# andi611/ZeroSpeech-TTS-without-T

Measured on AMD Instinct MI355X. Metric: mel-frames/sec (train_ae, seg_len=128, enc_size=1024), higher is better.
Workload: dtype bf16; 1 GPU; train_ae english hps seg_len=128 enc_size=1024 emb_size=1024 n_speakers=102 F=513, batch=256/GPU, dropout+Gumbel on, fwd+bwd+clip+Adam; global_batch=256, parallelism=dp1

## Files before the change

include/zs_amd.h:

```cpp
#ifndef ZS_AMD_H
#define ZS_AMD_H
#include <stddef.h>
#include <stdint.h>

#ifdef __cplusplus
extern "C" {
#endif

#define ZS_ABI_VERSION 1

enum { ZS_F32 = 0, ZS_BF16 = 1 };
enum { ZS_OK = 0, ZS_EINVAL = -1, ZS_ELAUNCH = -2, ZS_EWORKSPACE = -3 };
enum { ZS_PAD_ZERO = 0, ZS_PAD_REFLECT = 1 };
enum { ZS_ACT_NONE = 0, ZS_ACT_LRELU = 1, ZS_ACT_SIGMOID = 2, ZS_ACT_TANH = 3 };
enum { ZS_STORE_ROWS = 0, ZS_STORE_SPLIT2 = 1 };
enum { ZS_RES_NONE = 0, ZS_RES_IDENTITY = 1, ZS_RES_AVGPOOL2 = 2, ZS_RES_UPSAMPLE2 = 3 };

int zs_abi_version(void);
const char* zs_last_error(void);
int zs_set_option(const char* key, int value);

typedef struct {
  int32_t dtype;
  const void* A; int64_t lda; int64_t a_batch_stride;
  int32_t B, T_in, T_out;
  int32_t taps, stride, pad_left, pad_mode, gather;
  int32_t cin_pad;
  const void* W; int64_t ldw;
  int32_t N, n_pad;
  const float* bias;
  const float* pre_vec; int64_t pre_vec_ld; const int64_t* vec_idx;
  int32_t act; float slope;
  const void* dact_src; int64_t dact_ld;
  const void* add_src; int64_t add_ld; int32_t add_f32;
  void* out; int64_t ldc; int32_t out_f32; int32_t out_cols; int32_t store_mode;
  void* out2; int64_t ldc2; int32_t out2_cols; int32_t store_mode2;
  const float* vec2; int64_t vec2_ld;
  int32_t groups; int64_t a_gstride, w_gstride, out_gstride, bias_gstride;
  float* colsum; int64_t colsum_ld; int32_t colsum_col0;
  int32_t colsum_post;
  const int32_t* lengths; int32_t pad_right;
  int32_t w_in, w_out, taps_h;
} ZsGemmConv;
int zs_gemm_conv(const ZsGemmConv* p, void* stream);
enum { ZS_GEMM_PATH_P8 = 0, ZS_GEMM_PATH_RING_PP = 1, ZS_GEMM_PATH_RING = 2, ZS_GEMM_PATH_DMA64 = 3, ZS_GEMM_PATH_DMA128 = 4,
       ZS_GEMM_PATH_REG = 5 };
int zs_gemm_conv_path(const ZsGemmConv* p);

typedef struct {
  int32_t dtype;
  const void* dY; int64_t ldy; int32_t y_cols;
  const void* X; int64_t ldx; int64_t x_batch_stride; int32_t x_cols;
  int32_t B, T_in, T_out;
  int32_t taps, stride, pad_left, pad_mode;
  int32_t Cout, Cin;
  float* dW; int64_t so, si, sj;
  float* db;
  int32_t co_split2; int32_t accumulate;
  int32_t splits;
  void* workspace; size_t workspace_bytes;
  int32_t w_in, w_out, taps_h;
} ZsGemmWgrad;
size_t zs_gemm_wgrad_workspace_bytes(const ZsGemmWgrad* p);
int zs_gemm_wgrad(const ZsGemmWgrad* p, void* stream);

typedef struct {
  int32_t dtype;
  const float* W; int64_t so, si, sj;
  int32_t Cout, Cin, taps;
  int32_t transpose, co_split2;
  int32_t inner_pad;
  void* dst; int64_t ldw;
  int32_t n_rows, n_cols, row_offset, col_offset;
  const int32_t* row_perm;
} ZsPackWeight;
int zs_pack_weight(const ZsPackWeight* p, void* stream);
int zs_pack_weight_batch(const ZsPackWeight* jobs, int32_t n, int32_t max_blocks, void* stream);

typedef struct {
  const float* src; float* dst;
  int32_t len, src_stride, dst_stride;
} ZsVecCopy;
int zs_copy_vec_batch(const ZsVecCopy* jobs, int32_t n, void* stream);

typedef struct {
  int32_t dtype;
  const void* src; int64_t ld_src; int32_t src_f32;
  void* dst; int64_t ld_dst; int32_t dst_f32; int32_t col_off;
  int64_t rows; int32_t cols, fill_cols;
  int32_t act; float slope;
  void* dst2; int64_t ld_dst2; int32_t col_off2, fill_cols2; int32_t act2; float slope2;
} ZsCastRows;
int zs_cast_rows(const ZsCastRows* p, void* stream);

typedef struct {
  int32_t dtype;
  const void* x; int64_t ldx;
  const float* vec; int64_t vec_ld; const int64_t* idx;
  void* out; int64_t ldo; int32_t B, T, C, fill_cols;
} ZsAddRowvec;
int zs_add_rowvec(const ZsAddRowvec* p, void* stream);

typedef struct {
  int32_t dtype;
  const void* x; int64_t ldx;
  void* out; int64_t ldo;
  void* out2; int64_t ldo2; const float* vec2; int64_t vec2_ld; int32_t vec2_cols; const int64_t* idx;
  float* mean; float* rstd;
  int32_t B, T, C; float eps;
  float drop_p; uint64_t seed; uint32_t stream_id; const uint8_t* mask; int64_t mask_ld;
  int32_t res_mode; const void* res; int64_t ldres; int32_t T_res; int32_t res_pad_mode;
  const uint64_t* seed_ptr;
  const int32_t* lengths; const int32_t* res_lengths;
  int32_t stats_given;
} ZsInstNormFwd;
int zs_instnorm_fwd(const ZsInstNormFwd* p, void* stream);

typedef struct {
  int32_t dtype;
  const void* dout; int64_t ldd;
  const void* x; int64_t ldx;
  const float* mean; const float* rstd;
  void* dz; int64_t ldz;
  int32_t B, T, C;
  float drop_p; uint64_t seed; uint32_t stream_id; const uint8_t* mask; int64_t mask_ld;
  float slope;
  const uint64_t* seed_ptr;
} ZsInstNormBwd;
int zs_instnorm_bwd(const ZsInstNormBwd* p, void* stream);

typedef struct {
  int32_t dtype;
  const void* gp; int64_t ldg; int32_t pad_left, pad_right, pad_mode;
  int32_t B, T, C;
  float* emb_sum; int64_t emb_ld; int32_t emb_cols;
  int32_t res_mode; const void* res; int64_t ldres;
  const void* dact_src; int64_t dact_ld; float slope;
  void* out; int64_t ldo; int32_t unshuffle;
} ZsGradCombine;
int zs_grad_combine(const ZsGradCombine* p, void* stream);
int zs_norm_decomposition(int32_t kernel, int32_t dtype, int32_t T, int32_t C);

typedef struct {
  const float* emb_sum; int64_t emb_ld; const int64_t* idx; int32_t B;
  float* demb; int64_t demb_ld; int32_t n_rows, C; int32_t accumulate;
} ZsEmbScatter;
int zs_emb_scatter(const ZsEmbScatter* p, void* stream);

typedef struct {
  int32_t dtype;
  const void* logits; int64_t ld; int32_t logits_f32;
  const float* noise; int32_t noise_kind; uint64_t seed;
  int64_t rows; int32_t E; float tau;
  void* bits; int64_t ld_bits; int32_t bits_fill_cols;
  float* bits_f32;
  float* y0;
  const uint64_t* seed_ptr;
} ZsMbvFwd;
int zs_mbv_fwd(const ZsMbvFwd* p, void* stream);
typedef struct {
  int32_t dtype;
  const void* dbits; int64_t ld_dbits;
  const float* y0; int64_t rows; int32_t E; float tau;
  void* dlogits; int64_t ld; int32_t fill_cols;
} ZsMbvBwd;
int zs_mbv_bwd(const ZsMbvBwd* p, void* stream);

enum { ZS_ENC_ONE_HOT = 0, ZS_ENC_BINARY = 1, ZS_ENC_CONTINUES = 2 };
typedef struct {
  int32_t dtype; int32_t mode;
  const void* logits; int64_t ld; int32_t logits_f32;
  const float* noise; int32_t noise_kind; uint64_t seed;
  int64_t rows; int32_t E; float tau; float slope;
  void* bits; int64_t ld_bits; int32_t bits_fill_cols;
  float* bits_f32;
  float* y;
  float* s;
  const uint64_t* seed_ptr;
} ZsGumbelStFwd;
int zs_gumbel_st_fwd(const ZsGumbelStFwd* p, void* stream);
typedef struct {
  int32_t dtype; int32_t mode;
  const void* dbits; int64_t ld_dbits;
  const float* y; int64_t ld_y;
  const float* s;
  int64_t rows; int32_t E; float tau; float slope;
  void* dlogits; int64_t ld; int32_t fill_cols;
} ZsGumbelStBwd;
int zs_gumbel_st_bwd(const ZsGumbelStBwd* p, void* stream);

typedef struct {
  int32_t dtype;
  int32_t B, T, H;
  const void* gi; int64_t ldgi;
  const void* whh; int64_t ldw; int32_t n_pad; int64_t w_gstride;
  const float* bhh; int64_t bhh_gstride;
  void* out; int64_t ldo; int32_t out_col;
  void* gates;
  float* work; size_t work_bytes;
  int32_t whh_interleaved;
  uint32_t* status;
  const float* bcast_vec; int64_t bcast_ld; const int64_t* bcast_idx; int32_t bcast_col;
  int32_t dir1_forward;
} ZsGruFwd;
size_t zs_gru_work_bytes(int32_t B, int32_t H);
int zs_gru_fwd(const ZsGruFwd* p, void* stream);
int zs_gru_check(const float* work, int32_t B, int32_t H, void* stream);

typedef struct {
  int32_t dtype;
  void* x; int64_t ld; int32_t col0, cols;
  int32_t B, T; const int32_t* lengths;
} ZsRowsReverse;
int zs_rows_reverse(const ZsRowsReverse* p, void* stream);
typedef struct {
  int32_t dtype;
  int32_t B, T, H;
  const void* dout; int64_t ldd; int32_t dout_col;
  const void* out; int64_t ldo; int32_t out_col;
  const void* gates;
  const void* whh_t; int64_t ldw; int32_t n_pad; int64_t w_gstride;
  void* dgi; int64_t ldgi;
  void* dgh; int64_t ldgh;
  float* work; size_t work_bytes;
  uint32_t* status;
} ZsGruBwd;
int zs_gru_bwd(const ZsGruBwd* p, void* stream);
enum { ZS_GRU_PATH_WIDE = 0, ZS_GRU_PATH_PERSIST = 1, ZS_GRU_PATH_STEP_FUSED = 2, ZS_GRU_PATH_STEP_GEMM = 3 };
int zs_gru_path(int32_t pass, int32_t dtype, int32_t B, int32_t T, int32_t H, int32_t whh_interleaved, int32_t wide_aligned);

typedef struct {
  int32_t dtype;
  const float* x_dec; int64_t ld_dec;
  const float* x; int64_t ldx;
  int64_t rows; int32_t F;
  void* dlogits; int64_t ldg; int32_t fill_cols;
  float* partial; float* loss_out; float grad_scale;
} ZsL1Loss;
int zs_l1_loss(const ZsL1Loss* p, void* stream);

int zs_sqnorm(const float* g, int64_t n, double* partial, float* out_sq, void* stream);

typedef struct {
  float* p; float* g; float* m; float* v; int64_t n;
  float lr, beta1, beta2, eps, bc1, bc2;
  const float* sumsq; float max_norm; int32_t write_clipped_grad;
  const int32_t* step_ptr;
  float grad_scale;
  int32_t max_blocks;
} ZsAdam;
int zs_adam_clip(const ZsAdam* p, void* stream);

int zs_host_fetch(const void* src, void* dst, size_t bytes, int32_t workgroups, void* stream);

typedef struct {
  const float* pool; const int32_t* speaker; const int64_t* first;
  int64_t* cursor;
  int64_t n; int32_t B, seg_len, F, rank, world;
  float* x; int64_t* c;
  int32_t advance;
} ZsPoolGather;
int zs_pool_gather(const ZsPoolGather* p, void* stream);

int zs_step_counters(uint64_t* seed, int32_t* step, void* stream);

typedef struct {
  const float* logits; int64_t ld; const int64_t* target; int32_t B, n_class;
  float* loss_out; float* dlogits; int64_t ldg; float grad_scale; int32_t* correct_out;
} ZsSoftmaxCE;
int zs_softmax_ce(const ZsSoftmaxCE* p, void* stream);

typedef struct {
  const float* spec; const float* mag; const int32_t* lengths; int32_t n_utt, T_max;
  float* wav; int64_t wav_ld; float* frames_ws;
} ZsGlIstft;
int zs_gl_istft(const ZsGlIstft* p, void* stream);
typedef struct {
  const float* wav; int64_t wav_ld; const float* mag; const int32_t* lengths; int32_t n_utt, T_max;
  float* spec;
} ZsGlStft;
int zs_gl_stft_project(const ZsGlStft* p, void* stream);
typedef struct {
  const float* spec_in; float* spec_out;
  const float* mag; const int32_t* lengths; int32_t n_utt, T_max;
  float* wav; int64_t wav_ld;
  int32_t tile_frames;
  const int32_t* host_lengths;
  float momentum;
  float* spec_prev;
} ZsGlIter;
int zs_gl_iter(const ZsGlIter* p, void* stream);
int zs_griffin_lim(const ZsGlIter* p, float* spec_a, float* spec_b, int32_t n_iter, void* stream);
int zs_gl_chains_used(void);
typedef struct {
  const float* wav; int64_t wav_ld; const int32_t* n_samples; int32_t n_utt, T_max;
  float preemph, ref_db, max_db;
  float* mag; int64_t mag_ld;
  float* amp;
  const int32_t* start;
} ZsPreSpec;
int zs_pre_spectrogram(const ZsPreSpec* p, void* stream);
typedef struct {
  const float* wav; int64_t wav_ld;
  const int32_t* n_samples;
  int32_t n_utt, frame_length, hop;
  float top_db;
  int32_t* bounds;
  double* work; size_t work_bytes;
} ZsTrim;
size_t zs_trim_workspace_bytes(int32_t n_utt, int64_t wav_ld, int32_t frame_length, int32_t hop);
int zs_trim(const ZsTrim* p, void* stream);
int zs_pre_mel(const float* amp, const float* basis, float* mel, int64_t rows, int32_t n_mels, float ref_db, float max_db, void* stream);
int zs_gl_denormalize(const float* mag_norm, float* mag_amp, int64_t n, void* stream);
typedef struct {
  const float* xd; int64_t ld_xd;
  const float* m; int64_t ld_m;
  const int32_t* dst; int64_t rows;
  float* amp; int64_t amp_ld, amp_rows;
  int32_t mode, denorm;
} ZsGenScatter;
int zs_gen_scatter(const ZsGenScatter* p, void* stream);
typedef struct {
  const float* src; int64_t utt_stride; int32_t n_utt, T_max;
  const int32_t* table; int32_t n_frag, seg_len;
  float* dst;
} ZsFragGather;
int zs_frag_gather(const ZsFragGather* p, void* stream);
typedef struct {
  const float* logits; int64_t ld;
  const int32_t* target; int32_t n_frag;
  int32_t* pred; int32_t* correct; int32_t* count;
} ZsTclfScore;
int zs_tclf_score(const ZsTclfScore* p, void* stream);
int zs_gl_deemphasis(float* wav, int64_t wav_ld, const int32_t* lengths, int32_t n_utt, float coef, void* stream);
int zs_gl_frame_mse(const float* wav, int64_t wav_ld, const int32_t* lengths, int32_t n_utt, int32_t frame_length, int32_t hop,
                    double* mse, int64_t mse_ld, void* stream);
typedef struct {
  const float* src; int64_t src_ld;
  const int32_t* n_in;
  int32_t n_utt, sr_in, sr_out;
  const float* bank; int32_t n_phase, n_tap;
  float* dst; int64_t dst_ld;
  int32_t n_in_max;
} ZsResample;
int zs_resample(const ZsResample* p, void* stream);


typedef struct {
  int32_t dtype;
  const void* x; int64_t ldx; int32_t x_f32;
  void* out; int64_t ldo;
  int32_t B, H_in, H_out, Wd, C;
  int32_t k, stride, pad, pad_mode;
  int32_t full;
} ZsConv2dGather;
int zs_conv2d_gather(const ZsConv2dGather* p, void* stream);
typedef struct {
  int32_t dtype;
  const void* gp; int64_t ldg;
  void* out; int64_t ldo; int32_t out_f32;
  int32_t fill_cols;
  const void* add; int64_t ldadd;
  int32_t B, H_in, H_out, Wd, C;
  int32_t k, stride, pad, pad_mode;
  int32_t gp_rows;
  int32_t full;
} ZsConv2dFold;
int zs_conv2d_fold(const ZsConv2dFold* p, void* stream);
typedef struct {
  const float* x;
  const void* W; int64_t ldw;
  const float* bias; int32_t act; float slope;
  void* out; int64_t ldo;
  int32_t B, H, Wd, Cout, k, pad_mode;
} ZsConv1Fwd;
int zs_conv1_fwd(const ZsConv1Fwd* p, void* stream);
typedef struct {
  const float* x;
  const void* gz; int64_t ldg;
  float* dW; int64_t lddw;
  float* db;
  int32_t accumulate;
  int32_t B, H, Wd, Cout, k, pad_mode;
  float* workspace; size_t workspace_bytes;
} ZsConv1Wgrad;
size_t zs_conv1_wgrad_workspace(void);
int zs_conv1_wgrad(const ZsConv1Wgrad* p, void* stream);
typedef struct {
  int32_t dtype;
  const void* g00; const void* g01; const void* g10; const void* g11; int64_t ldg;
  int32_t B, H, W, C, Hp, Wp, pad, pad_mode;
  const void* add; int64_t ldadd;
  void* out; int64_t ldo; int32_t fill_cols;
} ZsConv2dUnpad;
int zs_conv2d_unpad(const ZsConv2dUnpad* p, void* stream);

typedef struct {
  int32_t dtype;
  const void* u; int64_t ldu;
  const void* v; int64_t ldv;
  const void* y; int64_t ldy; float slope;
  const void* w; int64_t ldw;
  const float* center_sum; float center_scale;
  int32_t B, T, C;
  float* s1; float* s2; float* s3;
  float* partial; size_t partial_bytes;
} ZsRowMoments;
size_t zs_row_moments_workspace(int32_t B, int32_t T, int32_t C);
int zs_row_moments(const ZsRowMoments* p, void* stream);

int zs_in2d_finalize(const float* s1, const float* q, float* mean, float* rstd, int64_t n_bc, int32_t T, float eps, void* stream);
int zs_in2d_stats(int32_t dtype, const void* y, int64_t ldy, int32_t B, int32_t T, int32_t C, float eps, float* mean, float* rstd,
                  float* partial, size_t partial_bytes, void* stream);
typedef struct {
  int32_t dtype;
  const void* y; int64_t ldy; void* a; int64_t lda;
  const float* mean; const float* rstd; const float* dm;
  int32_t B, T, C;
} ZsIn2dFwd;
int zs_in2d_fwd(const ZsIn2dFwd* p, void* stream);
typedef struct {
  int32_t dtype;
  const void* ga; int64_t ldga; const void* ga2; int64_t ldga2;
  const void* a; int64_t lda; const void* y; int64_t ldy;
  const float* S1; const float* S2; const float* S2x; const float* rstd; const float* dm;
  float slope;
  void* gz; int64_t ldgz;
  int32_t B, T, C;
} ZsIn2dBwd;
int zs_in2d_bwd(const ZsIn2dBwd* p, void* stream);
typedef struct {
  int32_t dtype;
  const void* gbz; int64_t ldgbz; const void* y; int64_t ldy; const void* a; int64_t lda; const void* ga; int64_t ldga;
  const float* A1; const float* A2; const float* S2; const float* rstd; const float* dm;
  float slope;
  void* gba; int64_t ldgba; void* xba; int64_t ldxba;
  int32_t B, T, C;
} ZsIn2dAdj;
int zs_in2d_adj(const ZsIn2dAdj* p, void* stream);

int zs_lerp_rows(const float* x, const float* y, const float* alpha, float* out, int32_t B, int64_t n, void* stream);
int zs_gp_penalty(const float* g, int32_t B, int64_t n, float scale, float* s_out, float* gp_out, float* gbar, void* stream);

int zs_gen_combine_fwd(const float* xd, const float* m, int64_t ld_in, float* x_gen, int64_t rows, int32_t F, int32_t mode, void* stream);
typedef struct {
  int32_t dtype;
  const float* dx_gen; int64_t ld_dx; const float* xd; const float* m; int64_t ld_in;
  void* dpre; int64_t ldo; int32_t fill_cols;
  int64_t rows; int32_t F; int32_t mode, tanh_out;
} ZsGenCombineBwd;
int zs_gen_combine_bwd(const ZsGenCombineBwd* p, void* stream);
int zs_l1_plain(const float* a, const float* b, int64_t n, float scale, float* partial, float* loss_out, float* d, void* stream);

typedef struct {
  int32_t dtype;
  const float* bits; const float* y0; const float* target;
  int64_t rows; int32_t E; float tau; float grad_scale;
  void* dlogits; int64_t ld; int32_t fill_cols;
  double* partial; float* loss_out;
} ZsBceMbvBwd;
int zs_bce_mbv_bwd(const ZsBceMbvBwd* p, void* stream);

typedef struct {
  int32_t dtype;
  const float* g; int64_t ldg;
  const void* pass_through; int64_t ld_pass;
  int32_t B, T, C, pad, pad_mode;
  float* dx; int64_t ldx;
} ZsEncDxFold;
int zs_enc_dx_fold(const ZsEncDxFold* p, void* stream);

#ifdef __cplusplus
}
#endif
#endif
```

zerospeech-tts-without-t_amd/_lib.py:

```python
import ctypes
import os
import re

_PKG = os.path.dirname(os.path.abspath(__file__))
_ROOT = os.path.dirname(_PKG)
HEADER = os.path.join(_ROOT, 'include', 'zs_amd.h')
_SAN = os.environ.get('ZS_SANITIZE', '').strip()
LIB_PATH = os.environ.get('ZS_LIB_PATH') or os.path.join(_PKG, 'libzs_amd.%s.so' % _SAN if _SAN else 'libzs_amd.so')

_CTYPES = {
    'int32_t': ctypes.c_int32, 'int64_t': ctypes.c_int64, 'uint32_t': ctypes.c_uint32, 'uint64_t': ctypes.c_uint64,
    'float': ctypes.c_float, 'double': ctypes.c_double, 'size_t': ctypes.c_size_t, 'int': ctypes.c_int,
}


def _strip_comments(text):
    return re.sub(r'/\*.*?\*/', ' ', text, flags=re.S)


def parse_header(path=HEADER):
    text = _strip_comments(open(path).read())
    structs = {}
    for body, name in re.findall(r'typedef\s+struct\s*\{(.*?)\}\s*(\w+)\s*;', text, flags=re.S):
        fields = []
        for decl in body.split(';'):
            decl = decl.strip()
            if not decl:
                continue
            decl = re.sub(r'\bconst\b', ' ', decl).strip()
            m = re.match(r'(\w+)\s*(.*)', decl, flags=re.S)
            base, rest = m.group(1), m.group(2)
            for item in rest.split(','):
                item = item.strip()
                ptr = item.startswith('*')
                fname = item.lstrip('* ').strip()
                fields.append((fname, ctypes.c_void_p if ptr else _CTYPES[base]))
        structs[name] = fields
    funcs = re.findall(r'^\s*(?:const\s+)?(?:int|size_t|char\s*\*|const char\s*\*)\s*\*?\s*(zs_\w+)\s*\(', text, flags=re.M)
    enums = {k: int(v) for k, v in re.findall(r'#define\s+(ZS_\w+)\s+(\d+)', text)}
    for body in re.findall(r'enum\s*\{(.*?)\}', text, flags=re.S):
        val = -1
        for item in body.split(','):
            item = item.strip()
            if not item:
                continue
            if '=' in item:
                k, v = item.split('=')
                val = int(v.strip(), 0)
                enums[k.strip()] = val
            else:
                val += 1
                enums[item] = val
    return structs, funcs, enums


_STRUCT_FIELDS, FUNCTIONS, ENUMS = parse_header()
globals().update(ENUMS)


def _make_struct(name, fields):
    return type(name, (ctypes.Structure,), {'_fields_': fields})


STRUCTS = {name: _make_struct(name, fields) for name, fields in _STRUCT_FIELDS.items()}

_lib = None


class ZsError(RuntimeError):
    pass


def lib():
    global _lib
    if _lib is None:
        if not os.path.exists(LIB_PATH):
            raise ZsError('libzs_amd.so is missing at %s: run `python -c "import __graft_entry__ as g; g.build()"` '
                          '(the HIP extension is mandatory; there is no fallback path)' % LIB_PATH)
        L = ctypes.CDLL(LIB_PATH)
        L.zs_last_error.restype = ctypes.c_char_p
        L.zs_abi_version.restype = ctypes.c_int
        L.zs_gemm_wgrad_workspace_bytes.restype = ctypes.c_size_t
        L.zs_gru_work_bytes.restype = ctypes.c_size_t
        L.zs_gru_work_bytes.argtypes = [ctypes.c_int32, ctypes.c_int32]
        L.zs_gru_check.argtypes = [ctypes.c_void_p, ctypes.c_int32, ctypes.c_int32, ctypes.c_void_p]
        L.zs_sqnorm.argtypes = [ctypes.c_void_p, ctypes.c_int64, ctypes.c_void_p, ctypes.c_void_p, ctypes.c_void_p]
        L.zs_step_counters.argtypes = [ctypes.c_void_p, ctypes.c_void_p, ctypes.c_void_p]
        L.zs_set_option.argtypes = [ctypes.c_char_p, ctypes.c_int]
        L.zs_pre_mel.argtypes = [ctypes.c_void_p, ctypes.c_void_p, ctypes.c_void_p, ctypes.c_int64, ctypes.c_int32, ctypes.c_float,
                                 ctypes.c_float, ctypes.c_void_p]
        V, I32, I64, F32 = ctypes.c_void_p, ctypes.c_int32, ctypes.c_int64, ctypes.c_float
        L.zs_row_moments_workspace.restype = ctypes.c_size_t
        L.zs_row_moments_workspace.argtypes = [I32, I32, I32]
        L.zs_in2d_finalize.argtypes = [V, V, V, V, I64, I32, F32, V]
        L.zs_in2d_stats.argtypes = [I32, V, I64, I32, I32, I32, F32, V, V, V, ctypes.c_size_t, V]
        L.zs_lerp_rows.argtypes = [V, V, V, V, I32, I64, V]
        L.zs_gp_penalty.argtypes = [V, I32, I64, F32, V, V, V, V]
        L.zs_gen_combine_fwd.argtypes = [V, V, I64, V, I64, I32, I32, V]
        L.zs_l1_plain.argtypes = [V, V, I64, F32, V, V, V, V]
        L.zs_host_fetch.argtypes = [V, V, ctypes.c_size_t, I32, V]
        L.zs_griffin_lim.argtypes = [ctypes.c_void_p, ctypes.c_void_p, ctypes.c_void_p, ctypes.c_int32, ctypes.c_void_p]
        L.zs_conv1_wgrad_workspace.restype = ctypes.c_size_t
        L.zs_conv1_wgrad_workspace.argtypes = []
        L.zs_gl_chains_used.argtypes = []
        L.zs_gl_chains_used.restype = ctypes.c_int
        if hasattr(L, 'zs_gl_denormalize'):
            L.zs_gl_denormalize.argtypes = [ctypes.c_void_p, ctypes.c_void_p, ctypes.c_int64, ctypes.c_void_p]
        if hasattr(L, 'zs_gl_deemphasis'):
            L.zs_gl_deemphasis.argtypes = [ctypes.c_void_p, ctypes.c_int64, ctypes.c_void_p, ctypes.c_int32, ctypes.c_float,
                                           ctypes.c_void_p]
        L.zs_gl_frame_mse.argtypes = [ctypes.c_void_p, ctypes.c_int64, ctypes.c_void_p, ctypes.c_int32, ctypes.c_int32, ctypes.c_int32,
                                      ctypes.c_void_p, ctypes.c_int64, ctypes.c_void_p]
        L.zs_trim_workspace_bytes.restype = ctypes.c_size_t
        L.zs_trim_workspace_bytes.argtypes = [I32, I64, I32, I32]
        if L.zs_abi_version() != ENUMS.get('ZS_ABI_VERSION', 1) and 'ZS_ABI_VERSION' in ENUMS:
            raise ZsError('libzs_amd.so ABI version mismatch')
        _lib = L
        for kv in filter(None, os.environ.get('ZS_OPTIONS', '').split(',')):
            k, _, v = kv.partition('=')
            set_option(k.strip(), int(v))
    return _lib


def set_option(key, value):
    rc = lib().zs_set_option(key.encode(), int(value))
    if rc < 0:
        check(rc, 'zs_set_option')
    return rc


def last_error():
    return lib().zs_last_error().decode('utf-8', 'replace')


def check(rc, what):
    if rc != 0:
        raise ZsError('%s failed (%d): %s' % (what, rc, last_error()))


def ptr(t, offset_elems=0):
    if t is None:
        return None
    return t.data_ptr() + offset_elems * t.element_size()


_FN = {}
_PACK = None
_VEC = None


def vec_copy(dst, src, stream, src_stride=1, dst_stride=1, n=None):
    n = n if n is not None else (dst.numel() + dst_stride - 1) // dst_stride
    job = STRUCTS['ZsVecCopy'](src=ptr(src), dst=ptr(dst), len=n, src_stride=src_stride, dst_stride=dst_stride)
    if _VEC is not None:
        _VEC.append(job)
        return
    fn = lib().zs_copy_vec_batch
    fn.argtypes = [ctypes.c_void_p, ctypes.c_int32, ctypes.c_void_p]
    check(fn(ctypes.addressof(job), 1, stream), 'zs_copy_vec_batch')


class pack_batch(object):

    def __init__(self, stream):
        self.stream = stream

    def __enter__(self):
        global _PACK, _VEC
        self._outer = (_PACK, _VEC)
        _PACK, _VEC = [], []
        return self

    def __exit__(self, et, ev, tb):
        global _PACK, _VEC
        jobs, vjobs = _PACK, _VEC
        _PACK, _VEC = self._outer
        if et is None and jobs:
            S = STRUCTS['ZsPackWeight']
            arr = (S * len(jobs))(*jobs)
            fn = lib().zs_pack_weight_batch
            fn.argtypes = [ctypes.c_void_p, ctypes.c_int32, ctypes.c_int32, ctypes.c_void_p]
            check(fn(ctypes.addressof(arr), len(jobs), 0, self.stream), 'zs_pack_weight_batch')
        if et is None and vjobs:
            S = STRUCTS['ZsVecCopy']
            arr = (S * len(vjobs))(*vjobs)
            fn = lib().zs_copy_vec_batch
            fn.argtypes = [ctypes.c_void_p, ctypes.c_int32, ctypes.c_void_p]
            check(fn(ctypes.addressof(arr), len(vjobs), self.stream), 'zs_copy_vec_batch')
        return False


def call(fname, sname, stream, **kw):
    try:
        s = STRUCTS[sname](**{k: v for k, v in kw.items() if v is not None})
    except TypeError as e:
        raise KeyError('%s: %s' % (sname, e))
    if _PACK is not None and fname == 'zs_pack_weight':
        _PACK.append(s)
        return s
    fn = _FN.get(fname)
    if fn is None:
        fn = getattr(lib(), fname)
        fn.argtypes = [ctypes.c_void_p, ctypes.c_void_p]
        _FN[fname] = fn
    rc = fn(ctypes.addressof(s), stream)
    if rc != 0:
        check(rc, fname)
    return s
```

zerospeech-tts-without-t_amd/csrc/zs_api.hip:

```cpp
#include <stdarg.h>

#include "zs_common.h"

static thread_local char g_err[512] = "";

void zs_set_error(const char* fmt, ...) {
  va_list ap;
  va_start(ap, fmt);
  vsnprintf(g_err, sizeof(g_err), fmt, ap);
  va_end(ap);
}

Knob* g_knobs = nullptr;

extern "C" int zs_set_option(const char* key, int value) {
  for (Knob* k = g_knobs; key && k; k = k->next)
    if (!strcmp(k->key, key)) return k->set(value);
  zs_set_error("zs_set_option: unknown key %s", key ? key : "(null)");
  return ZS_EINVAL;
}

int zs_check_launch(const char* what) {
  hipError_t e = hipGetLastError();
  if (e != hipSuccess) {
    zs_set_error("%s: launch failed: %s", what, hipGetErrorString(e));
    return ZS_ELAUNCH;
  }
  return ZS_OK;
}

extern "C" int zs_abi_version(void) { return ZS_ABI_VERSION; }
extern "C" const char* zs_last_error(void) { return g_err; }
```

zerospeech-tts-without-t_amd/csrc/zs_elem.hip:

```cpp
#include <string.h>

#include "zs_common.h"

namespace {

constexpr int NTE = 256;

template <typename T> __device__ __forceinline__ float ldT(const void* p, int64_t i) { return Elem<T>::ld((const T*)p + i); }
template <typename T> __device__ __forceinline__ void stT(void* p, int64_t i, float v) { Elem<T>::st((T*)p + i, v); }

template <typename T>
__device__ __forceinline__ void pack_weight_body(const ZsPackWeight& p, int64_t first, int64_t step) {
  const int64_t total = (int64_t)p.n_rows * p.n_cols;
  for (int64_t i = first; i < total; i += step) {
    const int row = (int)(i / p.n_cols);
    const int k = (int)(i - (int64_t)row * p.n_cols);
    const int tap = k / p.inner_pad, inner = k - tap * p.inner_pad;
    int n, ci;
    if (p.transpose == 0) { n = row; ci = inner; } else { n = inner; ci = row; }
    float v = 0.f;
    if (n < p.Cout && ci < p.Cin && tap < p.taps) {
      const int half = p.Cout >> 1;
      const int co = p.row_perm ? p.row_perm[n] : (p.co_split2 ? (n < half ? 2 * n : 2 * (n - half) + 1) : n);
      v = p.W[(int64_t)co * p.so + (int64_t)ci * p.si + (int64_t)tap * p.sj];
    }
    stT<T>(p.dst, (int64_t)(row + p.row_offset) * p.ldw + p.col_offset + k, v);
  }
}

template <typename T>
__global__ void pack_weight_kernel(const ZsPackWeight p) {
  pack_weight_body<T>(p, (int64_t)blockIdx.x * blockDim.x + threadIdx.x, (int64_t)gridDim.x * blockDim.x);
}

constexpr int PK_THREADS = 256, PK_MAX_TAPS = 7;
__host__ __device__ constexpr int pk_pow2_le(int x) { return x >= 64 ? 64 : x >= 32 ? 32 : x >= 16 ? 16 : x >= 8 ? 8 : x >= 4 ? 4 : x >= 2 ? 2 : 1; }
__host__ __device__ constexpr int pk_inner(int transpose) { return transpose ? 64 : 128; }
__host__ __device__ constexpr int pk_rows(int transpose, int taps) { return pk_pow2_le((transpose ? 64 : 32) / taps); }
inline int pk_tiles(const ZsPackWeight& p) {
  const int R = pk_rows(p.transpose, p.taps), I = pk_inner(p.transpose);
  return ((p.n_rows + R - 1) / R) * ((p.inner_pad + I - 1) / I);
}
constexpr size_t PK_LDS_BYTES = (4096 + 128) * sizeof(float);

template <typename T, int TAPS, int TR>
__device__ __forceinline__ void pack_tile(const ZsPackWeight& p, int tile, float* lds) {
  constexpr int R = pk_rows(TR, TAPS), I = pk_inner(TR);
  const int tid = threadIdx.x;
  const int tiles_i = (p.inner_pad + I - 1) / I;
  const int tr = tile / tiles_i, ti = tile - tr * tiles_i;
  const int r0 = tr * R, i0 = ti * I;
  if (r0 >= p.n_rows) return;
  const int half = p.Cout >> 1;
  auto co_of = [&](int n) { return p.row_perm ? p.row_perm[n] : (p.co_split2 ? (n < half ? 2 * n : 2 * (n - half) + 1) : n); };
  if (TR == 0) {
    constexpr int RUN = I * TAPS, PITCH = RUN + 1;
#pragma unroll 4
    for (int e = tid; e < R * RUN; e += PK_THREADS) {
      const int rl = e / RUN, x = e - rl * RUN;
      const int il = x / TAPS, tap = x - il * TAPS;
      const int n = r0 + rl, ci = i0 + il;
      float v = 0.f;
      if (n < p.Cout && ci < p.Cin) v = p.W[(int64_t)co_of(n) * p.so + (int64_t)ci * p.si + (int64_t)tap * p.sj];
      lds[rl * PITCH + x] = v;
    }
  } else {
    constexpr int RUN = R * TAPS, PITCH = RUN + 1;
#pragma unroll 4
    for (int e = tid; e < I * RUN; e += PK_THREADS) {
      const int il = e / RUN, x = e - il * RUN;
      const int rl = x / TAPS, tap = x - rl * TAPS;
      const int n = i0 + il, ci = r0 + rl;
      float v = 0.f;
      if (n < p.Cout && ci < p.Cin) v = p.W[(int64_t)co_of(n) * p.so + (int64_t)ci * p.si + (int64_t)tap * p.sj];
      lds[il * PITCH + x] = v;
    }
  }
  __syncthreads();
#pragma unroll 4
  for (int e = tid; e < R * TAPS * I; e += PK_THREADS) {
    const int il = e % I, t2 = e / I;
    const int tap = t2 % TAPS, rl = t2 / TAPS;
    const int row = r0 + rl, inner = i0 + il;
    if (row < p.n_rows && inner < p.inner_pad) {
      const float v = TR ? lds[il * (R * TAPS + 1) + rl * TAPS + tap] : lds[rl * (I * TAPS + 1) + il * TAPS + tap];
      stT<T>(p.dst, (int64_t)(row + p.row_offset) * p.ldw + p.col_offset + tap * p.inner_pad + inner, v);
    }
  }
  const int tail0 = TAPS * p.inner_pad, tw = p.n_cols - tail0;
  if (ti == 0 && tw > 0) {
    for (int e = tid; e < R * tw; e += PK_THREADS) {
      const int rl = e / tw, k = e - rl * tw;
      if (r0 + rl < p.n_rows) stT<T>(p.dst, (int64_t)(r0 + rl + p.row_offset) * p.ldw + p.col_offset + tail0 + k, 0.f);
    }
  }
}

template <typename T>
__device__ __forceinline__ void pack_tile_any(const ZsPackWeight& p, int tile, float* lds) {
#define ZS_PK_CASE(K) case K: if (p.transpose) pack_tile<T, K, 1>(p, tile, lds); else pack_tile<T, K, 0>(p, tile, lds); break;
  switch (p.taps) { ZS_PK_CASE(1) ZS_PK_CASE(2) ZS_PK_CASE(3) ZS_PK_CASE(4) ZS_PK_CASE(5) ZS_PK_CASE(6) ZS_PK_CASE(7) default: break; }
#undef ZS_PK_CASE
}

template <typename T>
__global__ __launch_bounds__(PK_THREADS) void pack_weight_tiled_kernel(const ZsPackWeight p) {
  extern __shared__ float pk_lds[];
  pack_tile_any<T>(p, blockIdx.x, pk_lds);
}

constexpr int PACK_BATCH = 32;
struct PackBatch { ZsPackWeight job[PACK_BATCH]; int32_t tile_start[PACK_BATCH + 1]; int32_t n; };

template <typename T>
__global__ __launch_bounds__(PK_THREADS) void pack_weight_batch_kernel(const PackBatch b) {
  extern __shared__ float pk_lds[];
  const int total = b.tile_start[b.n];
  for (int g = blockIdx.x; g < total; g += gridDim.x) {
    int j = 0;
    while (g >= b.tile_start[j + 1]) ++j;
    const ZsPackWeight& p = b.job[j];
    const int tile = g - b.tile_start[j], ntile = b.tile_start[j + 1] - b.tile_start[j];
    if (p.taps <= PK_MAX_TAPS) pack_tile_any<T>(p, tile, pk_lds);
    else pack_weight_body<T>(p, (int64_t)tile * blockDim.x + threadIdx.x, (int64_t)ntile * blockDim.x);
    __syncthreads();
  }
}

constexpr int VEC_BATCH = 32;
struct VecBatch { ZsVecCopy job[VEC_BATCH]; };
__global__ void copy_vec_batch_kernel(const VecBatch b) {
  const ZsVecCopy& j = b.job[blockIdx.y];
  for (int i = blockIdx.x * blockDim.x + threadIdx.x; i < j.len; i += gridDim.x * blockDim.x)
    j.dst[(int64_t)i * j.dst_stride] = j.src[(int64_t)i * j.src_stride];
}

template <typename T>
__global__ void cast_rows_kernel(const ZsCastRows p) {
  const int fc = (p.dst2 && p.fill_cols2 > p.fill_cols) ? p.fill_cols2 : p.fill_cols;
  const int lane = threadIdx.x & 63, wpb = blockDim.x >> 6;
  const int64_t nw = (int64_t)gridDim.x * wpb;
  const bool pair1 = !p.dst_f32 && sizeof(T) == 2 && ((p.col_off | (int)(p.ld_dst & 1)) & 1) == 0 && (((uintptr_t)p.dst) & 3) == 0;
  const bool pair2 = p.dst2 && sizeof(T) == 2 && ((p.col_off2 | (int)(p.ld_dst2 & 1)) & 1) == 0 && (((uintptr_t)p.dst2) & 3) == 0;
  for (int64_t r = (int64_t)blockIdx.x * wpb + (threadIdx.x >> 6); r < p.rows; r += nw) {
    for (int c = 2 * lane; c < fc; c += 128) {
      float x[2];
#pragma unroll
      for (int e = 0; e < 2; ++e)
        x[e] = (c + e < p.cols) ? (p.src_f32 ? ((const float*)p.src)[r * p.ld_src + c + e] : ldT<T>(p.src, r * p.ld_src + c + e)) : 0.f;
      {
        const float v0 = (p.act == ZS_ACT_LRELU) ? lrelu_f(x[0], p.slope) : x[0], v1 = (p.act == ZS_ACT_LRELU) ? lrelu_f(x[1], p.slope) : x[1];
        if (pair1 && c + 1 < p.fill_cols) {
          *reinterpret_cast<uint32_t*>((bf16_t*)p.dst + r * p.ld_dst + p.col_off + c) = (uint32_t)f2bf(v0) | ((uint32_t)f2bf(v1) << 16);
        } else {
          if (c < p.fill_cols) { if (p.dst_f32) ((float*)p.dst)[r * p.ld_dst + p.col_off + c] = v0; else stT<T>(p.dst, r * p.ld_dst + p.col_off + c, v0); }
          if (c + 1 < p.fill_cols) { if (p.dst_f32) ((float*)p.dst)[r * p.ld_dst + p.col_off + c + 1] = v1; else stT<T>(p.dst, r * p.ld_dst + p.col_off + c + 1, v1); }
        }
      }
      if (p.dst2) {
        const float v0 = (p.act2 == ZS_ACT_LRELU) ? lrelu_f(x[0], p.slope2) : x[0], v1 = (p.act2 == ZS_ACT_LRELU) ? lrelu_f(x[1], p.slope2) : x[1];
        if (pair2 && c + 1 < p.fill_cols2) {
          *reinterpret_cast<uint32_t*>((bf16_t*)p.dst2 + r * p.ld_dst2 + p.col_off2 + c) = (uint32_t)f2bf(v0) | ((uint32_t)f2bf(v1) << 16);
        } else {
          if (c < p.fill_cols2) stT<T>(p.dst2, r * p.ld_dst2 + p.col_off2 + c, v0);
          if (c + 1 < p.fill_cols2) stT<T>(p.dst2, r * p.ld_dst2 + p.col_off2 + c + 1, v1);
        }
      }
    }
  }
}

template <typename T>
__global__ void add_rowvec_kernel(const ZsAddRowvec p) {
  const int64_t rows = (int64_t)p.B * p.T;
  const int64_t total = rows * p.fill_cols;
  for (int64_t i = (int64_t)blockIdx.x * blockDim.x + threadIdx.x; i < total; i += (int64_t)gridDim.x * blockDim.x) {
    const int64_t r = i / p.fill_cols;
    const int c = (int)(i - r * p.fill_cols);
    const int b = (int)(r / p.T);
    float v = p.x ? ldT<T>(p.x, r * p.ldx + c) : 0.f;
    if (c < p.C) v += p.vec[p.idx[b] * p.vec_ld + c];
    stT<T>(p.out, r * p.ldo + c, v);
  }
}

template <typename T>
__global__ void add_rowvec_bcast8_kernel(const ZsAddRowvec p) {
  const int groups = p.fill_cols / 8;
  const int64_t total = (int64_t)p.B * p.T * groups;
  for (int64_t i = (int64_t)blockIdx.x * blockDim.x + threadIdx.x; i < total; i += (int64_t)gridDim.x * blockDim.x) {
    const int64_t r = i / groups;
    const int c0 = (int)(i - r * groups) * 8;
    const int b = (int)(r / p.T);
    const float* v = p.vec + p.idx[b] * p.vec_ld + c0;
    float o[8];
#pragma unroll
    for (int e = 0; e < 8; ++e) o[e] = (c0 + e < p.C) ? v[e] : 0.f;
    store8<T>((T*)p.out + r * p.ldo + c0, o);
  }
}

__global__ __launch_bounds__(128) void emb_scatter_kernel(const ZsEmbScatter p) {
  __shared__ int list[128];
  __shared__ int wcount[2];
  const int tid = threadIdx.x, lane = tid & 63, wave = tid >> 6;
  const int c = blockIdx.x * 128 + tid;
  const int r = blockIdx.y;
  float s = 0.f;
  for (int b0 = 0; b0 < p.B; b0 += 128) {
    const int b = b0 + tid;
    const bool hit = b < p.B && p.idx[b] == (int64_t)r;
    const unsigned long long m = __ballot(hit);
    if (lane == 0) wcount[wave] = __popcll(m);
    __syncthreads();
    const int n0 = wcount[0], n = n0 + wcount[1];
    if (hit) list[(wave ? n0 : 0) + __popcll(m & ((1ull << lane) - 1ull))] = b;
    __syncthreads();
    if (c < p.C)
      for (int i = 0; i < n; ++i) s += p.emb_sum[(int64_t)list[i] * p.emb_ld + c];
    __syncthreads();
  }
  if (c >= p.C) return;
  float* d = p.demb + (int64_t)r * p.demb_ld + c;
  *d = p.accumulate ? (*d + s) : s;
}

template <typename T>
__global__ void mbv_fwd_kernel(const ZsMbvFwd p) {
  const int64_t total = p.rows * p.bits_fill_cols;
  const uint64_t seed = p.seed + (p.seed_ptr ? *p.seed_ptr : 0ull);
  for (int64_t i = (int64_t)blockIdx.x * blockDim.x + threadIdx.x; i < total; i += (int64_t)gridDim.x * blockDim.x) {
    const int64_t r = i / p.bits_fill_cols;
    const int e = (int)(i - r * p.bits_fill_cols);
    float bit = 0.f;
    if (e < p.E) {
      float l0, l1;
      if (p.logits_f32) { l0 = ((const float*)p.logits)[r * p.ld + 2 * e]; l1 = ((const float*)p.logits)[r * p.ld + 2 * e + 1]; }
      else { l0 = ldT<T>(p.logits, r * p.ld + 2 * e); l1 = ldT<T>(p.logits, r * p.ld + 2 * e + 1); }
      const int64_t ni = (r * p.E + e) * 2;
      float g0, g1;
      if (p.noise_kind == 0) { g0 = p.noise[ni]; g1 = p.noise[ni + 1]; }
      else {
        float u0, u1;
        if (p.noise_kind == 1) { u0 = p.noise[ni]; u1 = p.noise[ni + 1]; }
        else { u0 = zs_uniform(seed, 0x6d627600u, (uint64_t)ni); u1 = zs_uniform(seed, 0x6d627600u, (uint64_t)ni + 1); }
        g0 = -logf(-logf(u0 + 1e-20f) + 1e-20f);
        g1 = -logf(-logf(u1 + 1e-20f) + 1e-20f);
      }
      const float a0 = __fdiv_rn(__fadd_rn(l0, g0), p.tau);
      const float a1 = __fdiv_rn(__fadd_rn(l1, g1), p.tau);
      const float mx = fmaxf(a0, a1);
      const float e0 = expf(a0 - mx), e1 = expf(a1 - mx);
      const float sum = __fadd_rn(e0, e1);
      const float y0 = __fdiv_rn(e0, sum), y1 = __fdiv_rn(e1, sum);
      const float hard = (y0 >= y1) ? 1.f : 0.f;
      bit = __fadd_rn(__fsub_rn(hard, y0), y0);
      if (p.bits_f32) p.bits_f32[r * p.E + e] = bit;
      if (p.y0) p.y0[r * p.E + e] = y0;
    }
    if (p.bits) stT<T>(p.bits, r * p.ld_bits + e, bit);
  }
}

template <typename T>
__global__ void mbv_bwd_kernel(const ZsMbvBwd p) {
  const int64_t total = p.rows * (p.fill_cols / 2);
  for (int64_t i = (int64_t)blockIdx.x * blockDim.x + threadIdx.x; i < total; i += (int64_t)gridDim.x * blockDim.x) {
    const int64_t r = i / (p.fill_cols / 2);
    const int e = (int)(i - r * (p.fill_cols / 2));
    float d0 = 0.f;
    if (e < p.E) {
      const float y0 = p.y0[r * p.E + e];
      d0 = ldT<T>(p.dbits, r * p.ld_dbits + e) * y0 * (1.f - y0) / p.tau;
    }
    stT<T>(p.dlogits, r * p.ld + 2 * e, d0);
    stT<T>(p.dlogits, r * p.ld + 2 * e + 1, -d0);
  }
}

template <typename T>
__global__ void l1_stage1_kernel(const ZsL1Loss p) {
  __shared__ float red[NTE / 64];
  const float gs = p.grad_scale / ((float)p.rows * (float)p.F);
  const int lane = threadIdx.x & 63, wpb = blockDim.x >> 6;
  const int64_t nw = (int64_t)gridDim.x * wpb;
  float s = 0.f;
  const bool pair = p.dlogits && sizeof(T) == 2 && (p.ldg & 1) == 0 && (((uintptr_t)p.dlogits) & 3) == 0;
  for (int64_t r = (int64_t)blockIdx.x * wpb + (threadIdx.x >> 6); r < p.rows; r += nw) {
    for (int c = 2 * lane; c < p.fill_cols; c += 128) {
      float g[2] = {0.f, 0.f};
#pragma unroll
      for (int e = 0; e < 2; ++e)
        if (c + e < p.F) {
          const float xd = p.x_dec[r * p.ld_dec + c + e];
          const float d = xd - p.x[r * p.ldx + c + e];
          s += fabsf(d);
          g[e] = (d > 0.f ? gs : (d < 0.f ? -gs : 0.f)) * xd * (1.f - xd);
        }
      if (pair && c + 1 < p.fill_cols) {
        *reinterpret_cast<uint32_t*>((bf16_t*)p.dlogits + r * p.ldg + c) = (uint32_t)f2bf(g[0]) | ((uint32_t)f2bf(g[1]) << 16);
      } else if (p.dlogits) {
        stT<T>(p.dlogits, r * p.ldg + c, g[0]);
        if (c + 1 < p.fill_cols) stT<T>(p.dlogits, r * p.ldg + c + 1, g[1]);
      }
    }
  }
  s = wave_sum(s);
  if (lane == 0) red[threadIdx.x >> 6] = s;
  __syncthreads();
  if (threadIdx.x == 0) { float t = 0.f; for (int w = 0; w < NTE / 64; ++w) t += red[w]; p.partial[blockIdx.x] = t; }
}
__global__ void l1_stage2_kernel(const float* partial, int n, float* out, double denom) {
  __shared__ double red[4];
  double s = 0.0;
  for (int i = threadIdx.x; i < n; i += blockDim.x) s += (double)partial[i];
  s = wave_sum_d(s);
  if ((threadIdx.x & 63) == 0) red[threadIdx.x >> 6] = s;
  __syncthreads();
  if (threadIdx.x == 0) *out = (float)((red[0] + red[1] + red[2] + red[3]) / denom);
}

__global__ void sqnorm_stage1_kernel(const float* g, int64_t n, double* partial) {
  __shared__ double red[NTE / 64];
  double s = 0.0;
  const int64_t n4 = ((((uintptr_t)g) & 15) == 0) ? (n >> 2) : 0;
  const float4* g4 = reinterpret_cast<const float4*>(g);
  const int64_t stride = (int64_t)gridDim.x * blockDim.x;
  int64_t i = (int64_t)blockIdx.x * blockDim.x + threadIdx.x;
  for (; i + stride < n4; i += 2 * stride) {
    const float4 a = g4[i], b = g4[i + stride];
    s += (double)a.x * a.x + (double)a.y * a.y + (double)a.z * a.z + (double)a.w * a.w;
    s += (double)b.x * b.x + (double)b.y * b.y + (double)b.z * b.z + (double)b.w * b.w;
  }
  for (; i < n4; i += stride) {
    const float4 a = g4[i];
    s += (double)a.x * a.x + (double)a.y * a.y + (double)a.z * a.z + (double)a.w * a.w;
  }
  for (int64_t k = 4 * n4 + (int64_t)blockIdx.x * blockDim.x + threadIdx.x; k < n; k += stride) {
    const float v = g[k]; s += (double)v * (double)v;
  }
  s = wave_sum_d(s);
  if ((threadIdx.x & 63) == 0) red[threadIdx.x >> 6] = s;
  __syncthreads();
  if (threadIdx.x == 0) { double t = 0.0; for (int w = 0; w < NTE / 64; ++w) t += red[w]; partial[blockIdx.x] = t; }
}
__global__ void sqnorm_stage2_kernel(const double* partial, int n, float* out) {
  __shared__ double red[4];
  double s = 0.0;
  for (int i = threadIdx.x; i < n; i += blockDim.x) s += partial[i];
  s = wave_sum_d(s);
  if ((threadIdx.x & 63) == 0) red[threadIdx.x >> 6] = s;
  __syncthreads();
  if (threadIdx.x == 0) *out = (float)(red[0] + red[1] + red[2] + red[3]);
}

__global__ void adam_kernel(const ZsAdam p) {
  const float gs = p.grad_scale != 0.f ? p.grad_scale : 1.f;
  float coef = gs;
  if (p.max_norm > 0.f && p.sumsq) {
    const float norm = sqrtf(*p.sumsq) * gs;
    coef = gs * fminf(p.max_norm / (norm + 1e-6f), 1.f);
  }
  float bc1 = p.bc1, bc2 = p.bc2;
  if (p.step_ptr) {
    const float t = (float)(*p.step_ptr);
    bc1 = 1.f - powf(p.beta1, t);
    bc2 = 1.f - powf(p.beta2, t);
  }
  const float step_size = p.lr / bc1;
  const float bc2_sqrt = sqrtf(bc2);
  auto upd = [&](float& w, float& g, float& m, float& v) {
    g *= coef;
    m = m + (g - m) * (1.f - p.beta1);
    v = v * p.beta2 + g * g * (1.f - p.beta2);
    const float denom = sqrtf(v) / bc2_sqrt + p.eps;
    w = w - step_size * (m / denom);
  };
  const int64_t tid = (int64_t)blockIdx.x * blockDim.x + threadIdx.x, nthr = (int64_t)gridDim.x * blockDim.x;
  const bool vec = ((((uintptr_t)p.p) | ((uintptr_t)p.g) | ((uintptr_t)p.m) | ((uintptr_t)p.v)) & 15) == 0;
  const int64_t n4 = vec ? p.n / 4 : 0;
  for (int64_t i = tid; i < n4; i += nthr) {
    float4 w = reinterpret_cast<float4*>(p.p)[i], g = reinterpret_cast<float4*>(p.g)[i];
    float4 m = reinterpret_cast<float4*>(p.m)[i], v = reinterpret_cast<float4*>(p.v)[i];
    upd(w.x, g.x, m.x, v.x); upd(w.y, g.y, m.y, v.y); upd(w.z, g.z, m.z, v.z); upd(w.w, g.w, m.w, v.w);
    reinterpret_cast<float4*>(p.p)[i] = w; reinterpret_cast<float4*>(p.m)[i] = m; reinterpret_cast<float4*>(p.v)[i] = v;
    if (p.write_clipped_grad) reinterpret_cast<float4*>(p.g)[i] = g;
  }
  for (int64_t i = 4 * n4 + tid; i < p.n; i += nthr) {
    float w = p.p[i], g = p.g[i], m = p.m[i], v = p.v[i];
    upd(w, g, m, v);
    p.p[i] = w; p.m[i] = m; p.v[i] = v;
    if (p.write_clipped_grad) p.g[i] = g;
  }
}

typedef __attribute__((ext_vector_type(4))) unsigned fetch_u32x4;
__global__ __launch_bounds__(256) void host_fetch_kernel(const fetch_u32x4* __restrict__ src, fetch_u32x4* __restrict__ dst, int64_t n16) {
  const int64_t stride = (int64_t)gridDim.x * blockDim.x;
  int64_t i = (int64_t)blockIdx.x * blockDim.x + threadIdx.x;
  for (; i + 7 * stride < n16; i += 8 * stride) {
    fetch_u32x4 v[8];
#pragma unroll
    for (int u = 0; u < 8; ++u) v[u] = __builtin_nontemporal_load(src + i + u * stride);
#pragma unroll
    for (int u = 0; u < 8; ++u) dst[i + u * stride] = v[u];
  }
  for (; i < n16; i += stride) dst[i] = __builtin_nontemporal_load(src + i);
}

__global__ void step_counters_kernel(uint64_t* seed, int32_t* step) {
  if (threadIdx.x == 0 && blockIdx.x == 0) {
    if (seed) *seed += 0x9E3779B97F4A7C15ull;
    if (step) *step += 1;
  }
}

__global__ void softmax_ce_kernel(const ZsSoftmaxCE p) {
  __shared__ float red[4];
  __shared__ int redc[4];
  float ls = 0.f; int corr = 0;
  for (int b = threadIdx.x; b < p.B; b += blockDim.x) {
    const float* l = p.logits + (int64_t)b * p.ld;
    float mx = l[0]; int am = 0;
    for (int j = 1; j < p.n_class; ++j) if (l[j] > mx) { mx = l[j]; am = j; }
    float se = 0.f;
    for (int j = 0; j < p.n_class; ++j) se += expf(l[j] - mx);
    const int t = (int)p.target[b];
    ls += (logf(se) + mx) - l[t];
    corr += (am == t);
    if (p.dlogits) {
      const float gs = p.grad_scale / (float)p.B;
      for (int j = 0; j < p.n_class; ++j)
        p.dlogits[(int64_t)b * p.ldg + j] = (expf(l[j] - mx) / se - (j == t ? 1.f : 0.f)) * gs;
    }
  }
  ls = wave_sum(ls);
  corr = (int)wave_sum((float)corr);
  if ((threadIdx.x & 63) == 0) { red[threadIdx.x >> 6] = ls; redc[threadIdx.x >> 6] = corr; }
  __syncthreads();
  if (threadIdx.x == 0) {
    *p.loss_out = (red[0] + red[1] + red[2] + red[3]) / (float)p.B;
    if (p.correct_out) *p.correct_out = redc[0] + redc[1] + redc[2] + redc[3];
  }
}

inline unsigned nblocks(int64_t total, int cap = 2048) {
  int64_t b = (total + NTE - 1) / NTE;
  if (b > cap) b = cap;
  if (b < 1) b = 1;
  return (unsigned)b;
}

}

#define ZS_DISPATCH(dtype, KERNEL, grid, block, stream, ...)                                            \
  do {                                                                                                  \
    if ((dtype) == ZS_F32) hipLaunchKernelGGL(KERNEL<float>, grid, block, 0, (hipStream_t)(stream), __VA_ARGS__); \
    else hipLaunchKernelGGL(KERNEL<bf16_t>, grid, block, 0, (hipStream_t)(stream), __VA_ARGS__);          \
  } while (0)

__global__ __launch_bounds__(NTE) void rows_reverse_kernel(const ZsRowsReverse p, int words, int64_t ld_bytes, int64_t col_bytes) {
  const int half = p.T >> 1;
  const int64_t total = (int64_t)p.B * half * words;
  for (int64_t i = (int64_t)blockIdx.x * blockDim.x + threadIdx.x; i < total; i += (int64_t)gridDim.x * blockDim.x) {
    const int w = (int)(i % words);
    const int64_t r = i / words;
    const int t = (int)(r % half), b = (int)(r / half);
    const int len = p.lengths ? p.lengths[b] : p.T;
    if (t >= (len >> 1)) continue;
    unsigned char* base = (unsigned char*)p.x + col_bytes + (int64_t)w * 4;
    uint32_t* lo = reinterpret_cast<uint32_t*>(base + ((int64_t)b * p.T + t) * ld_bytes);
    uint32_t* hi = reinterpret_cast<uint32_t*>(base + ((int64_t)b * p.T + (len - 1 - t)) * ld_bytes);
    const uint32_t a = *lo, c = *hi;
    *lo = c; *hi = a;
  }
}

static int pack_check(const ZsPackWeight* p) {
  ZS_REQUIRE(p && p->W && p->dst, "zs_pack_weight: null operand");
  ZS_REQUIRE(p->dtype == ZS_F32 || p->dtype == ZS_BF16, "zs_pack_weight: bad dtype");
  ZS_REQUIRE(p->Cout > 0 && p->Cin > 0 && p->taps > 0 && p->inner_pad > 0 && p->n_rows > 0 && p->n_cols > 0 &&
                 p->ldw >= (int64_t)p->col_offset + p->n_cols && p->n_cols >= p->taps * p->inner_pad,
             "zs_pack_weight: sizes (ldw %lld n_cols %d taps %d inner_pad %d)", (long long)p->ldw, p->n_cols, p->taps, p->inner_pad);
  ZS_REQUIRE((p->transpose ? p->Cout : p->Cin) <= p->inner_pad, "zs_pack_weight: inner_pad too small");
  ZS_REQUIRE(!p->co_split2 || p->Cout % 2 == 0, "zs_pack_weight: SPLIT2 needs even Cout");
  return ZS_OK;
}

extern "C" int zs_pack_weight(const ZsPackWeight* p, void* stream) {
  int rc = pack_check(p);
  if (rc) return rc;
  if (p->taps <= PK_MAX_TAPS) {
    const size_t lds = PK_LDS_BYTES;
    if (p->dtype == ZS_F32) hipLaunchKernelGGL(pack_weight_tiled_kernel<float>, dim3(pk_tiles(*p)), dim3(PK_THREADS), lds, (hipStream_t)stream, *p);
    else hipLaunchKernelGGL(pack_weight_tiled_kernel<bf16_t>, dim3(pk_tiles(*p)), dim3(PK_THREADS), lds, (hipStream_t)stream, *p);
  } else {
    ZS_DISPATCH(p->dtype, pack_weight_kernel, dim3(nblocks((int64_t)p->n_rows * p->n_cols, 4096)), dim3(NTE), stream, *p);
  }
  return zs_check_launch("zs_pack_weight");
}

extern "C" int zs_pack_weight_batch(const ZsPackWeight* jobs, int32_t n, int32_t max_blocks, void* stream) {
  ZS_REQUIRE(jobs && n > 0, "zs_pack_weight_batch: no jobs");
  for (int i = 0; i < n; ++i) {
    int rc = pack_check(jobs + i);
    if (rc) return rc;
    ZS_REQUIRE(jobs[i].dtype == jobs[0].dtype, "zs_pack_weight_batch: mixed dtypes");
  }
  for (int i0 = 0; i0 < n; i0 += PACK_BATCH) {
    const int m = n - i0 < PACK_BATCH ? n - i0 : PACK_BATCH;
    PackBatch b;
    memset(&b, 0, sizeof(b));
    int64_t total = 0;
    for (int i = 0; i < m; ++i) {
      b.job[i] = jobs[i0 + i];
      const ZsPackWeight& j = jobs[i0 + i];
      b.tile_start[i] = (int32_t)total;
      total += j.taps <= PK_MAX_TAPS ? (int64_t)pk_tiles(j) : (int64_t)nblocks((int64_t)j.n_rows * j.n_cols, 4096);
      ZS_REQUIRE(total < (1ll << 30), "zs_pack_weight_batch: too many tiles");
    }
    for (int i = m; i <= PACK_BATCH; ++i) b.tile_start[i] = (int32_t)total;
    b.n = m;
    const unsigned gx = (unsigned)((max_blocks > 0 && total > max_blocks) ? max_blocks : total);
    const size_t lds = PK_LDS_BYTES;
    if (jobs[0].dtype == ZS_F32) hipLaunchKernelGGL(pack_weight_batch_kernel<float>, dim3(gx), dim3(PK_THREADS), lds, (hipStream_t)stream, b);
    else hipLaunchKernelGGL(pack_weight_batch_kernel<bf16_t>, dim3(gx), dim3(PK_THREADS), lds, (hipStream_t)stream, b);
    int rc = zs_check_launch("zs_pack_weight_batch");
    if (rc) return rc;
  }
  return ZS_OK;
}

extern "C" int zs_copy_vec_batch(const ZsVecCopy* jobs, int32_t n, void* stream) {
  ZS_REQUIRE(jobs && n > 0, "zs_copy_vec_batch: no jobs");
  for (int i = 0; i < n; ++i)
    ZS_REQUIRE(jobs[i].src && jobs[i].dst && jobs[i].len > 0, "zs_copy_vec_batch: bad job %d", i);
  for (int i0 = 0; i0 < n; i0 += VEC_BATCH) {
    const int m = n - i0 < VEC_BATCH ? n - i0 : VEC_BATCH;
    VecBatch b;
    memset(&b, 0, sizeof(b));
    int mx = 1;
    for (int i = 0; i < m; ++i) { b.job[i] = jobs[i0 + i]; if (jobs[i0 + i].len > mx) mx = jobs[i0 + i].len; }
    unsigned gx = (unsigned)((mx + 255) / 256);
    if (gx > 64) gx = 64;
    hipLaunchKernelGGL(copy_vec_batch_kernel, dim3(gx, (unsigned)m), dim3(256), 0, (hipStream_t)stream, b);
    int rc = zs_check_launch("zs_copy_vec_batch");
    if (rc) return rc;
  }
  return ZS_OK;
}

extern "C" int zs_cast_rows(const ZsCastRows* p, void* stream) {
  ZS_REQUIRE(p && p->src && p->dst && p->rows > 0 && p->cols > 0 && p->fill_cols >= p->cols, "zs_cast_rows: bad args");
  ZS_REQUIRE(p->dtype == ZS_F32 || p->dtype == ZS_BF16, "zs_cast_rows: bad dtype");
  ZS_REQUIRE(!p->dst2 || p->fill_cols2 >= p->cols, "zs_cast_rows: fill_cols2 < cols");
  ZS_DISPATCH(p->dtype, cast_rows_kernel, dim3(nblocks(p->rows * 64, 2048)), dim3(NTE), stream, *p);
  return zs_check_launch("zs_cast_rows");
}

extern "C" int zs_add_rowvec(const ZsAddRowvec* p, void* stream) {
  ZS_REQUIRE(p && p->vec && p->idx && p->out && p->B > 0 && p->T > 0 && p->C > 0 && p->fill_cols >= p->C, "zs_add_rowvec: bad args");
  ZS_REQUIRE(p->dtype == ZS_F32 || p->dtype == ZS_BF16, "zs_add_rowvec: bad dtype");
  if (!p->x && p->fill_cols % 8 == 0 && p->ldo % 8 == 0 && (((uintptr_t)p->out) & 15) == 0) {
    ZS_DISPATCH(p->dtype, add_rowvec_bcast8_kernel, dim3(nblocks((int64_t)p->B * p->T * (p->fill_cols / 8), 4096)), dim3(NTE), stream, *p);
    return zs_check_launch("zs_add_rowvec");
  }
  ZS_DISPATCH(p->dtype, add_rowvec_kernel, dim3(nblocks((int64_t)p->B * p->T * p->fill_cols, 4096)), dim3(NTE), stream, *p);
  return zs_check_launch("zs_add_rowvec");
}

extern "C" int zs_rows_reverse(const ZsRowsReverse* p, void* stream) {
  ZS_REQUIRE(p && p->x && p->B > 0 && p->T > 0 && p->cols > 0 && p->col0 >= 0 && p->ld >= (int64_t)p->col0 + p->cols, "zs_rows_reverse: bad args");
  ZS_REQUIRE(p->dtype == ZS_F32 || p->dtype == ZS_BF16, "zs_rows_reverse: bad dtype");
  const int es = p->dtype == ZS_F32 ? 4 : 2;
  ZS_REQUIRE((p->cols * es) % 4 == 0 && (p->col0 * es) % 4 == 0 && (p->ld * es) % 4 == 0 && (((uintptr_t)p->x) & 3) == 0,
             "zs_rows_reverse: the column block must be made of whole 4-byte words");
  if (p->T < 2) return ZS_OK;
  const int words = p->cols * es / 4;
  hipLaunchKernelGGL(rows_reverse_kernel, dim3(nblocks((int64_t)p->B * (p->T >> 1) * words, 4096)), dim3(NTE), 0, (hipStream_t)stream, *p, words,
                     (int64_t)p->ld * es, (int64_t)p->col0 * es);
  return zs_check_launch("zs_rows_reverse");
}

extern "C" int zs_emb_scatter(const ZsEmbScatter* p, void* stream) {
  ZS_REQUIRE(p && p->emb_sum && p->idx && p->demb && p->B > 0 && p->n_rows > 0 && p->C > 0, "zs_emb_scatter: bad args");
  hipLaunchKernelGGL(emb_scatter_kernel, dim3((p->C + 127) / 128, p->n_rows), dim3(128), 0, (hipStream_t)stream, *p);
  return zs_check_launch("zs_emb_scatter");
}

extern "C" int zs_mbv_fwd(const ZsMbvFwd* p, void* stream) {
  ZS_REQUIRE(p && p->logits && p->rows > 0 && p->E > 0 && p->tau > 0.f, "zs_mbv_fwd: bad args");
  ZS_REQUIRE(p->dtype == ZS_F32 || p->dtype == ZS_BF16, "zs_mbv_fwd: bad dtype");
  ZS_REQUIRE(p->noise_kind == 2 || p->noise, "zs_mbv_fwd: noise missing");
  ZS_REQUIRE(p->bits || p->bits_f32, "zs_mbv_fwd: no output");
  ZsMbvFwd q = *p;
  if (!q.bits || q.bits_fill_cols < q.E) q.bits_fill_cols = q.E;
  ZS_DISPATCH(p->dtype, mbv_fwd_kernel, dim3(nblocks(q.rows * q.bits_fill_cols)), dim3(NTE), stream, q);
  return zs_check_launch("zs_mbv_fwd");
}

extern "C" int zs_mbv_bwd(const ZsMbvBwd* p, void* stream) {
  ZS_REQUIRE(p && p->dbits && p->y0 && p->dlogits && p->rows > 0 && p->E > 0 && p->fill_cols >= 2 * p->E && p->fill_cols % 2 == 0,
             "zs_mbv_bwd: bad args");
  ZS_REQUIRE(p->dtype == ZS_F32 || p->dtype == ZS_BF16, "zs_mbv_bwd: bad dtype");
  ZS_DISPATCH(p->dtype, mbv_bwd_kernel, dim3(nblocks(p->rows * (p->fill_cols / 2))), dim3(NTE), stream, *p);
  return zs_check_launch("zs_mbv_bwd");
}

extern "C" int zs_l1_loss(const ZsL1Loss* p, void* stream) {
  ZS_REQUIRE(p && p->x_dec && p->x && p->partial && p->loss_out && p->rows > 0 && p->F > 0, "zs_l1_loss: bad args");
  ZS_REQUIRE(p->dtype == ZS_F32 || p->dtype == ZS_BF16, "zs_l1_loss: bad dtype");
  ZsL1Loss q = *p;
  if (!q.dlogits || q.fill_cols < q.F) q.fill_cols = q.F;
  const unsigned nb = nblocks(q.rows * 64, 1024);
  ZS_DISPATCH(p->dtype, l1_stage1_kernel, dim3(nb), dim3(NTE), stream, q);
  int rc = zs_check_launch("zs_l1_loss.stage1");
  if (rc) return rc;
  hipLaunchKernelGGL(l1_stage2_kernel, dim3(1), dim3(256), 0, (hipStream_t)stream, (const float*)p->partial, (int)nb, p->loss_out,
                     (double)p->rows * (double)p->F);
  return zs_check_launch("zs_l1_loss.stage2");
}

extern "C" int zs_sqnorm(const float* g, int64_t n, double* partial, float* out_sq, void* stream) {
  ZS_REQUIRE(g && partial && out_sq && n > 0, "zs_sqnorm: bad args");
  const unsigned nb = nblocks(n, 1024);
  hipLaunchKernelGGL(sqnorm_stage1_kernel, dim3(nb), dim3(NTE), 0, (hipStream_t)stream, g, n, partial);
  int rc = zs_check_launch("zs_sqnorm.stage1");
  if (rc) return rc;
  hipLaunchKernelGGL(sqnorm_stage2_kernel, dim3(1), dim3(256), 0, (hipStream_t)stream, (const double*)partial, (int)nb, out_sq);
  return zs_check_launch("zs_sqnorm.stage2");
}

extern "C" int zs_adam_clip(const ZsAdam* p, void* stream) {
  ZS_REQUIRE(p && p->p && p->g && p->m && p->v && p->n > 0, "zs_adam_clip: bad args");
  ZS_REQUIRE(p->step_ptr || (p->bc1 > 0.f && p->bc2 > 0.f), "zs_adam_clip: bias corrections");
  unsigned nb = nblocks((p->n + 3) / 4, 4096);
  if (p->max_blocks > 0 && nb > (unsigned)p->max_blocks) nb = (unsigned)p->max_blocks;
  hipLaunchKernelGGL(adam_kernel, dim3(nb), dim3(NTE), 0, (hipStream_t)stream, *p);
  return zs_check_launch("zs_adam_clip");
}

extern "C" int zs_host_fetch(const void* src, void* dst, size_t bytes, int32_t workgroups, void* stream) {
  ZS_REQUIRE(src && dst && bytes > 0 && bytes % 16 == 0 && (((uintptr_t)src) & 15) == 0 && (((uintptr_t)dst) & 15) == 0, "zs_host_fetch: bad args (16-byte granularity)");
  const int wg = workgroups > 0 ? workgroups : 32;
  hipLaunchKernelGGL(host_fetch_kernel, dim3((unsigned)wg), dim3(256), 0, (hipStream_t)stream, (const fetch_u32x4*)src, (fetch_u32x4*)dst, (int64_t)(bytes / 16));
  return zs_check_launch("zs_host_fetch");
}

extern "C" int zs_step_counters(uint64_t* seed, int32_t* step, void* stream) {
  ZS_REQUIRE(seed || step, "zs_step_counters: bad args");
  hipLaunchKernelGGL(step_counters_kernel, dim3(1), dim3(64), 0, (hipStream_t)stream, seed, step);
  return zs_check_launch("zs_step_counters");
}

extern "C" int zs_softmax_ce(const ZsSoftmaxCE* p, void* stream) {
  ZS_REQUIRE(p && p->logits && p->target && p->loss_out && p->B > 0 && p->n_class > 0, "zs_softmax_ce: bad args");
  hipLaunchKernelGGL(softmax_ce_kernel, dim3(1), dim3(256), 0, (hipStream_t)stream, *p);
  return zs_check_launch("zs_softmax_ce");
}
```

zerospeech-tts-without-t_amd/engine.py:

```python
import functools
import os
import torch

from . import _lib as L
from .layers import (Act, ConvLayer, GruLayer, cast_rows, colsum_ok, fork_side, grad_combine, instnorm_bwd, instnorm_fwd, join_side,
                     next_uid, rup)

LRELU = L.ZS_ACT_LRELU


def _half_up(t):
    return (t + 1) // 2


def _norm_stats(ctx, training, prefix, key, n):
    if not training:
        return None, None
    return ctx.f32(prefix + 'mean' + key, n), ctx.f32(prefix + 'rstd' + key, n)


def ragged_lengths(who, lengths, training, B, T, lo):
    if training:
        raise L.ZsError('%s: ragged batches are an inference feature' % who)
    l0 = torch.as_tensor(lengths, dtype=torch.int32).reshape(-1)
    if l0.numel() != B or int(l0.max()) > T or int(l0.min()) < lo:
        raise L.ZsError('%s: lengths must be %d values in [%d, %d]' % (who, B, lo, T))
    return l0


GUMBEL_MODES = {'one_hot': L.ZS_ENC_ONE_HOT, 'binary': L.ZS_ENC_BINARY, 'continues': L.ZS_ENC_CONTINUES}


def linear_width(enc_mode, E):
    return {'multilabel_binary': 2 * E, 'binary': E * E}.get(enc_mode, E)


class EncoderEngine(object):
    def __init__(self, ctx, P, G, c_in, c_h1, c_h2, c_h3, enc_size, ns, dp, seg_len, enc_mode='multilabel_binary'):
        self.ctx = ctx
        self.uid = next_uid()
        self.c_in, self.c1, self.c2, self.H, self.E = c_in, c_h1, c_h2, c_h3, enc_size
        self.mode = enc_mode
        self.n_lin = linear_width(enc_mode, enc_size)
        self.ns, self.dp = float(ns), float(dp)
        self.pad_mode = L.ZS_PAD_REFLECT if seg_len >= 64 else L.ZS_PAD_ZERO
        if c_h1 % 8 or c_h2 % 8:
            raise ValueError('c_h1 and c_h2 must be multiples of 8 (16-byte rows)')
        mk = functools.partial(ConvLayer.from_params, ctx, P, G, pad_mode=self.pad_mode)
        self.conv1s = [mk('conv1s.%d' % i) for i in range(7)]
        self.conv2 = mk('conv2')
        self.convs = [(mk('conv%d' % a), mk('conv%d' % b, stride=2)) for a, b in ((3, 4), (5, 6), (7, 8))]
        self.dense = [(mk('dense%d' % a), mk('dense%d' % b)) for a, b in ((1, 2), (3, 4))]
        self.gru = GruLayer(ctx, P, G, 'RNN.', name='enc%d' % self.uid)
        self.linear = mk('linear')
        self.layers = self.conv1s + [self.conv2] + [l for p in self.convs for l in p] + [l for p in self.dense for l in p] + \
            [self.linear]
        self.ncat = 7 * c_h1 + c_in
        self.tape = None
        self.tapes = {}
        self.bank_d = None

    def pack(self):
        with L.pack_batch(self.ctx.stream):
            for l in self.layers:
                l.pack()
            self.gru.pack()
            if self.bank_d is not None:
                self._pack_bank_d()

    def forward(self, x, training, noise=None, noise_kind=2, seed=0, drop_masks=None, seed_ptr=None, lengths=None, tape=None):
        c, ns = self.ctx, self.ns
        B, T, F = x.shape
        Ls = [None] * 4
        if lengths is not None:
            l0 = ragged_lengths('EncoderEngine', lengths, training, B, T, 9)
            l1 = (l0 + 1) // 2; l2 = (l1 + 1) // 2; l3 = (l2 + 1) // 2
            self.last_lengths = l3
            ld = torch.stack([l0, l1, l2, l3]).to(c.device, non_blocking=True)
            Ls = [ld[i] for i in range(4)]
        assert F == self.c_in and x.dtype == torch.float32 and x.is_contiguous()
        st = c.stream
        c1, c2, H, E = self.c1, self.c2, self.H, self.E
        dp = self.dp if training else 0.0
        masks = drop_masks if drop_masks is not None else [None] * 6
        Ts = [T, _half_up(T), _half_up(_half_up(T)), _half_up(_half_up(_half_up(T)))]
        T4 = Ts[3]
        ksfx = '' if tape is None else '_' + str(tape)
        tag = '_%d_%d_%d' % (self.uid, B, T) + ksfx
        tp = {'B': B, 'T': T, 'Ts': Ts, 'training': training, 'seed': seed, 'masks': masks, 'dp': dp, 'seed_ptr': seed_ptr,
              'tag': tag, 'ksfx': ksfx}
        drop = dict(p=dp, seed=seed, seed_ptr=seed_ptr)
        skey = lambda k, Tk: '%d_%d_%d_%d' % (self.uid, k, B, Tk) + ksfx

        xin = c.act('e_xin' + tag, B, T, F)
        cat = c.act('e_cat' + tag, B, T, self.ncat)
        cast_rows(c, L.ptr(x), F, xin, dst2=cat, col_off2=7 * c1, act2=LRELU, slope2=ns)
        if c.overlap_wgrad and B * T >= 4096:
            sts = fork_side(c.device)
            for i, l in enumerate(self.conv1s):
                with torch.cuda.stream(sts[i % len(sts)]):
                    l.fwd(xin, out=cat.sub(i * c1, c1), act=LRELU, slope=ns, lengths=Ls[0])
            join_side(c.device)
        else:
            for i, l in enumerate(self.conv1s):
                l.fwd(xin, out=cat.sub(i * c1, c1), act=LRELU, slope=ns, lengths=Ls[0])
        y2 = c.act('e_y2' + tag, B, T, c2)
        self.conv2.fwd(cat, out=y2, act=LRELU, slope=ns)
        a = c.act('e_a0' + tag, B, T, c2)
        mean, rstd = _norm_stats(c, training, 'e_', skey(0, T), B * y2.ld)
        instnorm_fwd(c, y2, a, mean, rstd, self.pad_mode, lengths=Ls[0], stream_id=1, mask=masks[0], **drop)
        tp.update(xin=xin, cat=cat, y2=y2, a0=a, st0=(mean, rstd, 0), blocks=[], dense=[])
        for i, (la, lb) in enumerate(self.convs):
            ya = c.act('e_ya%d' % i + tag, B, Ts[i], c2)
            la.fwd(a, out=ya, act=LRELU, slope=ns, lengths=Ls[i])
            yb = c.act('e_yb%d' % i + tag, B, Ts[i + 1], c2)
            lb.fwd(ya, out=yb, act=LRELU, slope=ns, lengths=Ls[i])
            an = c.act('e_a%d' % (i + 1) + tag, B, Ts[i + 1], c2)
            k = 1 + i
            mean, rstd = _norm_stats(c, training, 'e_', skey(k, Ts[i + 1]), B * yb.ld)
            instnorm_fwd(c, yb, an, mean, rstd, self.pad_mode, res_mode=L.ZS_RES_AVGPOOL2, res=a, lengths=Ls[i + 1],
                         res_lengths=Ls[i], stream_id=k + 1, mask=masks[k], **drop)
            tp['blocks'].append((a, ya, yb, (mean, rstd, k)))
            a = an
        cat2 = c.act('e_cat2' + tag, B, T4, c2 + 2 * H)
        for j, (la, lb) in enumerate(self.dense):
            d1 = c.act('e_d1%d' % j + tag, B, T4, c2)
            la.fwd(a, out=d1, act=LRELU, slope=ns)
            d2 = c.act('e_d2%d' % j + tag, B, T4, c2)
            lb.fwd(d1, out=d2, act=LRELU, slope=ns)
            out = c.act('e_do%d' % j + tag, B, T4, c2) if j == 0 else Act(cat2.t, B, T4, c2, cat2.ld, 0, rup(c2, 32))
            k = 4 + j
            mean, rstd = _norm_stats(c, training, 'e_', skey(k, T4), B * d2.ld)
            instnorm_fwd(c, d2, out, mean, rstd, self.pad_mode, res_mode=L.ZS_RES_IDENTITY, res=a, lengths=Ls[3], stream_id=k + 1,
                         mask=masks[k], **drop)
            tp['dense'].append((a, d1, d2, (mean, rstd, k)))
            a = out
        gi = c.act('e_gi' + tag, B, T4, 6 * H)
        gates = c.raw('e_gates' + tag, B * T4 * 8 * H, c.tdt) if training else None
        self.gru.fwd(a, cat2, c2, gi, gates, lengths=Ls[3])
        logits = c.act('e_logits' + tag, B, T4, self.n_lin, dtype=torch.float32)
        self.linear.fwd(cat2, out=logits, out_f32=True)
        bits = c.act('e_bits' + tag, B, T4, E)
        bits_f32 = c.f32('e_bitsf' + tag, B * T4 * E)
        s = None
        if self.mode == 'multilabel_binary':
            y0 = c.f32('e_y0' + tag, B * T4 * E)
            L.call('zs_mbv_fwd', 'ZsMbvFwd', st, dtype=c.dt, logits=logits.ptr(), ld=logits.ld, logits_f32=1,
                   noise=L.ptr(noise), noise_kind=noise_kind, seed=seed, seed_ptr=seed_ptr, rows=B * T4, E=E, tau=0.1, bits=bits.ptr(),
                   ld_bits=bits.ld, bits_fill_cols=bits.ld, bits_f32=L.ptr(bits_f32), y0=L.ptr(y0))
        else:
            soft = self.mode != 'continues'
            y0 = c.f32('e_y0' + tag, B * T4 * self.n_lin) if (training and soft) else None
            s = c.f32('e_s' + tag, B * T4 * E) if (training and self.mode == 'binary') else None
            L.call('zs_gumbel_st_fwd', 'ZsGumbelStFwd', st, dtype=c.dt, mode=GUMBEL_MODES[self.mode], logits=logits.ptr(),
                   ld=logits.ld, logits_f32=1, noise=(L.ptr(noise) if soft else None), noise_kind=noise_kind, seed=seed,
                   seed_ptr=seed_ptr, rows=B * T4, E=E, tau=0.1, slope=self.ns, bits=bits.ptr(), ld_bits=bits.ld,
                   bits_fill_cols=bits.ld, bits_f32=L.ptr(bits_f32), y=L.ptr(y0), s=L.ptr(s))
        tp.update(cat2=cat2, gates=gates, y0=y0, s=s, T4=T4, gru_in=a, logits=logits, bits_f32=bits_f32)
        self.tape = tp
        self.tapes[tape] = tp
        return bits, bits_f32[:B * T4 * E].view(B, T4, E), logits

    def backward(self, dbits, dlogits_extra=None):
        self.backward_main(dbits, dlogits_extra)
        self.backward_bank()

    def backward_main(self, dbits, dlogits_extra=None, param_grads=True, tape=None):
        c, ns = self.ctx, self.ns
        tp = self.tape if tape is None else self.tapes[tape]
        assert tp is not None and tp['training']
        pg = param_grads
        B, T, Ts, T4 = tp['B'], tp['T'], tp['Ts'], tp['T4']
        c1, c2, H, E = self.c1, self.c2, self.H, self.E
        st = c.stream
        tag = tp['tag']
        cat2 = tp['cat2']
        drop, masks = dict(p=tp['dp'], seed=tp['seed'], seed_ptr=tp['seed_ptr']), tp['masks']
        dlog = c.act('e_dlog' + tag, B, T4, self.n_lin)
        if dbits is not None:
            if self.mode == 'multilabel_binary':
                L.call('zs_mbv_bwd', 'ZsMbvBwd', st, dtype=c.dt, dbits=dbits.ptr(), ld_dbits=dbits.ld, y0=L.ptr(tp['y0']),
                       rows=B * T4, E=E, tau=0.1, dlogits=dlog.ptr(), ld=dlog.ld, fill_cols=dlog.ld)
            else:
                cont = self.mode == 'continues'
                y, ld_y = (tp['logits'].ptr(), tp['logits'].ld) if cont else (L.ptr(tp['y0']), self.n_lin)
                L.call('zs_gumbel_st_bwd', 'ZsGumbelStBwd', st, dtype=c.dt, mode=GUMBEL_MODES[self.mode], dbits=dbits.ptr(),
                       ld_dbits=dbits.ld, y=y, ld_y=ld_y, s=L.ptr(tp['s']), rows=B * T4, E=E, tau=0.1, slope=ns,
                       dlogits=dlog.ptr(), ld=dlog.ld, fill_cols=dlog.ld)
            if dlogits_extra is not None:
                dlog.t[:B * T4 * dlog.ld].add_(dlogits_extra.t[:B * T4 * dlogits_extra.ld])
        else:
            dlog = dlogits_extra
        if pg:
            self.linear.wgrad(dlog, cat2)
        dcat2 = c.act('e_dcat2' + tag, B, T4, cat2.C)
        self.linear.dgrad(dlog, T4, dcat2)
        dgi = c.act('e_dgi' + tag, B, T4, 6 * H)
        dgh = c.act('e_dgh' + tag, B, T4, 6 * H)
        gin = tp['gru_in']
        da = c.act('e_da_d' + tag, B, T4, c2)
        self.gru.bwd(dcat2, c2, cat2, c2, tp['gates'], gin, dgi, dgh, da, add_src=dcat2, param_grads=pg)
        for j in (1, 0):
            la, lb = self.dense[j]
            xin, d1, d2, (mean, rstd, k) = tp['dense'][j]
            dz2 = c.act('e_dz2%d' % j + tag, B, T4, c2)
            instnorm_bwd(c, da, d2, mean, rstd, dz2, ns, stream_id=k + 1, mask=masks[k], **drop)
            if pg:
                lb.wgrad(dz2, d1)
            dz1 = c.act('e_dz1%d' % j + tag, B, T4, c2)
            lb.dgrad(dz2, T4, dz1, dact_src=d1, slope=ns)
            if pg:
                la.wgrad(dz1, xin)
            dn = c.act('e_da_d%d' % j + tag, B, T4, c2)
            la.dgrad(dz1, T4, dn, add_src=da)
            da = dn
        for i in (2, 1, 0):
            la, lb = self.convs[i]
            a, ya, yb, (mean, rstd, k) = tp['blocks'][i]
            dzb = c.act('e_dzb%d' % i + tag, B, Ts[i + 1], c2)
            instnorm_bwd(c, da, yb, mean, rstd, dzb, ns, stream_id=k + 1, mask=masks[k], **drop)
            if pg:
                lb.wgrad(dzb, ya)
            gp = c.act('e_gp%d' % i + tag, B, Ts[i] + 4, c2)
            lb.dgrad(dzb, Ts[i], gp)
            dza = c.act('e_dza%d' % i + tag, B, Ts[i], c2)
            grad_combine(c, gp, Ts[i], 2, 2, self.pad_mode, gp.ld, dza, ns, dact=ya)
            if pg:
                la.wgrad(dza, a)
            la.dgrad(dza, Ts[i], gp)
            dn = c.act('e_da%d' % i + tag, B, Ts[i], c2)
            grad_combine(c, gp, Ts[i], 2, 2, self.pad_mode, gp.ld, dn, ns, res_mode=L.ZS_RES_AVGPOOL2, res=da)
            da = dn
        y2, cat, xin = tp['y2'], tp['cat'], tp['xin']
        dz = c.act('e_dzy2' + tag, B, T, c2)
        mean, rstd, k = tp['st0']
        instnorm_bwd(c, da, y2, mean, rstd, dz, ns, stream_id=k + 1, mask=masks[k], **drop)
        dcat = c.act('e_dcat' + tag, B, T, self.ncat)
        if not pg:
            self.conv2.dgrad(dz, T, dcat, dact_src=cat, slope=ns)
            return dcat
        self.conv2.wgrad(dz, cat)
        self.conv2.dgrad(dz, T, dcat, dact_src=cat, slope=ns, n_cols=7 * c1)
        self._bank = (dcat, xin)

    BANK_PAD = 3

    def _pack_bank_d(self):
        c, c1 = self.ctx, self.c1
        ld, cp = self.bank_d_ld, self.bank_d_cp
        for i, l in enumerate(self.conv1s):
            k = l.k
            for j in range(k):
                s = j + self.BANK_PAD - k // 2
                L.call('zs_pack_weight', 'ZsPackWeight', c.stream, dtype=c.dt, W=L.ptr(l.w, j), so=self.c_in * k, si=k, sj=1,
                       Cout=c1, Cin=self.c_in, taps=1, transpose=1, co_split2=0, inner_pad=c1, dst=L.ptr(self.bank_d), ldw=ld,
                       n_rows=self.bank_d_rows, n_cols=c1, row_offset=0, col_offset=s * cp + i * c1)

    def _bank_operand(self):
        if self.bank_d is None:
            c = self.ctx
            self.bank_d_cp = rup(7 * self.c1, c.kc)
            self.bank_d_ld = 7 * self.bank_d_cp
            self.bank_d_rows = rup(self.c_in, 128)
            self.bank_d = torch.zeros(self.bank_d_rows * self.bank_d_ld + 512, dtype=c.tdt, device=c.device)
            with L.pack_batch(c.stream):
                self._pack_bank_d()
        return self.bank_d

    def backward_input(self, dbits=None, dlogits=None, tape=None):
        if dbits is None and dlogits is None:
            raise ValueError('backward_input: dbits or dlogits')
        tp = self.tape if tape is None else self.tapes[tape]
        dcat = self.backward_main(dbits, dlogits, param_grads=False, tape=tape)
        c = self.ctx
        B, T, P = tp['B'], tp['T'], self.BANK_PAD
        W = self._bank_operand()
        if dcat.ld < self.bank_d_cp:
            raise L.ZsError('backward_input: concatenation rows of %d columns < K chunk %d' % (dcat.ld, self.bank_d_cp))
        g = c.act('e_gbank' + tp['tag'], B, T + 2 * P, self.c_in, dtype=torch.float32)
        L.call('zs_gemm_conv', 'ZsGemmConv', c.stream, dtype=c.dt, A=dcat.ptr(), lda=dcat.ld, a_batch_stride=T * dcat.ld, B=B, T_in=T,
               T_out=T + 2 * P, taps=7, stride=1, pad_left=0, pad_mode=L.ZS_PAD_ZERO, gather=1, cin_pad=self.bank_d_cp, W=L.ptr(W),
               ldw=self.bank_d_ld, N=self.c_in, n_pad=self.bank_d_rows, act=L.ZS_ACT_NONE, out=g.ptr(), ldc=g.ld,
               out_cols=g.ld, store_mode=L.ZS_STORE_ROWS, groups=1, out_f32=1)
        n = B * T * self.c_in
        dx = c.f32('e_dx' + tp['tag'], n)[:n].view(B, T, self.c_in)
        L.call('zs_enc_dx_fold', 'ZsEncDxFold', c.stream, dtype=c.dt, g=g.ptr(), ldg=g.ld, pass_through=dcat.ptr(7 * self.c1), ld_pass=dcat.ld, B=B, T=T, C=self.c_in, pad=P,
               pad_mode=self.pad_mode, dx=L.ptr(dx), ldx=self.c_in)
        return dx

    def backward_bank(self):
        dcat, xin = self._bank
        for i, l in enumerate(self.conv1s):
            l.wgrad(dcat.sub(i * self.c1, self.c1), xin)


class DecoderEngine(object):
    def __init__(self, ctx, P, G, c_in, c_out, c_h, c_a, ns, seg_len, output_mask=False):
        self.ctx = ctx
        self.uid = next_uid()
        self.E, self.F, self.ch, self.n_spk = c_in, c_out, c_h, c_a
        self.ns = float(ns)
        self.pad_mode = L.ZS_PAD_REFLECT if seg_len >= 64 else L.ZS_PAD_ZERO
        self.out_act = L.ZS_ACT_TANH if output_mask else L.ZS_ACT_SIGMOID
        if c_h % 32:
            raise ValueError('Decoder c_h must be a multiple of 32 (got %d)' % c_h)
        mk = functools.partial(ConvLayer.from_params, ctx, P, G, pad_mode=self.pad_mode)
        self.input_emb = mk('input_emb')
        self.convs = [(mk('conv%d' % a, split2=True), mk('conv%d' % b)) for a, b in ((1, 2), (3, 4), (5, 6))]
        self.dense = [(mk('dense%d' % a), mk('dense%d' % b)) for a, b in ((1, 2), (3, 4))]
        self.gru = GruLayer(ctx, P, G, 'RNN.', name='dec%d' % self.uid)
        self.dense5 = mk('dense5')
        self.linear = mk('linear')
        self.emb = [P['emb%d.weight' % i] for i in range(1, 6)]
        self.gemb = [G['emb%d.weight' % i] for i in range(1, 6)]
        self.e_dense, self.e_rnn = 3, 4
        self.layers = [self.input_emb] + [l for p in self.convs for l in p] + [l for p in self.dense for l in p] + \
            [self.dense5, self.linear]
        self.tape = None

    def pack(self):
        with L.pack_batch(self.ctx.stream):
            for l in self.layers:
                l.pack()
            self.gru.pack()

    def forward(self, bits, cidx, training, lengths=None):
        c, ns, ch = self.ctx, self.ns, self.ch
        B, T0 = bits.B, bits.T
        Ls = [None] * 4
        if lengths is not None:
            l0 = ragged_lengths('DecoderEngine', lengths, training, B, T0, 2)
            ld = torch.stack([l0, 2 * l0, 4 * l0, 8 * l0]).to(c.device, non_blocking=True)
            Ls = [ld[i] for i in range(4)]
        tag = '_%d_%d_%d' % (self.uid, B, T0)
        st = c.stream
        emb = self.emb
        tp = {'B': B, 'T0': T0, 'training': training, 'cidx': cidx, 'bits': bits, 'blocks': [], 'dense': []}
        x = c.act('d_x0' + tag, B, T0, ch)
        xe = c.act('d_xe0' + tag, B, T0, ch)
        self.input_emb.fwd(bits, out=x, out2=xe, vec2=emb[0], idx=cidx)
        T = T0
        for i, (la, lb) in enumerate(self.convs):
            ya = c.act('d_ya%d' % i + tag, B, T, 2 * ch) if training else None
            s = c.act('d_s%d' % i + tag, B, 2 * T, ch)
            la.fwd(xe, out=ya, act=LRELU, slope=ns, out2=s, vec2=emb[i], idx=cidx, store_mode2=L.ZS_STORE_SPLIT2, lengths=Ls[i])
            yb = c.act('d_yb%d' % i + tag, B, 2 * T, ch)
            lb.fwd(s, out=yb, act=LRELU, slope=ns, lengths=Ls[i + 1])
            xn = c.act('d_x%d' % (i + 1) + tag, B, 2 * T, ch)
            xen = c.act('d_xe%d' % (i + 1) + tag, B, 2 * T, ch)
            nxt = emb[i + 1] if i < 2 else emb[3]
            stt = _norm_stats(c, training, 'd_', '%d_c%d_%d_%d' % (self.uid, i, B, 2 * T), B * yb.ld)
            instnorm_fwd(c, yb, xn, *stt, self.pad_mode, res_mode=L.ZS_RES_UPSAMPLE2, res=x, lengths=Ls[i + 1], out2=xen, vec2=nxt,
                         idx=cidx)
            tp['blocks'].append((x, xe, ya, s, yb, stt, T))
            x, xe, T = xn, xen, 2 * T
        return self._fwd_dense(tp, x, xe, cidx, T, tag, B, training, Ls[3])

    def _fwd_dense(self, tp, x, xe, cidx, T, tag, B, training, lengths):
        c, ns, ch, emb = self.ctx, self.ns, self.ch, self.emb
        ed, er = self.e_dense, self.e_rnn
        cat3 = c.act('d_cat3' + tag, B, T, 3 * ch)
        for j, (la, lb) in enumerate(self.dense):
            y1 = c.act('d_y1%d' % j + tag, B, T, ch)
            y1e = c.act('d_y1e%d' % j + tag, B, T, ch)
            la.fwd(xe, out=y1, act=LRELU, slope=ns, out2=y1e, vec2=emb[ed], idx=cidx)
            y2 = c.act('d_y2%d' % j + tag, B, T, ch)
            lb.fwd(y1e, out=y2, act=LRELU, slope=ns)
            xn = c.act('d_dx%d' % j + tag, B, T, ch) if j == 0 else Act(cat3.t, B, T, ch, cat3.ld, 0, ch)
            xen = c.act('d_dxe%d' % j + tag, B, T, ch)
            stt = _norm_stats(c, training, 'd_', '%d_d%d_%d_%d' % (self.uid, j, B, T), B * y2.ld)
            instnorm_fwd(c, y2, xn, *stt, self.pad_mode, res_mode=L.ZS_RES_IDENTITY, res=x, lengths=lengths, out2=xen,
                         vec2=(emb[ed] if j == 0 else emb[er]), idx=cidx)
            tp['dense'].append((x, xe, y1, y1e, y2, stt))
            x, xe = xn, xen
        H = ch // 2
        gi = c.act('d_gi' + tag, B, T, 6 * H)
        gates = c.raw('d_gates' + tag, B * T * 8 * H, c.tdt) if training else None
        self.gru.fwd(xe, cat3, ch, gi, gates, bcast=(emb[er], cidx, 2 * ch), lengths=lengths)
        h5 = c.act('d_h5' + tag, B, T, ch)
        self.dense5.fwd(cat3, out=h5, act=LRELU, slope=ns)
        return self._fwd_tail(c, tp, h5, cat3, gates, xe, T, tag, B)

    def _fwd_tail(self, c, tp, h5, cat3, gates, xe, T, tag, B):
        xdec = c.act('d_xdec' + tag, B, T, self.F, dtype=torch.float32)
        self.linear.fwd(h5, out=xdec, act=self.out_act, out_f32=True)
        tp.update(cat3=cat3, gates=gates, gru_in=xe, h5=h5, T=T)
        self.tape = tp
        return xdec

    def backward(self, dlogit, need_dbits=True):
        self.backward_head(dlogit)
        return self.backward_convs(need_dbits)

    def backward_head(self, dlogit):
        c, ns, ch, tp = self.ctx, self.ns, self.ch, self.tape
        assert tp is not None and tp['training']
        B, T0, T = tp['B'], tp['T0'], tp['T']
        tag = '_%d_%d_%d' % (self.uid, B, T0)
        cat3, h5 = tp['cat3'], tp['h5']
        H = ch // 2
        ed, er = self.e_dense, self.e_rnn
        self._embsum = c.f32('d_embsum' + tag, 6 * B * ch)
        self._embsum.zero_()
        self.linear.wgrad(dlogit, h5)
        dz5 = c.act('d_dz5' + tag, B, T, ch)
        fuse = colsum_ok(T) and os.environ.get('ZS_FUSE_COLSUM', '1') == '1'
        esum = lambda k: L.ptr(self._embsum, k * B * ch)
        slot = lambda k, col0=0: (esum(k), ch, col0)
        thin5 = fuse and ch % 128 == 0 and os.environ.get('ZS_THIN_EMB5', '1') == '1'
        self.linear.dgrad(dlogit, T, dz5, dact_src=h5, slope=ns, colsum=(slot(5) if thin5 else None), colsum_post=True)
        self.dense5.wgrad(dz5, cat3)
        dcat3 = c.act('d_dcat3' + tag, B, T, 3 * ch)
        if thin5:
            self.dense5.dgrad(dz5, T, dcat3, n_cols=2 * ch)
            s32 = Act(self._embsum, B, 1, ch, ch, 5 * B * ch)
            sT = c.act('d_s5' + tag, B, 1, ch)
            cast_rows(c, s32.ptr(), ch, sT)
            slot4 = Act(self._embsum, B, 1, ch, ch, er * B * ch)
            self.dense5.dgrad(sT, 1, slot4, add_src=slot4, out_f32=True, add_f32=True, n_cols=ch, n_off=2 * ch)
        elif fuse:
            self.dense5.dgrad(dz5, T, dcat3, colsum=slot(er, 2 * ch), out_cols=2 * ch)
        else:
            self.dense5.dgrad(dz5, T, dcat3)
            grad_combine(c, dcat3.sub(2 * ch, ch), T, 0, 0, self.pad_mode, ch, None, ns, emb_sum=esum(er))
        dgi = c.act('d_dgi' + tag, B, T, 6 * H)
        dgh = c.act('d_dgh' + tag, B, T, 6 * H)
        gp = c.act('d_gpA' + tag, B, T + 2, ch)
        gpv = Act(gp.t, B, T, ch, gp.ld)
        dx = c.act('d_dxA' + tag, B, T, ch)
        if fuse:
            self.gru.bwd(dcat3, ch, cat3, ch, tp['gates'], tp['gru_in'], dgi, dgh, dx, add_src=dcat3.sub(0, ch), colsum=slot(er))
        else:
            self.gru.bwd(dcat3, ch, cat3, ch, tp['gates'], tp['gru_in'], dgi, dgh, gpv)
            grad_combine(c, gpv, T, 0, 0, self.pad_mode, ch, dx, ns, emb_sum=esum(er), res_mode=L.ZS_RES_IDENTITY, res=dcat3.sub(0, ch))
        for j in (1, 0):
            la, lb = self.dense[j]
            xin, xe, y1, y1e, y2, stt = tp['dense'][j]
            dz2 = c.act('d_dz2%d' % j + tag, B, T, ch)
            instnorm_bwd(c, dx, y2, *stt, dz2, ns)
            lb.wgrad(dz2, y1e)
            dz1 = c.act('d_dz1%d' % j + tag, B, T, ch)
            if fuse:
                lb.dgrad(dz2, T, dz1, dact_src=y1, slope=ns, colsum=slot(ed))
            else:
                lb.dgrad(dz2, T, gpv)
                grad_combine(c, gpv, T, 0, 0, self.pad_mode, ch, dz1, ns, emb_sum=esum(ed), dact=y1)
            la.wgrad(dz1, xe)
            dn = c.act('d_dxD%d' % j + tag, B, T, ch)
            if fuse:
                la.dgrad(dz1, T, dn, add_src=dx, colsum=slot(ed))
            else:
                la.dgrad(dz1, T, gpv)
                grad_combine(c, gpv, T, 0, 0, self.pad_mode, ch, dn, ns, emb_sum=esum(ed), res_mode=L.ZS_RES_IDENTITY, res=dx)
            dx = dn
        self._bw = (dx, gp, tag)

    def backward_convs(self, need_dbits=True):
        c, ns, ch, tp = self.ctx, self.ns, self.ch, self.tape
        dx, gp, tag = self._bw
        B, T0 = tp['B'], tp['T0']
        for i in (2, 1, 0):
            la, lb = self.convs[i]
            xin, xe, ya, s, yb, stt, Ti = tp['blocks'][i]
            esum = L.ptr(self._embsum, i * B * ch)
            T2 = 2 * Ti
            dzb = c.act('d_dzb%d' % i + tag, B, T2, ch)
            instnorm_bwd(c, dx, yb, *stt, dzb, ns)
            lb.wgrad(dzb, s)
            gp2 = Act(gp.t, B, T2 + 2, ch, gp.ld)
            lb.dgrad(dzb, T2, gp2)
            dza = c.act('d_dza%d' % i + tag, B, Ti, 2 * ch)
            grad_combine(c, gp2, T2, 1, 1, self.pad_mode, ch, dza, ns, emb_sum=esum, dact=ya, unshuffle=1)
            la.wgrad(dza, xe)
            gp1 = Act(gp.t, B, Ti + 2, ch, gp.ld)
            la.dgrad(dza, Ti, gp1)
            dn = c.act('d_dxC%d' % i + tag, B, Ti, ch)
            grad_combine(c, gp1, Ti, 1, 1, self.pad_mode, ch, dn, ns, emb_sum=esum, res_mode=L.ZS_RES_UPSAMPLE2,
                         res=dx)
            dx = dn
        sts = fork_side(c.device) if c.overlap_wgrad else None
        for k in range(5):
            st_k = sts[k % len(sts)].cuda_stream if sts is not None else c.stream
            L.call('zs_emb_scatter', 'ZsEmbScatter', st_k, emb_sum=L.ptr(self._embsum, k * B * ch), emb_ld=ch,
                   idx=L.ptr(tp['cidx']), B=B, demb=L.ptr(self.gemb[k]), demb_ld=ch, n_rows=self.n_spk, C=ch, accumulate=0)
        bits = tp['bits']
        self.input_emb.wgrad(dx, bits)
        dbits = None
        if need_dbits:
            dbits = c.act('d_dbits' + tag, B, T0, self.E)
            self.input_emb.dgrad(dx, T0, dbits)
        return dbits


class PatcherEngine(DecoderEngine):

    def __init__(self, ctx, P, G, c_in, c_out, c_h, c_a, ns):
        self.ctx = ctx
        self.uid = next_uid()
        self.E, self.F, self.ch, self.n_spk = c_in, c_out, c_h, c_a
        self.ns = float(ns)
        self.pad_mode = L.ZS_PAD_ZERO
        self.out_act = L.ZS_ACT_SIGMOID
        if c_h % 32:
            raise ValueError('Spectrogram_Patcher c_h must be a multiple of 32 (got %d)' % c_h)
        mk = functools.partial(ConvLayer.from_params, ctx, P, G, pad_mode=self.pad_mode)
        self.input_layer = mk('input_layer')
        self.dense = [(mk('dense%d' % a), mk('dense%d' % b)) for a, b in ((1, 2), (3, 4))]
        self.gru = GruLayer(ctx, P, G, 'RNN.', name='sp%d' % self.uid)
        self.dense5 = mk('dense5')
        self.linear = mk('linear')
        self.emb = [P['emb1.weight'], P['emb2.weight']]
        self.gemb = [G['emb1.weight'], G['emb2.weight']]
        self.e_dense, self.e_rnn = 0, 1
        self.layers = [self.input_layer] + [l for p in self.dense for l in p] + [self.dense5, self.linear]
        self.tape = None

    def forward(self, xd, cidx, training, lengths=None):
        c, ch = self.ctx, self.ch
        B, T = xd.B, xd.T
        ln = None
        if lengths is not None:
            ln = ragged_lengths('PatcherEngine', lengths, training, B, T, 1).to(c.device, non_blocking=True)
        tag = '_%d_%d_%d' % (self.uid, B, T)
        xin = c.act('p_xin' + tag, B, T, self.E)
        cast_rows(c, xd.ptr(), xd.ld, xin)
        tp = {'B': B, 'T0': T, 'training': training, 'cidx': cidx, 'xin': xin, 'dense': []}
        x = c.act('d_x0' + tag, B, T, ch)
        xe = c.act('d_xe0' + tag, B, T, ch)
        self.input_layer.fwd(xin, out=x, out2=xe, vec2=self.emb[0], idx=cidx)
        return self._fwd_dense(tp, x, xe, cidx, T, tag, B, training, ln)

    def backward(self, dlogit, need_dbits=False):
        if need_dbits:
            raise L.ZsError('PatcherEngine: the gradient w.r.t. the input spectrogram is not computed')
        self.backward_head(dlogit)
        dx, _, _ = self._bw
        c, tp, B, ch = self.ctx, self.tape, self.tape['B'], self.ch
        for k in range(2):
            L.call('zs_emb_scatter', 'ZsEmbScatter', c.stream, emb_sum=L.ptr(self._embsum, k * B * ch), emb_ld=ch, idx=L.ptr(tp['cidx']),
                   B=B, demb=L.ptr(self.gemb[k]), demb_ld=ch, n_rows=self.n_spk, C=ch, accumulate=0)
        self.input_layer.wgrad(dx, tp['xin'])
        return None


class ClassifierEngine(object):

    def __init__(self, ctx, P, G, c_in, c_h, n_class, dp, ns, seg_len):
        self.ctx, self.uid = ctx, next_uid()
        self.c_in, self.c_h, self.n_class = c_in, c_h, n_class
        self.ns, self.dp = float(ns), float(dp)
        self.pad_mode = L.ZS_PAD_REFLECT if seg_len >= 64 else L.ZS_PAD_ZERO
        mk = functools.partial(ConvLayer.from_params, ctx, P, G, pad_mode=self.pad_mode)
        self.blocks = [(mk('conv1'), mk('conv2'), False), (mk('conv3'), mk('conv4'), True), (mk('conv5'), mk('conv6'), True),
                       (mk('conv7'), mk('conv8'), False)]
        self.conv9 = mk('conv9', padded=False)
        self.layers = [l for b in self.blocks for l in b[:2]] + [self.conv9]
        self.tape = None

    def pack(self):
        with L.pack_batch(self.ctx.stream):
            for l in self.layers:
                l.pack()

    def forward(self, x, training, seed=0, drop_masks=None):
        c, ns = self.ctx, self.ns
        B, T = x.B, x.T
        if T != self.conv9.k:
            raise L.ZsError('SpeakerClassifier expects %d encoded frames (got %d)' % (self.conv9.k, T))
        tag = '_%d_%d_%d' % (self.uid, B, T)
        dp = self.dp if training else 0.0
        masks = drop_masks if drop_masks is not None else [None] * 4
        tp = {'B': B, 'T': T, 'training': training, 'seed': seed, 'masks': masks, 'dp': dp, 'x': x, 'blocks': []}
        a = x
        for i, (la, lb, res) in enumerate(self.blocks):
            ya = c.act('c_ya%d' % i + tag, B, T, la.Cout)
            la.fwd(a, out=ya, act=LRELU, slope=ns)
            yb = c.act('c_yb%d' % i + tag, B, T, lb.Cout)
            lb.fwd(ya, out=yb, act=LRELU, slope=ns)
            out = c.act('c_o%d' % i + tag, B, T, lb.Cout)
            mean, rstd = _norm_stats(c, training, 'c_', '%d' % i + tag, B * yb.ld)
            instnorm_fwd(c, yb, out, mean, rstd, self.pad_mode, res_mode=(L.ZS_RES_IDENTITY if res else L.ZS_RES_NONE),
                         res=(a if res else None), p=dp, seed=seed, stream_id=20 + i, mask=masks[i])
            tp['blocks'].append((a, ya, yb, (mean, rstd, i), res))
            a = out
        logits = c.act('c_logits' + tag, B, 1, self.n_class, dtype=torch.float32)
        self.conv9.fwd(a, out=logits, out_f32=True)
        tp['last'] = a
        self.tape = tp
        return logits

    def backward(self, dlogits_f32, ld, need_dx=True, param_grads=True):
        c, ns, tp = self.ctx, self.ns, self.tape
        B, T = tp['B'], tp['T']
        tag = '_%d_%d_%d' % (self.uid, B, T)
        dl = c.act('c_dl' + tag, B, 1, self.n_class)
        cast_rows(c, L.ptr(dlogits_f32), ld, dl)
        if param_grads:
            self.conv9.wgrad(dl, tp['last'])
        da = c.act('c_da_last' + tag, B, T, self.conv9.Cin)
        self.conv9.dgrad(dl, T, da)
        for i in (3, 2, 1, 0):
            la, lb, _ = self.blocks[i]
            a, ya, yb, stt, res = tp['blocks'][i]
            mean, rstd, k = stt
            dzb = c.act('c_dzb%d' % i + tag, B, T, lb.Cout)
            instnorm_bwd(c, da, yb, mean, rstd, dzb, ns, p=tp['dp'], seed=tp['seed'], stream_id=20 + k, mask=tp['masks'][k])
            if param_grads:
                lb.wgrad(dzb, ya)
            gp = c.act('c_gp%d' % i + tag, B, T + lb.pad_l + lb.pad_r, lb.Cin)
            lb.dgrad(dzb, T, gp)
            dza = c.act('c_dza%d' % i + tag, B, T, la.Cout)
            grad_combine(c, gp, T, lb.pad_l, lb.pad_r, self.pad_mode, gp.ld, dza, ns, dact=ya)
            if param_grads:
                la.wgrad(dza, a)
            if i == 0 and not need_dx:
                return None
            gp2 = c.act('c_gq%d' % i + tag, B, T + la.pad_l + la.pad_r, la.Cin)
            la.dgrad(dza, T, gp2)
            dn = c.act('c_da%d' % i + tag, B, T, la.Cin)
            grad_combine(c, gp2, T, la.pad_l, la.pad_r, self.pad_mode, gp2.ld, dn, ns, res_mode=(L.ZS_RES_IDENTITY if res else L.ZS_RES_NONE),
                         res=(da if res else None))
            da = dn
        return da
```

zerospeech-tts-without-t_amd/layers.py:

```python
import ctypes
import os

import torch

from . import _lib as L


def colsum_ok(T):
    return T > 0 and 128 % T == 0


def rup(x, m):
    return (x + m - 1) // m * m


DTYPES = {'fp32': (L.ZS_F32, torch.float32), 'bf16': (L.ZS_BF16, torch.bfloat16)}
SLACK = 512
EPS_IN = 1e-5


class Act(object):
    __slots__ = ('t', 'B', 'T', 'C', 'ld', 'off', 'cols')

    def __init__(self, t, B, T, C, ld, off=0, cols=None):
        self.t, self.B, self.T, self.C, self.ld, self.off = t, B, T, C, ld, off
        self.cols = cols if cols is not None else ld

    @property
    def rows(self):
        return self.B * self.T

    def ptr(self, col=0):
        return self.t.data_ptr() + (self.off + col) * self.t.element_size()

    def sub(self, col, C, cols=None):
        return Act(self.t, self.B, self.T, C, self.ld, self.off + col, cols if cols is not None else C)

    def view2d(self):
        return self.t[self.off:self.off + self.rows * self.ld].view(self.rows, self.ld) if self.off == 0 else \
            self.t[self.off - (self.off % self.ld):][:self.rows * self.ld].view(self.rows, self.ld)

    def valid(self):
        base = self.t[self.off:self.off + (self.rows - 1) * self.ld + self.C]
        return torch.as_strided(base, (self.B, self.T, self.C), (self.T * self.ld, self.ld, 1))


_SIDE = {}
N_SIDE = max(1, int(os.environ.get('ZS_SIDE_STREAMS', '4')))
HW_QUEUES = int(os.environ.get('GPU_MAX_HW_QUEUES') or 4)
MULTI_STREAM = HW_QUEUES >= 4


def side_stream(device):
    key = (device.type, device.index)
    if key not in _SIDE:
        _SIDE[key] = {'streams': [torch.cuda.Stream(device) for _ in range(N_SIDE)], 'used': False, 'next': 0, 'ws': [None] * N_SIDE}
    return _SIDE[key]


def side_events(device):
    sd = side_stream(device)
    evs = []
    for st in sd['streams']:
        ev = torch.cuda.Event()
        ev.record(st)
        evs.append(ev)
    return evs


def fork_side(device):
    sd = side_stream(device)
    ev = torch.cuda.Event()
    ev.record(torch.cuda.current_stream(device))
    for st in sd['streams']:
        st.wait_event(ev)
    sd['used'] = True
    return sd['streams']


def join_side(device):
    sd = side_stream(device)
    if sd['used']:
        cur = torch.cuda.current_stream(device)
        for ev in side_events(device):
            cur.wait_event(ev)
        sd['used'] = False
    sd['next'] = 0


_OPT = {}


def opt_stream(device):
    key = (device.type, device.index)
    if key not in _OPT:
        _OPT[key] = torch.cuda.Stream(device)
    return _OPT[key]


_STATUS = {}


def device_status(device):
    device = torch.device(device)
    key = (device.type, device.index if device.index is not None else torch.cuda.current_device())
    if key not in _STATUS:
        _STATUS[key] = torch.zeros(4, dtype=torch.int32, device=device)
    return _STATUS[key]


def check_status(device):
    st = device_status(device)
    v = int(st[0].item())
    if v:
        st.zero_()
        raise L.ZsError('persistent GRU %s timed out waiting for its workgroup group: the results since the last check are '
                        'invalid (status 0x%x; is another process holding CUs of this GPU?)' %
                        (' and '.join(n for b, n in ((1, 'forward'), (2, 'BPTT')) if v & b), v))


_COPY = {}


def copy_stream(device):
    key = (device.type, device.index)
    if key not in _COPY:
        _COPY[key] = torch.cuda.Stream(device)
    return _COPY[key]


class Ctx(object):

    def __init__(self, device, dtype='fp32'):
        if dtype not in DTYPES:
            raise ValueError('dtype must be fp32 or bf16')
        self.device = torch.device(device)
        if self.device.type != 'cuda':
            raise L.ZsError('zs_amd runs on an MI355X only (device %s requested); there is no CPU path' % device)
        L.lib()
        self.dtype_name = dtype
        self.dt, self.tdt = DTYPES[dtype]
        self.es = 4 if dtype == 'fp32' else 2
        self.kc = 128 // self.es
        self._bufs = {}
        self._ws = None
        self.pin_wgrad_streams = False
        self.status = device_status(self.device)
        self.overlap_wgrad = os.environ.get('ZS_OVERLAP_WGRAD', '1' if MULTI_STREAM else '0') == '1'
        L.set_option('wgrad_alone', 0 if self.overlap_wgrad else 1)

    @property
    def stream(self):
        return torch.cuda.current_stream(self.device).cuda_stream

    def raw(self, name, n, dtype, zero=True):
        key = (name, n, dtype)
        t = self._bufs.get(key)
        if t is None:
            t = torch.zeros(n + SLACK, dtype=dtype, device=self.device)
            self._bufs[key] = t
        return t

    def act(self, name, B, T, C, ld=None, dtype=None):
        ld = ld if ld is not None else rup(C, 32)
        dtype = dtype if dtype is not None else self.tdt
        return Act(self.raw(name, B * T * ld, dtype), B, T, C, ld)

    def f32(self, name, n):
        return self.raw(name, n, torch.float32)

    def workspace(self, nbytes):
        if self._ws is None or self._ws.numel() < nbytes:
            if self._ws is not None:
                torch.cuda.synchronize(self.device)
            self._ws = torch.empty(int(nbytes * 1.25) + 1024, dtype=torch.uint8, device=self.device)
        return self._ws

    def release(self):
        self._bufs.clear()
        self._ws = None

    def check_status(self):
        check_status(self.device)


class ConvLayer(object):

    def __init__(self, ctx, weight, bias, gweight, gbias, stride=1, split2=False, pad_mode=L.ZS_PAD_REFLECT, name='', padded=True,
                 strides=None):
        self.ctx, self.name = ctx, name
        self.w, self.b, self.gw, self.gb = weight, bias, gweight, gbias
        self.Cout, self.Cin = weight.shape[0], weight.shape[1]
        self.k = weight.shape[2] if weight.dim() == 3 else 1
        self.stride, self.split2, self.pad_mode = stride, split2, pad_mode
        self.pad_l = self.k // 2 if padded else 0
        self.pad_r = (self.k - 1 - self.k // 2) if padded else 0
        self.so, self.si, self.sj = (self.Cin * self.k, self.k, 1) if weight.dim() == 3 else (self.Cin, 1, 0)
        if strides is not None:
            self.so, self.si, self.sj = strides
        kc = ctx.kc
        self.cin_pad, self.cout_pad = rup(self.Cin, kc), rup(self.Cout, kc)
        self.ldw, self.n_pad = self.k * self.cin_pad, rup(self.Cout, 128)
        self.ldw_d, self.n_pad_d = self.k * self.cout_pad, rup(self.Cin, 128)
        dev, tdt = ctx.device, ctx.tdt
        self.wf = torch.zeros(self.n_pad * self.ldw + SLACK, dtype=tdt, device=dev)
        self.wd = torch.zeros(self.n_pad_d * self.ldw_d + SLACK, dtype=tdt, device=dev)
        self.bias_p = torch.zeros(self.Cout, dtype=torch.float32, device=dev) if (split2 and bias is not None) else None
        self.sid = next_sid()
        self.parity = (stride == 2 and self.k > 1)

    @classmethod
    def from_params(cls, ctx, P, G, name, pad_mode, **kw):
        return cls(ctx, P[name + '.weight'], P[name + '.bias'], G[name + '.weight'], G[name + '.bias'], pad_mode=pad_mode, name=name, **kw)

    def pack(self):
        c = self.ctx
        common = dict(dtype=c.dt, W=L.ptr(self.w), so=self.so, si=self.si, sj=self.sj, Cout=self.Cout, Cin=self.Cin,
                      taps=self.k, co_split2=int(self.split2))
        L.call('zs_pack_weight', 'ZsPackWeight', c.stream, transpose=0, inner_pad=self.cin_pad, dst=L.ptr(self.wf),
               ldw=self.ldw, n_rows=self.n_pad, n_cols=self.ldw, **common)
        if self.parity:
            ne, no = (self.k + 1) // 2, self.k // 2
            ev = dict(common, taps=ne, sj=2 * self.sj)
            od = dict(common, taps=no, sj=2 * self.sj, W=L.ptr(self.w, self.sj))
            L.call('zs_pack_weight', 'ZsPackWeight', c.stream, transpose=1, inner_pad=self.cout_pad, dst=L.ptr(self.wd),
                   ldw=self.ldw_d, n_rows=self.n_pad_d, n_cols=ne * self.cout_pad, **ev)
            L.call('zs_pack_weight', 'ZsPackWeight', c.stream, transpose=1, inner_pad=self.cout_pad, dst=L.ptr(self.wd),
                   ldw=self.ldw_d, n_rows=self.n_pad_d, n_cols=no * self.cout_pad, col_offset=ne * self.cout_pad, **od)
        else:
            L.call('zs_pack_weight', 'ZsPackWeight', c.stream, transpose=1, inner_pad=self.cout_pad, dst=L.ptr(self.wd),
                   ldw=self.ldw_d, n_rows=self.n_pad_d, n_cols=self.ldw_d, **common)
        if self.bias_p is not None:
            h = self.Cout // 2
            L.vec_copy(self.bias_p[:h], self.b, c.stream, src_stride=2)
            L.vec_copy(self.bias_p[h:], self.b[1:], c.stream, src_stride=2)

    def bias_ptr(self):
        if self.b is None:
            return None
        return L.ptr(self.bias_p if self.bias_p is not None else self.b)

    def t_out(self, T_in):
        return (T_in + self.pad_l + self.pad_r - self.k) // self.stride + 1

    def fwd(self, A, out=None, act=L.ZS_ACT_NONE, slope=0.0, out_f32=False, out_cols=None, store_mode=L.ZS_STORE_ROWS,
            out2=None, vec2=None, idx=None, store_mode2=L.ZS_STORE_ROWS, out2_cols=None, pre_vec=None, bias=True, lengths=None):
        c = self.ctx
        T_out = self.t_out(A.T)
        kw = dict(dtype=c.dt, A=A.ptr(), lda=A.ld, a_batch_stride=A.T * A.ld, B=A.B, T_in=A.T, T_out=T_out, taps=self.k,
                  stride=self.stride, pad_left=self.pad_l, pad_mode=self.pad_mode, gather=0, cin_pad=self.cin_pad,
                  W=L.ptr(self.wf), ldw=self.ldw, N=self.Cout, n_pad=self.n_pad, bias=(self.bias_ptr() if bias else None), act=act,
                  slope=slope, groups=1)
        if pre_vec is not None:
            kw.update(pre_vec=L.ptr(pre_vec), pre_vec_ld=pre_vec.shape[1], vec_idx=L.ptr(idx))
        if lengths is not None and self.k > 1:
            kw.update(lengths=L.ptr(lengths), pad_right=self.pad_r)
        if out is not None:
            kw.update(out=out.ptr(), ldc=out.ld, out_f32=int(out_f32), store_mode=store_mode,
                      out_cols=out_cols if out_cols is not None else (min(out.cols, rup(self.Cout, 32)) if store_mode == L.ZS_STORE_ROWS else self.Cout // 2))
        if out2 is not None:
            kw.update(out2=out2.ptr(), ldc2=out2.ld, store_mode2=store_mode2,
                      out2_cols=out2_cols if out2_cols is not None else (min(out2.cols, rup(self.Cout, 32)) if store_mode2 == L.ZS_STORE_ROWS else self.Cout // 2))
            if vec2 is not None:
                kw.update(vec2=L.ptr(vec2), vec2_ld=vec2.shape[1], vec_idx=L.ptr(idx))
        L.call('zs_gemm_conv', 'ZsGemmConv', c.stream, **kw)
        return T_out

    def dgrad(self, dY, T_x, out, dact_src=None, slope=0.0, add_src=None, out_f32=False, add_f32=False, colsum=None, out_cols=None,
              n_cols=None, n_off=0, colsum_post=False):
        c = self.ctx
        Tp = T_x + self.pad_l + self.pad_r
        if self.parity:
            if dact_src is not None or add_src is not None or colsum is not None or n_cols is not None or n_off:
                raise ValueError('stride-2 dgrad: dact_src, add_src, colsum, n_cols and n_off are not supported')
            return self._dgrad_parity(dY, Tp, out, out_f32, out_cols)
        N, n_pad = self.Cin, self.n_pad_d
        if n_cols is not None and (n_cols < self.Cin or n_off):
            N = n_cols
            n_pad = rup(n_cols, 256) if n_off + rup(n_cols, 256) <= self.n_pad_d else rup(n_cols, 128)
            if n_off + n_pad > self.n_pad_d:
                raise ValueError('dgrad: channel block [%d, %d) does not fit the packed weight (%d rows)' % (n_off, n_off + n_cols, self.n_pad_d))
        kw = dict(dtype=c.dt, A=dY.ptr(), lda=dY.ld, a_batch_stride=dY.T * dY.ld, B=dY.B, T_in=dY.T, T_out=Tp, taps=self.k,
                  stride=self.stride, pad_left=0, pad_mode=L.ZS_PAD_ZERO, gather=1, cin_pad=self.cout_pad,
                  W=L.ptr(self.wd, n_off * self.ldw_d), ldw=self.ldw_d, N=N, n_pad=n_pad, act=L.ZS_ACT_NONE, slope=slope,
                  out=out.ptr(), ldc=out.ld, out_cols=(out_cols if out_cols is not None else min(out.cols, rup(N, 32))),
                  store_mode=L.ZS_STORE_ROWS, groups=1, out_f32=int(out_f32))
        if dact_src is not None:
            kw.update(dact_src=dact_src.ptr(), dact_ld=dact_src.ld)
        if add_src is not None:
            kw.update(add_src=add_src.ptr(), add_ld=add_src.ld, add_f32=int(add_f32))
        if colsum is not None:
            kw.update(colsum=colsum[0], colsum_ld=colsum[1], colsum_col0=colsum[2], colsum_post=int(colsum_post))
        L.call('zs_gemm_conv', 'ZsGemmConv', c.stream, **kw)
        return Tp

    def _dgrad_parity(self, dY, Tp, out, out_f32, out_cols):
        c = self.ctx
        Te = Tp + (Tp & 1)
        if out.T != Te:
            raise ValueError('stride-2 dgrad: the output needs %d rows per sample (padded domain %d rounded up to even), got %d' % (Te, Tp, out.T))
        ne = (self.k + 1) // 2
        for par, taps in ((0, ne), (1, self.k // 2)):
            kw = dict(dtype=c.dt, A=dY.ptr(), lda=dY.ld, a_batch_stride=dY.T * dY.ld, B=dY.B, T_in=dY.T, T_out=Te // 2, taps=taps,
                      stride=1, pad_left=0, pad_mode=L.ZS_PAD_ZERO, gather=1, cin_pad=self.cout_pad,
                      W=L.ptr(self.wd, par * ne * self.cout_pad), ldw=self.ldw_d, N=self.Cin, n_pad=self.n_pad_d, act=L.ZS_ACT_NONE,
                      out=out.ptr(par * out.ld), ldc=2 * out.ld, out_cols=(out_cols if out_cols is not None else min(out.cols, rup(self.Cin, 32))),
                      store_mode=L.ZS_STORE_ROWS, groups=1, out_f32=int(out_f32))
            L.call('zs_gemm_conv', 'ZsGemmConv', c.stream, **kw)
        return Tp

    def wgrad(self, dY, X, accumulate=False, bias=True):
        c = self.ctx
        es = c.es
        y_cols = min(dY.cols, rup(self.Cout, 16 // es))
        x_cols = min(X.cols, rup(self.Cin, 16 // es))
        kw = dict(dtype=c.dt, dY=dY.ptr(), ldy=dY.ld, y_cols=y_cols, X=X.ptr(), ldx=X.ld, x_batch_stride=X.T * X.ld,
                  x_cols=x_cols, B=X.B, T_in=X.T, T_out=dY.T, taps=self.k, stride=self.stride, pad_left=self.pad_l,
                  pad_mode=self.pad_mode, Cout=self.Cout, Cin=self.Cin, dW=L.ptr(self.gw), so=self.so, si=self.si, sj=self.sj,
                  db=(L.ptr(self.gb) if bias else None), co_split2=int(self.split2), accumulate=int(accumulate), splits=0)
        wgrad_call(c, kw, self.sid)


class Conv2dLayer(object):

    def __init__(self, ctx, weight, bias, gweight, gbias, stride=2, pad_mode=L.ZS_PAD_REFLECT, name='', dgrad_only=False):
        self.ctx, self.name = ctx, name
        self.w, self.b, self.gw, self.gb = weight, bias, gweight, gbias
        self.Cout, self.Cin, self.k = weight.shape[0], weight.shape[1], weight.shape[2]
        if weight.dim() != 4 or weight.shape[3] != self.k or stride not in (1, 2):
            raise ValueError('Conv2dLayer: square kernels, stride 1 or 2')
        self.stride, self.pad_mode, self.pad = stride, pad_mode, self.k // 2
        self.taps = self.k * self.k
        kc = ctx.kc
        self.cin_pad, self.cout_pad = rup(self.Cin, kc), rup(self.Cout, kc)
        self.ldw, self.n_pad, self.n_pad_d = self.taps * self.cin_pad, rup(self.Cout, 128), rup(self.Cin, 128)
        dev, tdt = ctx.device, ctx.tdt
        self.wf = None if dgrad_only else torch.zeros(self.n_pad * self.ldw + SLACK, dtype=tdt, device=dev)
        self.nt = [(self.k + 1) // 2, self.k // 2] if stride == 2 else [self.k]
        self.wd = {}
        for ph in range(len(self.nt)):
            for pw in range(len(self.nt)):
                ld = self.nt[ph] * self.nt[pw] * self.cout_pad
                self.wd[(ph, pw)] = (torch.zeros(self.n_pad_d * ld + SLACK, dtype=tdt, device=dev), ld)
        self.sid = next_sid()

    def out_hw(self, H, W):
        return (H + 2 * self.pad - self.k) // self.stride + 1, (W + 2 * self.pad - self.k) // self.stride + 1

    def pack(self):
        c, k = self.ctx, self.k
        common = dict(dtype=c.dt, so=self.Cin * self.taps, si=self.taps, Cout=self.Cout, Cin=self.Cin, co_split2=0)
        if self.wf is not None:
            L.call('zs_pack_weight', 'ZsPackWeight', c.stream, transpose=0, inner_pad=self.cin_pad, dst=L.ptr(self.wf), ldw=self.ldw,
                   n_rows=self.n_pad, n_cols=self.ldw, W=L.ptr(self.w), sj=1, taps=self.taps, **common)
        step = self.stride
        for (ph, pw), (buf, ld) in self.wd.items():
            nh, nw = self.nt[ph], self.nt[pw]
            for kwp in range(nw):
                L.call('zs_pack_weight', 'ZsPackWeight', c.stream, transpose=1, inner_pad=self.cout_pad, dst=L.ptr(buf), ldw=ld,
                       n_rows=self.n_pad_d, n_cols=nh * self.cout_pad, col_offset=kwp * nh * self.cout_pad,
                       W=L.ptr(self.w, (pw + step * kwp) * k + ph), sj=step, taps=nh, **common)

    def fwd(self, X, H, W, out, act=L.ZS_ACT_NONE, slope=0.0, bias=True, out_f32=False):
        c = self.ctx
        Ho, Wo = self.out_hw(H, W)
        if self.wf is None:
            raise ValueError('Conv2dLayer.fwd: built with dgrad_only')
        if X.T != H * W or out.T != Ho * Wo or X.B != out.B:
            raise ValueError('Conv2dLayer.fwd: rows %d x %d for an image of %d x %d, output %d x %d' % (X.B, X.T, H, W, out.B, out.T))
        L.call('zs_gemm_conv', 'ZsGemmConv', c.stream, dtype=c.dt, A=X.ptr(), lda=X.ld, a_batch_stride=X.T * X.ld, B=X.B, T_in=H * W,
               T_out=Ho * Wo, taps=self.taps, stride=self.stride, pad_left=self.pad, pad_mode=self.pad_mode, gather=0, cin_pad=self.cin_pad,
               W=L.ptr(self.wf), ldw=self.ldw, N=self.Cout, n_pad=self.n_pad, bias=(L.ptr(self.b) if (bias and self.b is not None) else None),
               act=act, slope=slope, groups=1, out=out.ptr(), ldc=out.ld, out_f32=int(out_f32), store_mode=L.ZS_STORE_ROWS,
               out_cols=min(out.cols, rup(self.Cout, 32)), w_in=W, w_out=Wo, taps_h=self.k)
        return Ho, Wo

    def wgrad(self, dY, X, H, W, accumulate=False, bias=True):
        c, es = self.ctx, self.ctx.es
        Ho, Wo = self.out_hw(H, W)
        kw = dict(dtype=c.dt, dY=dY.ptr(), ldy=dY.ld, y_cols=min(dY.cols, rup(self.Cout, 16 // es)), X=X.ptr(), ldx=X.ld,
                  x_batch_stride=X.T * X.ld, x_cols=min(X.cols, rup(self.Cin, 16 // es)), B=X.B, T_in=H * W, T_out=Ho * Wo, taps=self.taps,
                  stride=self.stride, pad_left=self.pad, pad_mode=self.pad_mode, Cout=self.Cout, Cin=self.Cin, dW=L.ptr(self.gw),
                  so=self.Cin * self.taps, si=self.taps, sj=1, db=(L.ptr(self.gb) if bias else None), co_split2=0,
                  accumulate=int(accumulate), splits=0, w_in=W, w_out=Wo, taps_h=self.k)
        wgrad_call(c, kw, self.sid)

    def padded_hw(self, H, W):
        Ho, Wo = self.out_hw(H, W)
        return (Ho - 1) * self.stride + self.k, (Wo - 1) * self.stride + self.k

    def dgrad(self, dY, H, W, out, name, add=None, fill_cols=None):
        c = self.ctx
        if self.stride != 2:
            raise ValueError('Conv2dLayer.dgrad: stride 2 only')
        Ho, Wo = self.out_hw(H, W)
        Hp, Wp = self.padded_hw(H, W)
        g = {}
        for (ph, pw), (buf, ld) in self.wd.items():
            Hc, Wc = (Hp - ph + 1) // 2, (Wp - pw + 1) // 2
            gq = c.act('%s_q%d%d' % (name, ph, pw), dY.B, Hc * Wc, self.Cin)
            L.call('zs_gemm_conv', 'ZsGemmConv', c.stream, dtype=c.dt, A=dY.ptr(), lda=dY.ld, a_batch_stride=dY.T * dY.ld, B=dY.B,
                   T_in=Ho * Wo, T_out=Hc * Wc, taps=self.nt[ph] * self.nt[pw], stride=1, pad_left=0, pad_mode=L.ZS_PAD_ZERO, gather=1,
                   cin_pad=self.cout_pad, W=L.ptr(buf), ldw=ld, N=self.Cin, n_pad=self.n_pad_d, act=L.ZS_ACT_NONE, out=gq.ptr(), ldc=gq.ld,
                   out_cols=min(gq.cols, rup(self.Cin, 32)), store_mode=L.ZS_STORE_ROWS, groups=1, out_f32=0, w_in=Wo, w_out=Wc,
                   taps_h=self.nt[ph])
            g[(ph, pw)] = gq
        g00 = g[(0, 0)]
        L.call('zs_conv2d_unpad', 'ZsConv2dUnpad', c.stream, dtype=c.dt, g00=g00.ptr(), g01=g[(0, 1)].ptr(), g10=g[(1, 0)].ptr(),
               g11=g[(1, 1)].ptr(), ldg=g00.ld, B=dY.B, H=H, W=W, C=rup(self.Cin, 8), Hp=Hp, Wp=Wp, pad=self.pad, pad_mode=self.pad_mode,
               add=(add.ptr() if add is not None else None), ldadd=(add.ld if add is not None else 0), out=out.ptr(), ldo=out.ld,
               fill_cols=(fill_cols if fill_cols is not None else out.ld))


_SID = [0]
_UID = [0]


def next_sid():
    _SID[0] += 1
    return _SID[0]


def next_uid():
    _UID[0] += 1
    return _UID[0]


def side_launch(ctx, sid, need):
    if not ctx.overlap_wgrad:
        return ctx.stream, ctx.workspace(need)
    sd = side_stream(ctx.device)
    if sid is not None and ctx.pin_wgrad_streams:
        i = sid % len(sd['streams'])
    else:
        i = sd['next']
        sd['next'] = (i + 1) % len(sd['streams'])
    ws = sd['ws'][i]
    if ws is None or ws.numel() < need:
        if any(w is not None for w in sd['ws']):
            torch.cuda.synchronize(ctx.device)
        size = int(need * 1.25) + 1024
        sd['ws'] = [torch.empty(size, dtype=torch.uint8, device=ctx.device) for _ in sd['streams']]
        ws = sd['ws'][i]
    ev = torch.cuda.Event()
    ev.record(torch.cuda.current_stream(ctx.device))
    sd['streams'][i].wait_event(ev)
    sd['used'] = True
    return sd['streams'][i].cuda_stream, ws


def wgrad_call(ctx, kw, sid=None):
    S = L.STRUCTS['ZsGemmWgrad']
    s = S()
    for k, v in kw.items():
        if v is not None:
            setattr(s, k, v)
    need = L.lib().zs_gemm_wgrad_workspace_bytes(ctypes.byref(s))
    stream, ws = side_launch(ctx, sid, need)
    s.workspace = ws.data_ptr()
    s.workspace_bytes = ws.numel()
    L.check(L.lib().zs_gemm_wgrad(ctypes.byref(s), ctypes.c_void_p(stream)), 'zs_gemm_wgrad')


def instnorm_fwd(ctx, x, out, mean, rstd, pad_mode, res_mode=L.ZS_RES_NONE, res=None, lengths=None, res_lengths=None, p=0.0,
                 seed=0, stream_id=0, mask=None, seed_ptr=None, out2=None, vec2=None, idx=None):
    L.call('zs_instnorm_fwd', 'ZsInstNormFwd', ctx.stream, dtype=ctx.dt, x=x.ptr(), ldx=x.ld, out=out.ptr(), ldo=out.ld,
           out2=(out2.ptr() if out2 is not None else None), ldo2=(out2.ld if out2 is not None else 0), vec2=L.ptr(vec2),
           vec2_ld=(vec2.shape[1] if vec2 is not None else 0), vec2_cols=(vec2.shape[1] if vec2 is not None else 0), idx=L.ptr(idx),
           mean=L.ptr(mean), rstd=L.ptr(rstd), B=x.B, T=x.T, C=x.ld, eps=EPS_IN, drop_p=p, seed=seed, stream_id=stream_id,
           mask=L.ptr(mask), mask_ld=(mask.shape[-1] if mask is not None else 0), res_mode=res_mode,
           res=(res.ptr() if res is not None else None), ldres=(res.ld if res is not None else 0), T_res=(res.T if res is not None else 0),
           res_pad_mode=pad_mode, seed_ptr=seed_ptr, lengths=L.ptr(lengths), res_lengths=L.ptr(res_lengths))


def instnorm_bwd(ctx, dout, x, mean, rstd, dz, slope, p=0.0, seed=0, stream_id=0, mask=None, seed_ptr=None):
    L.call('zs_instnorm_bwd', 'ZsInstNormBwd', ctx.stream, dtype=ctx.dt, dout=dout.ptr(), ldd=dout.ld, x=x.ptr(), ldx=x.ld,
           mean=L.ptr(mean), rstd=L.ptr(rstd), dz=dz.ptr(), ldz=dz.ld, B=x.B, T=x.T, C=x.ld, drop_p=p, seed=seed, stream_id=stream_id,
           mask=L.ptr(mask), mask_ld=(mask.shape[-1] if mask is not None else 0), slope=slope, seed_ptr=seed_ptr)


def grad_combine(ctx, gp, T, pad_l, pad_r, pad_mode, C, out, slope, res_mode=L.ZS_RES_NONE, res=None, dact=None, emb_sum=None,
                 unshuffle=0):
    L.call('zs_grad_combine', 'ZsGradCombine', ctx.stream, dtype=ctx.dt, gp=gp.ptr(), ldg=gp.ld, pad_left=pad_l, pad_right=pad_r,
           pad_mode=pad_mode, B=gp.B, T=T, C=C, emb_sum=emb_sum, emb_ld=(C if emb_sum is not None else 0),
           emb_cols=(C if emb_sum is not None else 0), res_mode=res_mode, res=(res.ptr() if res is not None else None),
           ldres=(res.ld if res is not None else 0), dact_src=(dact.ptr() if dact is not None else None),
           dact_ld=(dact.ld if dact is not None else 0), slope=slope, out=(out.ptr() if out is not None else None),
           ldo=(out.ld if out is not None else 0), unshuffle=unshuffle)


def cast_rows(ctx, src, ld_src, dst, dst_f32=False, dst2=None, col_off2=0, act2=L.ZS_ACT_NONE, slope2=0.0):
    L.call('zs_cast_rows', 'ZsCastRows', ctx.stream, dtype=ctx.dt, src=src, ld_src=ld_src, src_f32=1, dst=dst.ptr(), ld_dst=dst.ld,
           dst_f32=int(dst_f32), col_off=0, rows=dst.rows, cols=dst.C, fill_cols=dst.ld, act=L.ZS_ACT_NONE,
           dst2=(dst2.ptr() if dst2 is not None else None), ld_dst2=(dst2.ld if dst2 is not None else 0), col_off2=col_off2,
           fill_cols2=(dst2.ld - col_off2 if dst2 is not None else 0), act2=act2, slope2=slope2)


class GruLayer(object):

    def __init__(self, ctx, P, G, prefix, name=''):
        self.ctx, self.name = ctx, name
        sfx = ['', '_reverse']
        self.w_ih = [P[prefix + 'weight_ih_l0' + s] for s in sfx]
        self.w_hh = [P[prefix + 'weight_hh_l0' + s] for s in sfx]
        self.b_ih = [P[prefix + 'bias_ih_l0' + s] for s in sfx]
        self.b_hh = [P[prefix + 'bias_hh_l0' + s] for s in sfx]
        self.gw_ih = [G[prefix + 'weight_ih_l0' + s] for s in sfx]
        self.gw_hh = [G[prefix + 'weight_hh_l0' + s] for s in sfx]
        self.gb_ih = [G[prefix + 'bias_ih_l0' + s] for s in sfx]
        self.gb_hh = [G[prefix + 'bias_hh_l0' + s] for s in sfx]
        self.H = self.w_hh[0].shape[1]
        self.Cin = self.w_ih[0].shape[1]
        self.sids = [next_sid() for _ in range(4)]
        H, Cin = self.H, self.Cin
        if H % 8:
            raise ValueError('GRU hidden size must be a multiple of 8 (got %d)' % H)
        dev, tdt = ctx.device, ctx.tdt
        self.G6 = 6 * H
        self.g6_pad = rup(6 * H, ctx.kc)
        kc = ctx.kc
        self.cin_pad = rup(Cin, kc)
        self.ih_ldw, self.ih_npad = self.cin_pad, rup(6 * H, 128)
        self.wih_f = torch.zeros(self.ih_npad * self.ih_ldw + SLACK, dtype=tdt, device=dev)
        self.ih_ldw_d, self.ih_npad_d = self.g6_pad, rup(Cin, 128)
        self.wih_d = torch.zeros(self.ih_npad_d * self.ih_ldw_d + SLACK, dtype=tdt, device=dev)
        self.bih = torch.zeros(6 * H, dtype=torch.float32, device=dev)
        self.hh_ldw, self.hh_npad = rup(H, kc), rup(3 * H, 128)
        self.whh_f = torch.zeros(2 * self.hh_npad * self.hh_ldw + SLACK, dtype=tdt, device=dev)
        self.hh_ldw_t, self.hh_npad_t = rup(3 * H, kc), rup(H, 128)
        self.whh_t = torch.zeros(2 * self.hh_npad_t * self.hh_ldw_t + SLACK, dtype=tdt, device=dev)
        self.bhh = torch.zeros(2 * 3 * H, dtype=torch.float32, device=dev)
        self.fast = (H % 32 == 0)
        self.perm = None
        if self.fast:
            n = torch.arange(3 * H)
            hc, rem = n // 96, n % 96
            self.perm = ((rem // 32) * H + hc * 32 + (rem % 32)).to(torch.int32).to(dev)

    def pack(self):
        c, H, Cin = self.ctx, self.H, self.Cin
        for d in range(2):
            com = dict(dtype=c.dt, so=Cin, si=1, sj=0, Cout=3 * H, Cin=Cin, taps=1, co_split2=0, W=L.ptr(self.w_ih[d]))
            L.call('zs_pack_weight', 'ZsPackWeight', c.stream, transpose=0, inner_pad=self.cin_pad, dst=L.ptr(self.wih_f),
                   ldw=self.ih_ldw, n_rows=3 * H, n_cols=self.ih_ldw, row_offset=3 * H * d, **com)
            L.call('zs_pack_weight', 'ZsPackWeight', c.stream, transpose=1, inner_pad=3 * H, dst=L.ptr(self.wih_d),
                   ldw=self.ih_ldw_d, n_rows=self.ih_npad_d, n_cols=3 * H, col_offset=3 * H * d, **com)
            com = dict(dtype=c.dt, so=H, si=1, sj=0, Cout=3 * H, Cin=H, taps=1, co_split2=0, W=L.ptr(self.w_hh[d]))
            L.call('zs_pack_weight', 'ZsPackWeight', c.stream, transpose=0, inner_pad=rup(H, c.kc),
                   dst=L.ptr(self.whh_f, d * self.hh_npad * self.hh_ldw), ldw=self.hh_ldw,
                   n_rows=(3 * H if self.fast else self.hh_npad), n_cols=self.hh_ldw, row_perm=L.ptr(self.perm), **com)
            L.call('zs_pack_weight', 'ZsPackWeight', c.stream, transpose=1, inner_pad=rup(3 * H, c.kc),
                   dst=L.ptr(self.whh_t, d * self.hh_npad_t * self.hh_ldw_t), ldw=self.hh_ldw_t, n_rows=self.hh_npad_t,
                   n_cols=self.hh_ldw_t, **com)
            L.vec_copy(self.bih[3 * H * d:3 * H * (d + 1)], self.b_ih[d], c.stream)
            L.vec_copy(self.bhh[3 * H * d:3 * H * (d + 1)], self.b_hh[d], c.stream)

    def _work(self, B):
        n = L.lib().zs_gru_work_bytes(B, self.H)
        return self.ctx.f32('gru_work_%s' % self.name, (n + 3) // 4)

    def fwd(self, X, out, out_col, gi, gates, bcast=None, lengths=None):
        c, H = self.ctx, self.H
        if lengths is not None and gates is not None:
            raise L.ZsError('GruLayer.fwd: ragged batches are an inference feature (no tape)')
        L.call('zs_gemm_conv', 'ZsGemmConv', c.stream, dtype=c.dt, A=X.ptr(), lda=X.ld, a_batch_stride=X.T * X.ld, B=X.B,
               T_in=X.T, T_out=X.T, taps=1, stride=1, pad_left=0, pad_mode=L.ZS_PAD_ZERO, gather=0, cin_pad=self.cin_pad,
               W=L.ptr(self.wih_f), ldw=self.ih_ldw, N=6 * H, n_pad=self.ih_npad, bias=L.ptr(self.bih), act=L.ZS_ACT_NONE,
               out=gi.ptr(), ldc=gi.ld, out_cols=min(gi.cols, rup(6 * H, 32)), groups=1)
        if lengths is not None:
            L.call('zs_rows_reverse', 'ZsRowsReverse', c.stream, dtype=c.dt, x=gi.ptr(), ld=gi.ld, col0=3 * H, cols=3 * H, B=X.B, T=X.T,
                   lengths=L.ptr(lengths))
        work = self._work(X.B)
        L.call('zs_gru_fwd', 'ZsGruFwd', c.stream, dtype=c.dt, B=X.B, T=X.T, H=H, gi=gi.ptr(), ldgi=gi.ld,
               whh=L.ptr(self.whh_f), ldw=self.hh_ldw, n_pad=self.hh_npad, w_gstride=self.hh_npad * self.hh_ldw,
               bhh=L.ptr(self.bhh), bhh_gstride=3 * H, out=out.ptr(), ldo=out.ld, out_col=out_col,
               gates=L.ptr(gates) if gates is not None else None, work=L.ptr(work), work_bytes=work.numel() * 4,
               whh_interleaved=int(self.fast), status=L.ptr(c.status),
               bcast_vec=(L.ptr(bcast[0]) if bcast else None), bcast_ld=(bcast[0].shape[1] if bcast else 0),
               bcast_idx=(L.ptr(bcast[1]) if bcast else None), bcast_col=(bcast[2] if bcast else 0),
               dir1_forward=int(lengths is not None))
        if lengths is not None:
            L.call('zs_rows_reverse', 'ZsRowsReverse', c.stream, dtype=c.dt, x=out.ptr(), ld=out.ld, col0=out_col + H, cols=H, B=X.B, T=X.T,
                   lengths=L.ptr(lengths))

    def check(self, B):
        L.check(L.lib().zs_gru_check(L.ptr(self._work(B)), B, self.H, self.ctx.stream), 'zs_gru_check')

    def bwd(self, dout, dout_col, out, out_col, gates, X, dgi, dgh, dX, add_src=None, colsum=None, param_grads=True):
        c, H = self.ctx, self.H
        B, T = X.B, X.T
        work = self._work(B)
        L.call('zs_gru_bwd', 'ZsGruBwd', c.stream, dtype=c.dt, B=B, T=T, H=H, dout=dout.ptr(), ldd=dout.ld, dout_col=dout_col,
               out=out.ptr(), ldo=out.ld, out_col=out_col, gates=L.ptr(gates), whh_t=L.ptr(self.whh_t), ldw=self.hh_ldw_t,
               n_pad=self.hh_npad_t, w_gstride=self.hh_npad_t * self.hh_ldw_t, dgi=dgi.ptr(), ldgi=dgi.ld, dgh=dgh.ptr(),
               ldgh=dgh.ld, work=L.ptr(work), work_bytes=work.numel() * 4, status=L.ptr(c.status))
        for d in (range(2) if param_grads else ()):
            wgrad_call(c, dict(dtype=c.dt, dY=dgh.ptr(3 * H * d), ldy=dgh.ld, y_cols=3 * H, X=out.ptr(out_col + d * H),
                               ldx=out.ld, x_batch_stride=T * out.ld, x_cols=H, B=B, T_in=T, T_out=T, taps=1, stride=1,
                               pad_left=(1 if d == 0 else -1), pad_mode=L.ZS_PAD_ZERO, Cout=3 * H, Cin=H,
                               dW=L.ptr(self.gw_hh[d]), so=H, si=1, sj=0, db=L.ptr(self.gb_hh[d]), co_split2=0,
                               accumulate=0, splits=0), self.sids[2 * d])
            wgrad_call(c, dict(dtype=c.dt, dY=dgi.ptr(3 * H * d), ldy=dgi.ld, y_cols=3 * H, X=X.ptr(), ldx=X.ld,
                               x_batch_stride=T * X.ld, x_cols=min(X.cols, rup(self.Cin, 16 // c.es)), B=B, T_in=T, T_out=T,
                               taps=1, stride=1, pad_left=0, pad_mode=L.ZS_PAD_ZERO, Cout=3 * H, Cin=self.Cin,
                               dW=L.ptr(self.gw_ih[d]), so=self.Cin, si=1, sj=0, db=L.ptr(self.gb_ih[d]), co_split2=0,
                               accumulate=0, splits=0), self.sids[2 * d + 1])
        kw = dict(dtype=c.dt, A=dgi.ptr(), lda=dgi.ld, a_batch_stride=T * dgi.ld, B=B, T_in=T, T_out=T, taps=1, stride=1,
                  pad_left=0, pad_mode=L.ZS_PAD_ZERO, gather=0, cin_pad=self.g6_pad, W=L.ptr(self.wih_d), ldw=self.ih_ldw_d,
                  N=self.Cin, n_pad=self.ih_npad_d, act=L.ZS_ACT_NONE, out=dX.ptr(), ldc=dX.ld,
                  out_cols=min(dX.cols, rup(self.Cin, 32)), groups=1)
        if add_src is not None:
            kw.update(add_src=add_src.ptr(), add_ld=add_src.ld, add_f32=0)
        if colsum is not None:
            kw.update(colsum=colsum[0], colsum_ld=colsum[1], colsum_col0=colsum[2])
        L.call('zs_gemm_conv', 'ZsGemmConv', c.stream, **kw)
```

zerospeech-tts-without-t_amd/model.py:

```python
import os

import torch
import torch.nn as nn

from . import _lib as L
from .engine import ClassifierEngine, DecoderEngine, EncoderEngine, PatcherEngine, linear_width
from .layers import Act, Ctx, cast_rows, rup


def default_dtype():
    return os.environ.get('ZS_DTYPE', 'fp32')


class ZsModule(nn.Module):

    def __init__(self, dtype=None):
        super(ZsModule, self).__init__()
        self._zs_dtype = dtype or default_dtype()
        self._zs = {'flat': None, 'gflat': None, 'engine': None, 'ctx': None, 'version': None, 'offsets': None}

    def _flatten(self):
        params = list(self.named_parameters())
        if not params:
            return
        dev = params[0][1].device
        offs, n = {}, 0
        for name, p in params:
            offs[name] = n
            n += rup(p.numel(), 4)
        flat = torch.zeros(n, dtype=torch.float32, device=dev)
        gflat = torch.zeros(n, dtype=torch.float32, device=dev)
        for name, p in params:
            o = offs[name]
            flat[o:o + p.numel()].copy_(p.data.reshape(-1).float())
            p.data = flat[o:o + p.numel()].view(p.shape)
            p.grad = gflat[o:o + p.numel()].view(p.shape)
        self._zs.update(flat=flat, gflat=gflat, offsets=offs, engine=None, ctx=None, version=None)

    def _apply(self, fn, *a, **kw):
        out = super(ZsModule, self)._apply(fn, *a, **kw)
        self._flatten()
        return out

    def flat_params(self):
        if self._zs['flat'] is None:
            self._flatten()
        return self._zs['flat'], self._zs['gflat']

    def grad_view(self, name):
        o = self._zs['offsets'][name]
        p = dict(self.named_parameters())[name]
        return self._zs['gflat'][o:o + p.numel()].view(p.shape)

    def flat_range(self, first, last):
        if self._zs['flat'] is None:
            self._flatten()
        offs = self._zs['offsets']
        p = dict(self.named_parameters())[last]
        lo, hi = offs[first], offs[last] + rup(p.numel(), 4)
        if lo >= hi:
            raise ValueError('flat_range: %s does not precede %s' % (first, last))
        return lo, hi

    def mark_dirty(self):
        self._zs['version'] = None

    def repack(self):
        z = self._zs
        if z['engine'] is None:
            self._engine()
        else:
            z['engine'].pack()
            z['version'] = sum(p._version for p in self.parameters())

    def set_compute_dtype(self, dtype):
        if dtype != self._zs_dtype:
            self._zs_dtype = dtype
            self._zs.update(engine=None, ctx=None, version=None)

    def _engine(self):
        z = self._zs
        if z['flat'] is None:
            self._flatten()
        if z['engine'] is None:
            dev = z['flat'].device
            if dev.type != 'cuda':
                raise L.ZsError('zs_amd modules compute on an MI355X only: move the module to a cuda device '
                                '(there is no CPU fallback path)')
            z['ctx'] = Ctx(dev, self._zs_dtype)
            P = {k: p.data for k, p in self.named_parameters()}
            G = {k: self.grad_view(k) for k, _ in self.named_parameters()}
            z['engine'] = self._make_engine(z['ctx'], P, G)
            z['version'] = None
        ver = sum(p._version for p in self.parameters())
        if z['version'] != ver:
            z['engine'].pack()
            z['version'] = ver
        return z['engine']

    def load_state_dict(self, *a, **kw):
        out = super(ZsModule, self).load_state_dict(*a, **kw)
        self.mark_dirty()
        return out


ENC_MODES = ('multilabel_binary', 'one_hot', 'binary', 'continues')


class Encoder(ZsModule):

    def __init__(self, c_in=513, c_h1=128, c_h2=512, c_h3=128, ns=0.2, dp=0.5, enc_size=512, seg_len=64,
                 enc_mode='continues', dtype=None):
        super(Encoder, self).__init__(dtype)
        self.ns, self.dp, self.enc_size, self.seg_len, self.enc_mode = ns, dp, enc_size, seg_len, enc_mode
        self.c_in, self.c_h1, self.c_h2, self.c_h3 = c_in, c_h1, c_h2, c_h3
        if enc_mode not in ENC_MODES:
            if enc_mode == 'gumbel_t':
                raise NotImplementedError("enc_mode 'gumbel_t' (softmax over time) is not built: use one of %s" % ', '.join(ENC_MODES))
            raise NotImplementedError('Invalid encoding mode!')
        if enc_mode in ('one_hot', 'continues'):
            assert enc_size % 2 == 0
        if enc_mode == 'binary' and enc_size > 64:
            raise ValueError("enc_mode 'binary' supports enc_size <= 64 (its linear layer has enc_size^2 = %d outputs)" % enc_size ** 2)
        if enc_mode == 'one_hot' and enc_size > 1024:
            raise ValueError("enc_mode 'one_hot' supports enc_size <= 1024 (got %d)" % enc_size)
        self.n_lin = linear_width(enc_mode, enc_size)
        self.conv1s = nn.ModuleList([nn.Conv1d(c_in, c_h1, kernel_size=k) for k in range(1, 8)])
        self.conv2 = nn.Conv1d(len(self.conv1s) * c_h1 + c_in, c_h2, kernel_size=1)
        self.conv3 = nn.Conv1d(c_h2, c_h2, kernel_size=5)
        self.conv4 = nn.Conv1d(c_h2, c_h2, kernel_size=5, stride=2)
        self.conv5 = nn.Conv1d(c_h2, c_h2, kernel_size=5)
        self.conv6 = nn.Conv1d(c_h2, c_h2, kernel_size=5, stride=2)
        self.conv7 = nn.Conv1d(c_h2, c_h2, kernel_size=5)
        self.conv8 = nn.Conv1d(c_h2, c_h2, kernel_size=5, stride=2)
        self.dense1 = nn.Linear(c_h2, c_h2)
        self.dense2 = nn.Linear(c_h2, c_h2)
        self.dense3 = nn.Linear(c_h2, c_h2)
        self.dense4 = nn.Linear(c_h2, c_h2)
        self.RNN = nn.GRU(input_size=c_h2, hidden_size=c_h3, num_layers=1, bidirectional=True)
        self.linear = nn.Linear(c_h2 + 2 * c_h3, self.n_lin)

    def _make_engine(self, ctx, P, G):
        return EncoderEngine(ctx, P, G, self.c_in, self.c_h1, self.c_h2, self.c_h3, self.enc_size, self.ns, self.dp, self.seg_len,
                             enc_mode=self.enc_mode)

    def noise_shape(self, B, T4):
        E = self.enc_size
        return {'multilabel_binary': (B, T4, E, 2), 'one_hot': (B, T4, E), 'binary': (B, T4, E, E)}.get(self.enc_mode)

    def check_noise(self, x, U=None, G=None):
        noise = G if G is not None else U
        if noise is None or self.enc_mode == 'multilabel_binary':
            return
        B, T = x.shape[0], x.shape[2]
        want = self.noise_shape(B, (((T + 1) // 2 + 1) // 2 + 1) // 2)
        if want is None:
            raise ValueError("enc_mode %r draws no noise: U / G must be None" % self.enc_mode)
        if tuple(noise.shape) != want:
            raise ValueError('enc_mode %r: %s must have shape %s, got %s' % (self.enc_mode, 'G' if G is not None else 'U', want,
                                                                             tuple(noise.shape)))

    def forward(self, x, U=None, G=None, drop_masks=None, seed=None, lengths=None):
        self.check_noise(x, U=U, G=G)
        eng = self._engine()
        xb = x.detach().permute(0, 2, 1).contiguous().float()
        noise, kind = None, 2
        if G is not None:
            noise, kind = G.to(xb.device, torch.float32).contiguous(), 0
        elif U is not None:
            noise, kind = U.to(xb.device, torch.float32).contiguous(), 1
        if seed is None:
            seed = int(torch.randint(0, 2 ** 62, (1,)).item())
        masks = None
        if drop_masks is not None:
            masks = [m.to(xb.device, torch.uint8).contiguous() if m is not None else None for m in drop_masks]
        bits, bits_f32, logits = eng.forward(xb, self.training, noise=noise, noise_kind=kind, seed=seed, drop_masks=masks, lengths=lengths)
        self._last_bits = bits
        enc_act = bits_f32.permute(0, 2, 1).clone()
        enc = logits.valid().permute(0, 2, 1).clone()
        return enc_act, enc


class Decoder(ZsModule):

    def __init__(self, c_in=512, c_out=513, c_h=512, c_a=8, ns=0.2, seg_len=64, output_mask=False, dtype=None):
        super(Decoder, self).__init__(dtype)
        self.output_mask, self.ns, self.seg_len = output_mask, ns, seg_len
        self.c_in, self.c_out, self.c_h, self.c_a = c_in, c_out, c_h, c_a
        self.conv1 = nn.Conv1d(c_h, 2 * c_h, kernel_size=3)
        self.conv2 = nn.Conv1d(c_h, c_h, kernel_size=3)
        self.conv3 = nn.Conv1d(c_h, 2 * c_h, kernel_size=3)
        self.conv4 = nn.Conv1d(c_h, c_h, kernel_size=3)
        self.conv5 = nn.Conv1d(c_h, 2 * c_h, kernel_size=3)
        self.conv6 = nn.Conv1d(c_h, c_h, kernel_size=3)
        self.dense1 = nn.Linear(c_h, c_h)
        self.dense2 = nn.Linear(c_h, c_h)
        self.dense3 = nn.Linear(c_h, c_h)
        self.dense4 = nn.Linear(c_h, c_h)
        self.RNN = nn.GRU(input_size=c_h, hidden_size=c_h // 2, num_layers=1, bidirectional=True)
        self.dense5 = nn.Linear(2 * c_h + c_h, c_h)
        self.linear = nn.Linear(c_h, c_out)
        self.input_emb = nn.Linear(c_in, c_h)
        self.emb1 = nn.Embedding(c_a, c_h)
        self.emb2 = nn.Embedding(c_a, c_h)
        self.emb3 = nn.Embedding(c_a, c_h)
        self.emb4 = nn.Embedding(c_a, c_h)
        self.emb5 = nn.Embedding(c_a, c_h)

    def _make_engine(self, ctx, P, G):
        return DecoderEngine(ctx, P, G, self.c_in, self.c_out, self.c_h, self.c_a, self.ns, self.seg_len, self.output_mask)

    def emb_grad_views(self):
        return [self.grad_view('emb%d.weight' % i) for i in range(1, 6)]

    def forward(self, x, c, lengths=None):
        _, xdec = self.forward_rows(x, c, lengths=lengths)
        return xdec.valid().permute(0, 2, 1).clone()

    def forward_rows(self, x, c, lengths=None):
        eng = self._engine()
        ctx = eng.ctx
        xb = x.detach().permute(0, 2, 1).contiguous().float()
        B, T0, E = xb.shape
        bits = ctx.act('d_in_%d_%d_%d' % (eng.uid, B, T0), B, T0, E)
        cast_rows(ctx, L.ptr(xb), E, bits)
        cidx = c.detach().to(xb.device, torch.int64).contiguous()
        return bits, eng.forward(bits, cidx, self.training, lengths=lengths)


class Spectrogram_Patcher(ZsModule):

    def __init__(self, c_in=512, c_out=513, c_h=512, c_a=8, ns=0.2, seg_len=64, dtype=None):
        super(Spectrogram_Patcher, self).__init__(dtype)
        self.ns, self.seg_len = ns, seg_len
        self.c_in, self.c_out, self.c_h, self.c_a = c_in, c_out, c_h, c_a
        self.input_layer = nn.Linear(c_in, c_h)
        self.dense1 = nn.Linear(c_h, c_h)
        self.dense2 = nn.Linear(c_h, c_h)
        self.dense3 = nn.Linear(c_h, c_h)
        self.dense4 = nn.Linear(c_h, c_h)
        self.RNN = nn.GRU(input_size=c_h, hidden_size=c_h // 2, num_layers=1, bidirectional=True)
        self.dense5 = nn.Linear(2 * c_h + c_h, c_h)
        self.linear = nn.Linear(c_h, c_out)
        self.emb1 = nn.Embedding(c_a, c_h)
        self.emb2 = nn.Embedding(c_a, c_h)

    def _make_engine(self, ctx, P, G):
        return PatcherEngine(ctx, P, G, self.c_in, self.c_out, self.c_h, self.c_a, self.ns)

    def forward(self, x, c, lengths=None):
        eng = self._engine()
        ctx = eng.ctx
        xb = x.detach().permute(0, 2, 1).contiguous().float()
        B, T, F = xb.shape
        if F != self.c_in:
            raise ValueError('Spectrogram_Patcher expects %d channels (got %d)' % (self.c_in, F))
        xa = Act(xb.reshape(-1), B, T, F, F)
        cidx = c.detach().to(xb.device, torch.int64).contiguous()
        out = eng.forward(xa, cidx, self.training, lengths=lengths)
        return out.valid().permute(0, 2, 1).clone()


class SpeakerClassifier(ZsModule):

    def __init__(self, c_in=512, c_h=512, n_class=8, dp=0.1, ns=0.01, seg_len=128, dtype=None):
        super(SpeakerClassifier, self).__init__(dtype)
        self.dp, self.ns, self.seg_len = dp, ns, seg_len
        self.c_in, self.c_h, self.n_class = c_in, c_h, n_class
        self.conv1 = nn.Conv1d(c_in, c_h, kernel_size=5)
        self.conv2 = nn.Conv1d(c_h, c_h, kernel_size=5)
        self.conv3 = nn.Conv1d(c_h, c_h, kernel_size=5)
        self.conv4 = nn.Conv1d(c_h, c_h, kernel_size=5)
        self.conv5 = nn.Conv1d(c_h, c_h, kernel_size=5)
        self.conv6 = nn.Conv1d(c_h, c_h, kernel_size=5)
        self.conv7 = nn.Conv1d(c_h, c_h // 2, kernel_size=3)
        self.conv8 = nn.Conv1d(c_h // 2, c_h // 4, kernel_size=3)
        if seg_len == 128:
            self.conv9 = nn.Conv1d(c_h // 4, n_class, kernel_size=16)
        elif seg_len == 64:
            self.conv9 = nn.Conv1d(c_h // 4, n_class, kernel_size=8)
        elif seg_len == 32:
            self.conv9 = nn.Conv1d(c_h // 4, n_class, kernel_size=4)
        else:
            raise NotImplementedError('Segement length {} is not supported!'.format(seg_len))

    def _make_engine(self, ctx, P, G):
        return ClassifierEngine(ctx, P, G, self.c_in, self.c_h, self.n_class, self.dp, self.ns, self.seg_len)

    def input_act(self, x_btc_f32):
        eng = self._engine()
        ctx = eng.ctx
        B, T, C = x_btc_f32.shape
        a = ctx.act('c_in_%d_%d_%d' % (eng.uid, B, T), B, T, C)
        cast_rows(ctx, L.ptr(x_btc_f32), x_btc_f32.stride(1), a)
        return a

    def forward(self, x, drop_masks=None, seed=None):
        eng = self._engine()
        xb = x.detach().permute(0, 2, 1).contiguous().float()
        if seed is None:
            seed = int(torch.randint(0, 2 ** 62, (1,)).item())
        masks = None
        if drop_masks is not None:
            masks = [m.to(xb.device, torch.uint8).contiguous() if m is not None else None for m in drop_masks]
        logits = eng.forward(self.input_act(xb), self.training, seed=seed, drop_masks=masks)
        return logits.valid()[:, 0, :].clone()
```

zerospeech-tts-without-t_amd/optim.py:

```python
import torch

from . import _lib as L
from . import parallel


class NetOpt(object):

    def __init__(self, net, lr, betas=(0.5, 0.9), max_norm=0.0, reduce=True):
        self.net, self.lr, self.betas, self.max_norm, self.t = net, float(lr), betas, max_norm, 0
        flat, _ = net.flat_params()
        self.m, self.v = torch.zeros_like(flat), torch.zeros_like(flat)
        self.sq = torch.zeros(1, dtype=torch.float32, device=flat.device)
        self.part = torch.zeros(1024, dtype=torch.float64, device=flat.device)
        self.reducer = parallel.GradReducer() if reduce else None

    def state_dict(self):
        return {'m': self.m, 'v': self.v, 't': int(self.t)}

    def load_state_dict(self, sd):
        for k in ('m', 'v'):
            if tuple(sd[k].shape) != tuple(self.m.shape):
                raise ValueError('optimizer state: %s has %d elements, the net has %d' % (k, sd[k].numel(), self.m.numel()))
        self.m.copy_(sd['m'])
        self.v.copy_(sd['v'])
        self.t = int(sd['t'])
        self.net.mark_dirty()

    def sqnorm(self):
        _, gflat = self.net.flat_params()
        st = torch.cuda.current_stream(gflat.device).cuda_stream
        L.check(L.lib().zs_sqnorm(L.ptr(gflat), gflat.numel(), L.ptr(self.part), L.ptr(self.sq), st), 'zs_sqnorm')
        return self.sq

    def _adam(self, bc1, bc2, max_norm, step_ptr=None):
        flat, gflat = self.net.flat_params()
        b1, b2 = self.betas
        L.call('zs_adam_clip', 'ZsAdam', torch.cuda.current_stream(flat.device).cuda_stream, p=L.ptr(flat), g=L.ptr(gflat),
               m=L.ptr(self.m), v=L.ptr(self.v), n=flat.numel(), lr=self.lr, beta1=b1, beta2=b2, eps=1e-8, bc1=bc1, bc2=bc2,
               sumsq=L.ptr(self.sq), max_norm=float(max_norm) if max_norm else 0.0, write_clipped_grad=0, step_ptr=step_ptr,
               grad_scale=1.0 / parallel.world_size())

    def adam(self, t, max_norm=None):
        b1, b2 = self.betas
        self._adam(1.0 - b1 ** t, 1.0 - b2 ** t, self.max_norm if max_norm is None else max_norm)
        self.net.mark_dirty()

    def step(self, max_norm=None):
        if self.reducer is not None and parallel.world_size() > 1:
            self.reducer.start(self.net.flat_params()[1])
            self.reducer.finish()
        self.sqnorm()
        self.t += 1
        self.adam(self.t, max_norm)

    def device_step(self, step_ptr):
        self.sqnorm()
        self._adam(1.0, 1.0, self.max_norm, step_ptr=step_ptr)
        self.net.repack()


def softmax_ce(ctx, logits, target, loss, correct, grad_scale=1.0):
    B, n = logits.shape
    dl = ctx.f32('ce_dlogits_%d_%d' % (B, n), B * n)[:B * n].view(B, n)
    L.call('zs_softmax_ce', 'ZsSoftmaxCE', ctx.stream, logits=L.ptr(logits), ld=logits.stride(0), target=L.ptr(target), B=B,
           n_class=n, loss_out=L.ptr(loss), dlogits=L.ptr(dl), ldg=n, grad_scale=float(grad_scale), correct_out=L.ptr(correct))
    return dl
```

Baseline: 3.111 million frames/s.

## Fuse Adam update with weight repacking and sqnorm finalize into one kernel

Adds an adam_pack kernel that applies the clipped Adam update tile by tile and writes the new weights straight into the packed GEMM operand layouts (with transpose, parity and row permutation) through LDS. It also folds the second sqnorm reduction stage into that kernel. This replaces the separate sqnorm stage-2, adam and repack launches, and saves a full re-read of the parameters for packing. In exchange it adds a host-built job plan, a binary search per tile, and a fallback repack for operands the plan cannot cover.

```diff
diff --git a/include/zs_amd.h b/include/zs_amd.h
--- a/include/zs_amd.h
+++ b/include/zs_amd.h
@@ -19,6 +19,7 @@
 int zs_abi_version(void);
 const char* zs_last_error(void);
 int zs_set_option(const char* key, int value);
+int zs_get_option(const char* key);
 
 typedef struct {
   int32_t dtype;
@@ -251,6 +252,26 @@
 } ZsAdam;
 int zs_adam_clip(const ZsAdam* p, void* stream);
 
+int zs_sqnorm_stage1(const float* g, int64_t n, double* partial, void* stream);
+
+enum { ZS_APJ_WEIGHT = 0, ZS_APJ_VECTOR = 1, ZS_APJ_RANGE = 2 };
+typedef struct {
+  void* dst; int64_t ldw; int64_t dst_elems;
+  int32_t transpose, inner_pad, row_offset, col_offset, parity;
+  int32_t vlen, src_offset, src_stride;
+  const int32_t* row_inv;
+} ZsAdamPackView;
+typedef struct {
+  int32_t kind, dtype;
+  int64_t off, len;
+  int32_t Cout, Cin, taps, co_split2;
+  int32_t n_views, tile_start;
+  ZsAdamPackView view[2];
+} ZsAdamPackJob;
+int zs_adam_pack_tiles(const ZsAdamPackJob* job);
+int zs_adam_pack(const ZsAdam* a, const ZsAdamPackJob* jobs, const ZsAdamPackJob* jobs_dev, int32_t n, const double* sq_partial,
+                 int32_t n_partial, void* stream);
+
 int zs_host_fetch(const void* src, void* dst, size_t bytes, int32_t workgroups, void* stream);
 
 typedef struct {
diff --git a/zerospeech-tts-without-t_amd/_lib.py b/zerospeech-tts-without-t_amd/_lib.py
--- a/zerospeech-tts-without-t_amd/_lib.py
+++ b/zerospeech-tts-without-t_amd/_lib.py
@@ -18,9 +18,13 @@
     return re.sub(r'/\*.*?\*/', ' ', text, flags=re.S)
 
 
+def _make_struct(name, fields):
+    return type(name, (ctypes.Structure,), {'_fields_': fields})
+
+
 def parse_header(path=HEADER):
     text = _strip_comments(open(path).read())
-    structs = {}
+    structs, classes = {}, {}
     for body, name in re.findall(r'typedef\s+struct\s*\{(.*?)\}\s*(\w+)\s*;', text, flags=re.S):
         fields = []
         for decl in body.split(';'):
@@ -34,8 +38,13 @@
                 item = item.strip()
                 ptr = item.startswith('*')
                 fname = item.lstrip('* ').strip()
-                fields.append((fname, ctypes.c_void_p if ptr else _CTYPES[base]))
+                ct = ctypes.c_void_p if ptr else (_CTYPES.get(base) or classes[base])
+                arr = re.match(r'(\w+)\s*\[(\d+)\]$', fname)
+                if arr:
+                    fname, ct = arr.group(1), ct * int(arr.group(2))
+                fields.append((fname, ct))
         structs[name] = fields
+        classes[name] = _make_struct(name, fields)
     funcs = re.findall(r'^\s*(?:const\s+)?(?:int|size_t|char\s*\*|const char\s*\*)\s*\*?\s*(zs_\w+)\s*\(', text, flags=re.M)
     enums = {k: int(v) for k, v in re.findall(r'#define\s+(ZS_\w+)\s+(\d+)', text)}
     for body in re.findall(r'enum\s*\{(.*?)\}', text, flags=re.S):
@@ -57,12 +66,12 @@
 _STRUCT_FIELDS, FUNCTIONS, ENUMS = parse_header()
 globals().update(ENUMS)
 
-
-def _make_struct(name, fields):
-    return type(name, (ctypes.Structure,), {'_fields_': fields})
-
-
 STRUCTS = {name: _make_struct(name, fields) for name, fields in _STRUCT_FIELDS.items()}
+for _fields in _STRUCT_FIELDS.values():
+    for _, _ct in _fields:
+        _el = getattr(_ct, '_type_', None)
+        if isinstance(_el, type) and issubclass(_el, ctypes.Structure):
+            STRUCTS[_el.__name__] = _el
 
 _lib = None
 
@@ -85,6 +94,11 @@
         L.zs_gru_work_bytes.argtypes = [ctypes.c_int32, ctypes.c_int32]
         L.zs_gru_check.argtypes = [ctypes.c_void_p, ctypes.c_int32, ctypes.c_int32, ctypes.c_void_p]
         L.zs_sqnorm.argtypes = [ctypes.c_void_p, ctypes.c_int64, ctypes.c_void_p, ctypes.c_void_p, ctypes.c_void_p]
+        L.zs_sqnorm_stage1.argtypes = [ctypes.c_void_p, ctypes.c_int64, ctypes.c_void_p, ctypes.c_void_p]
+        L.zs_adam_pack_tiles.argtypes = [ctypes.c_void_p]
+        L.zs_adam_pack.argtypes = [ctypes.c_void_p, ctypes.c_void_p, ctypes.c_void_p, ctypes.c_int32, ctypes.c_void_p, ctypes.c_int32,
+                                   ctypes.c_void_p]
+        L.zs_get_option.argtypes = [ctypes.c_char_p]
         L.zs_step_counters.argtypes = [ctypes.c_void_p, ctypes.c_void_p, ctypes.c_void_p]
         L.zs_set_option.argtypes = [ctypes.c_char_p, ctypes.c_int]
         L.zs_pre_mel.argtypes = [ctypes.c_void_p, ctypes.c_void_p, ctypes.c_void_p, ctypes.c_int64, ctypes.c_int32, ctypes.c_float,
@@ -129,6 +143,13 @@
     return rc
 
 
+def get_option(key):
+    rc = lib().zs_get_option(key.encode())
+    if rc < 0:
+        check(rc, 'zs_get_option')
+    return rc
+
+
 def last_error():
     return lib().zs_last_error().decode('utf-8', 'replace')
 
diff --git a/zerospeech-tts-without-t_amd/csrc/zs_api.hip b/zerospeech-tts-without-t_amd/csrc/zs_api.hip
--- a/zerospeech-tts-without-t_amd/csrc/zs_api.hip
+++ b/zerospeech-tts-without-t_amd/csrc/zs_api.hip
@@ -20,6 +20,13 @@
   return ZS_EINVAL;
 }
 
+extern "C" int zs_get_option(const char* key) {
+  for (Knob* k = g_knobs; key && k; k = k->next)
+    if (!strcmp(k->key, key)) return k->get();
+  zs_set_error("zs_get_option: unknown key %s", key ? key : "(null)");
+  return ZS_EINVAL;
+}
+
 int zs_check_launch(const char* what) {
   hipError_t e = hipGetLastError();
   if (e != hipSuccess) {
diff --git a/zerospeech-tts-without-t_amd/csrc/zs_elem.hip b/zerospeech-tts-without-t_amd/csrc/zs_elem.hip
--- a/zerospeech-tts-without-t_amd/csrc/zs_elem.hip
+++ b/zerospeech-tts-without-t_amd/csrc/zs_elem.hip
@@ -354,11 +354,12 @@
   if (threadIdx.x == 0) *out = (float)(red[0] + red[1] + red[2] + red[3]);
 }
 
-__global__ void adam_kernel(const ZsAdam p) {
+struct AdamCoef { float coef, step_size, bc2_sqrt, beta1, beta2, eps; };
+__device__ __forceinline__ AdamCoef adam_coef(const ZsAdam& p, const float* sumsq) {
   const float gs = p.grad_scale != 0.f ? p.grad_scale : 1.f;
   float coef = gs;
-  if (p.max_norm > 0.f && p.sumsq) {
-    const float norm = sqrtf(*p.sumsq) * gs;
+  if (p.max_norm > 0.f && sumsq) {
+    const float norm = sqrtf(*sumsq) * gs;
     coef = gs * fminf(p.max_norm / (norm + 1e-6f), 1.f);
   }
   float bc1 = p.bc1, bc2 = p.bc2;
@@ -367,30 +368,187 @@
     bc1 = 1.f - powf(p.beta1, t);
     bc2 = 1.f - powf(p.beta2, t);
   }
-  const float step_size = p.lr / bc1;
-  const float bc2_sqrt = sqrtf(bc2);
-  auto upd = [&](float& w, float& g, float& m, float& v) {
-    g *= coef;
-    m = m + (g - m) * (1.f - p.beta1);
-    v = v * p.beta2 + g * g * (1.f - p.beta2);
-    const float denom = sqrtf(v) / bc2_sqrt + p.eps;
-    w = w - step_size * (m / denom);
-  };
+  return AdamCoef{coef, p.lr / bc1, sqrtf(bc2), p.beta1, p.beta2, p.eps};
+}
+__device__ __forceinline__ void adam_upd(const AdamCoef& c, float& w, float& g, float& m, float& v) {
+#pragma clang fp contract(off)
+  const float d = __builtin_fmaf(g, c.coef, -m);
+  g = g * c.coef;
+  m = __builtin_fmaf(d, 1.f - c.beta1, m);
+  v = __builtin_fmaf(g * g, 1.f - c.beta2, v * c.beta2);
+  const float denom = sqrtf(v) / c.bc2_sqrt + c.eps;
+  w = __builtin_fmaf(-c.step_size, m / denom, w);
+}
+__device__ __forceinline__ void adam_upd4(const ZsAdam& p, const AdamCoef& c, int64_t i, float4& w) {
+  float4 g = reinterpret_cast<float4*>(p.g)[i], m = reinterpret_cast<float4*>(p.m)[i], v = reinterpret_cast<float4*>(p.v)[i];
+  w = reinterpret_cast<float4*>(p.p)[i];
+  adam_upd(c, w.x, g.x, m.x, v.x); adam_upd(c, w.y, g.y, m.y, v.y); adam_upd(c, w.z, g.z, m.z, v.z); adam_upd(c, w.w, g.w, m.w, v.w);
+  reinterpret_cast<float4*>(p.p)[i] = w; reinterpret_cast<float4*>(p.m)[i] = m; reinterpret_cast<float4*>(p.v)[i] = v;
+  if (p.write_clipped_grad) reinterpret_cast<float4*>(p.g)[i] = g;
+}
+__device__ __forceinline__ float adam_upd1(const ZsAdam& p, const AdamCoef& c, int64_t i) {
+  float w = p.p[i], g = p.g[i], m = p.m[i], v = p.v[i];
+  adam_upd(c, w, g, m, v);
+  p.p[i] = w; p.m[i] = m; p.v[i] = v;
+  if (p.write_clipped_grad) p.g[i] = g;
+  return w;
+}
+__device__ __forceinline__ bool adam_aligned16(const ZsAdam& p) {
+  return ((((uintptr_t)p.p) | ((uintptr_t)p.g) | ((uintptr_t)p.m) | ((uintptr_t)p.v)) & 15) == 0;
+}
+
+__global__ void adam_kernel(const ZsAdam p) {
+  const AdamCoef c = adam_coef(p, p.sumsq);
   const int64_t tid = (int64_t)blockIdx.x * blockDim.x + threadIdx.x, nthr = (int64_t)gridDim.x * blockDim.x;
-  const bool vec = ((((uintptr_t)p.p) | ((uintptr_t)p.g) | ((uintptr_t)p.m) | ((uintptr_t)p.v)) & 15) == 0;
-  const int64_t n4 = vec ? p.n / 4 : 0;
+  const int64_t n4 = adam_aligned16(p) ? p.n / 4 : 0;
   for (int64_t i = tid; i < n4; i += nthr) {
-    float4 w = reinterpret_cast<float4*>(p.p)[i], g = reinterpret_cast<float4*>(p.g)[i];
-    float4 m = reinterpret_cast<float4*>(p.m)[i], v = reinterpret_cast<float4*>(p.v)[i];
-    upd(w.x, g.x, m.x, v.x); upd(w.y, g.y, m.y, v.y); upd(w.z, g.z, m.z, v.z); upd(w.w, g.w, m.w, v.w);
-    reinterpret_cast<float4*>(p.p)[i] = w; reinterpret_cast<float4*>(p.m)[i] = m; reinterpret_cast<float4*>(p.v)[i] = v;
-    if (p.write_clipped_grad) reinterpret_cast<float4*>(p.g)[i] = g;
-  }
-  for (int64_t i = 4 * n4 + tid; i < p.n; i += nthr) {
-    float w = p.p[i], g = p.g[i], m = p.m[i], v = p.v[i];
-    upd(w, g, m, v);
-    p.p[i] = w; p.m[i] = m; p.v[i] = v;
-    if (p.write_clipped_grad) p.g[i] = g;
+    float4 w;
+    adam_upd4(p, c, i, w);
+  }
+  for (int64_t i = 4 * n4 + tid; i < p.n; i += nthr) adam_upd1(p, c, i);
+}
+
+constexpr int AP_THREADS = 256, AP_MAX_JOBS = 256, AP_RANGE_TILE = 4096, AP_VEC_TILE = 1024;
+template <typename T, int TAPS> struct ApTile {
+  static constexpr int CB = TAPS == 1 ? 64 : 32;
+  static constexpr int IB = TAPS == 1 ? 64 : (sizeof(T) == 2 ? 32 : 16);
+  static constexpr int RUN = IB * TAPS;
+  static constexpr int PITCH = RUN + (sizeof(T) == 2 ? 2 : 1);
+  static_assert((size_t)CB * PITCH * sizeof(T) <= PK_LDS_BYTES, "adam_pack tile exceeds the pack kernels' LDS");
+};
+__host__ __device__ inline int ap_cb(int taps) { return taps == 1 ? 64 : 32; }
+__host__ __device__ inline int ap_ib(int taps, int dtype) { return taps == 1 ? 64 : (dtype == ZS_BF16 ? 32 : 16); }
+inline int64_t ap_tiles(const ZsAdamPackJob& j) {
+  if (j.kind == ZS_APJ_WEIGHT) {
+    const int cb = ap_cb(j.taps), ib = ap_ib(j.taps, j.dtype);
+    return (int64_t)((j.Cout + cb - 1) / cb) * ((j.Cin + ib - 1) / ib);
+  }
+  const int t = j.kind == ZS_APJ_VECTOR ? AP_VEC_TILE : AP_RANGE_TILE;
+  return (j.len + t - 1) / t;
+}
+
+template <typename T, int TAPS>
+__device__ __forceinline__ void ap_weight_tile(const ZsAdam& a, const AdamCoef& c, const ZsAdamPackJob& job, int tile, T* lds) {
+  using G = ApTile<T, TAPS>;
+  constexpr int CB = G::CB, IB = G::IB, RUN = G::RUN, PITCH = G::PITCH;
+  const int tid = threadIdx.x;
+  const int tiles_i = (job.Cin + IB - 1) / IB;
+  const int tn = tile / tiles_i, ti = tile - tn * tiles_i;
+  const int n0 = tn * CB, i0 = ti * IB;
+  const int half = job.Cout >> 1, split2 = job.co_split2;
+  const int rows = min(CB, job.Cout - n0), cis = min(IB, job.Cin - i0), runw = cis * TAPS;
+  const int64_t row_len = (int64_t)job.Cin * TAPS;
+  const int64_t base = job.off + (int64_t)i0 * TAPS;
+  auto co_of = [&](int n) { return split2 ? (n < half ? 2 * n : 2 * (n - half) + 1) : n; };
+  if (adam_aligned16(a) && ((row_len | job.off) & 3) == 0) {
+    constexpr int R4 = RUN / 4;
+    for (int e = tid; e < CB * R4; e += AP_THREADS) {
+      const int rl = e / R4, x = (e - rl * R4) * 4;
+      if (rl < rows && x < runw) {
+        float4 w;
+        adam_upd4(a, c, (base + (int64_t)co_of(n0 + rl) * row_len + x) >> 2, w);
+        T* d = lds + rl * PITCH + x;
+        Elem<T>::st(d, w.x); Elem<T>::st(d + 1, w.y); Elem<T>::st(d + 2, w.z); Elem<T>::st(d + 3, w.w);
+      }
+    }
+  } else {
+    for (int e = tid; e < CB * RUN; e += AP_THREADS) {
+      const int rl = e / RUN, x = e - rl * RUN;
+      if (rl < rows && x < runw) Elem<T>::st(lds + rl * PITCH + x, adam_upd1(a, c, base + (int64_t)co_of(n0 + rl) * row_len + x));
+    }
+  }
+  __syncthreads();
+  for (int vi = 0; vi < job.n_views; ++vi) {
+    const ZsAdamPackView& v = job.view[vi];
+    T* const dst = (T*)v.dst + v.col_offset;
+    const int ne = (TAPS + 1) / 2;
+    if (v.transpose == 0) {
+#pragma unroll 4
+      for (int e = tid; e < CB * TAPS * IB; e += AP_THREADS) {
+        const int il = e % IB, t2 = e / IB;
+        const int tap = t2 % TAPS, rl = t2 / TAPS;
+        if (rl < rows && il < cis) {
+          const int n = n0 + rl;
+          const int row = v.row_inv ? v.row_inv[co_of(n)] : n;
+          const int slot = v.parity ? ((tap & 1) ? ne + (tap >> 1) : (tap >> 1)) : tap;
+          dst[(int64_t)(row + v.row_offset) * v.ldw + slot * v.inner_pad + i0 + il] = lds[rl * PITCH + il * TAPS + tap];
+        }
+      }
+    } else {
+#pragma unroll 4
+      for (int e = tid; e < IB * TAPS * CB; e += AP_THREADS) {
+        const int nl = e % CB, t2 = e / CB;
+        const int tap = t2 % TAPS, il = t2 / TAPS;
+        if (nl < rows && il < cis) {
+          const int slot = v.parity ? ((tap & 1) ? ne + (tap >> 1) : (tap >> 1)) : tap;
+          dst[(int64_t)(i0 + il + v.row_offset) * v.ldw + slot * v.inner_pad + n0 + nl] = lds[nl * PITCH + il * TAPS + tap];
+        }
+      }
+    }
+  }
+}
+
+__device__ __forceinline__ void ap_range_tile(const ZsAdam& a, const AdamCoef& c, const ZsAdamPackJob& job, int tile) {
+  const int64_t lo = job.off + (int64_t)tile * AP_RANGE_TILE;
+  const int cnt = (int)min((int64_t)AP_RANGE_TILE, job.off + job.len - lo);
+  const int n4 = (adam_aligned16(a) && (lo & 3) == 0) ? cnt / 4 : 0;
+  for (int i = threadIdx.x; i < n4; i += AP_THREADS) {
+    float4 w;
+    adam_upd4(a, c, (lo >> 2) + i, w);
+  }
+  for (int i = 4 * n4 + threadIdx.x; i < cnt; i += AP_THREADS) adam_upd1(a, c, lo + i);
+}
+
+__device__ __forceinline__ void ap_vector_tile(const ZsAdam& a, const AdamCoef& c, const ZsAdamPackJob& job, int tile) {
+  const int lo = tile * AP_VEC_TILE;
+  const int hi = (int)min((int64_t)lo + AP_VEC_TILE, job.len);
+  for (int e = lo + threadIdx.x; e < hi; e += AP_THREADS) {
+    const float w = adam_upd1(a, c, job.off + e);
+    for (int vi = 0; vi < job.n_views; ++vi) {
+      const ZsAdamPackView& v = job.view[vi];
+      const int r = e - v.src_offset;
+      if (r >= 0 && r % v.src_stride == 0 && r / v.src_stride < v.vlen) ((float*)v.dst)[(int64_t)(r / v.src_stride) * v.ldw] = w;
+    }
+  }
+}
+
+template <typename T>
+__global__ __launch_bounds__(AP_THREADS) void adam_pack_kernel(const ZsAdam a, const ZsAdamPackJob* __restrict__ jobs, int n_jobs, int total,
+                                                                const double* __restrict__ part, int n_part) {
+  __shared__ int s_start[AP_MAX_JOBS + 1];
+  __shared__ double s_red[4];
+  __shared__ float s_sq;
+  __shared__ __align__(16) unsigned char s_tile[PK_LDS_BYTES];
+  const int tid = threadIdx.x;
+  for (int i = tid; i <= n_jobs; i += AP_THREADS) s_start[i] = i < n_jobs ? jobs[i].tile_start : total;
+  if (part) {
+    double s = 0.0;
+    for (int i = tid; i < n_part; i += AP_THREADS) s += part[i];
+    s = wave_sum_d(s);
+    if ((tid & 63) == 0) s_red[tid >> 6] = s;
+    __syncthreads();
+    if (tid == 0) {
+      s_sq = (float)(s_red[0] + s_red[1] + s_red[2] + s_red[3]);
+      if (blockIdx.x == 0 && a.sumsq) *const_cast<float*>(a.sumsq) = s_sq;
+    }
+  }
+  __syncthreads();
+  const AdamCoef c = adam_coef(a, part ? &s_sq : a.sumsq);
+  for (int g = blockIdx.x; g < total; g += gridDim.x) {
+    int lo = 0, hi = n_jobs;
+    while (hi - lo > 1) { const int mid = (lo + hi) >> 1; if (s_start[mid] <= g) lo = mid; else hi = mid; }
+    lo = __builtin_amdgcn_readfirstlane(lo);
+    const ZsAdamPackJob& job = jobs[lo];
+    const int tile = g - s_start[lo];
+    if (job.kind == ZS_APJ_RANGE) ap_range_tile(a, c, job, tile);
+    else if (job.kind == ZS_APJ_VECTOR) ap_vector_tile(a, c, job, tile);
+    else {
+      T* lds = reinterpret_cast<T*>(s_tile);
+#define ZS_AP_CASE(K) case K: ap_weight_tile<T, K>(a, c, job, tile, lds); break;
+      switch (job.taps) { ZS_AP_CASE(1) ZS_AP_CASE(2) ZS_AP_CASE(3) ZS_AP_CASE(4) ZS_AP_CASE(5) ZS_AP_CASE(6) ZS_AP_CASE(7) default: break; }
+#undef ZS_AP_CASE
+    }
+    __syncthreads();
   }
 }
 
@@ -621,13 +779,19 @@
   return zs_check_launch("zs_l1_loss.stage2");
 }
 
-extern "C" int zs_sqnorm(const float* g, int64_t n, double* partial, float* out_sq, void* stream) {
-  ZS_REQUIRE(g && partial && out_sq && n > 0, "zs_sqnorm: bad args");
+extern "C" int zs_sqnorm_stage1(const float* g, int64_t n, double* partial, void* stream) {
+  ZS_REQUIRE(g && partial && n > 0, "zs_sqnorm: bad args");
   const unsigned nb = nblocks(n, 1024);
   hipLaunchKernelGGL(sqnorm_stage1_kernel, dim3(nb), dim3(NTE), 0, (hipStream_t)stream, g, n, partial);
   int rc = zs_check_launch("zs_sqnorm.stage1");
-  if (rc) return rc;
-  hipLaunchKernelGGL(sqnorm_stage2_kernel, dim3(1), dim3(256), 0, (hipStream_t)stream, (const double*)partial, (int)nb, out_sq);
+  return rc ? rc : (int)nb;
+}
+
+extern "C" int zs_sqnorm(const float* g, int64_t n, double* partial, float* out_sq, void* stream) {
+  ZS_REQUIRE(out_sq, "zs_sqnorm: bad args");
+  const int nb = zs_sqnorm_stage1(g, n, partial, stream);
+  if (nb < 0) return nb;
+  hipLaunchKernelGGL(sqnorm_stage2_kernel, dim3(1), dim3(256), 0, (hipStream_t)stream, (const double*)partial, nb, out_sq);
   return zs_check_launch("zs_sqnorm.stage2");
 }
 
@@ -640,6 +804,74 @@
   return zs_check_launch("zs_adam_clip");
 }
 
+Knob g_adam_pack("adam_pack", "ZS_ADAM_PACK", 1);
+
+static int adam_pack_check(const ZsAdam* a, const ZsAdamPackJob& j, int i) {
+  ZS_REQUIRE(j.off >= 0 && j.len > 0 && j.off + j.len <= a->n, "zs_adam_pack: job %d covers [%lld, +%lld) of %lld elements", i,
+             (long long)j.off, (long long)j.len, (long long)a->n);
+  ZS_REQUIRE(j.n_views >= 0 && j.n_views <= 2, "zs_adam_pack: job %d has %d views", i, j.n_views);
+  if (j.kind == ZS_APJ_RANGE) return ZS_OK;
+  if (j.kind == ZS_APJ_VECTOR) {
+    ZS_REQUIRE(j.len < (1ll << 30), "zs_adam_pack: vector job %d too long", i);
+    for (int k = 0; k < j.n_views; ++k) {
+      const ZsAdamPackView& v = j.view[k];
+      ZS_REQUIRE(v.dst && v.vlen > 0 && v.src_stride > 0 && v.src_offset >= 0 && v.ldw > 0 &&
+                     v.src_offset + (int64_t)(v.vlen - 1) * v.src_stride < j.len && (int64_t)(v.vlen - 1) * v.ldw < v.dst_elems,
+                 "zs_adam_pack: vector job %d, copy %d out of range", i, k);
+    }
+    return ZS_OK;
+  }
+  ZS_REQUIRE(j.kind == ZS_APJ_WEIGHT, "zs_adam_pack: job %d: bad kind %d", i, j.kind);
+  ZS_REQUIRE(j.Cout > 0 && j.Cin > 0 && j.taps >= 1 && j.taps <= PK_MAX_TAPS && (int64_t)j.Cout * j.Cin * j.taps == j.len,
+             "zs_adam_pack: weight job %d: %d x %d x %d taps over %lld elements", i, j.Cout, j.Cin, j.taps, (long long)j.len);
+  ZS_REQUIRE(!j.co_split2 || j.Cout % 2 == 0, "zs_adam_pack: SPLIT2 needs even Cout");
+  for (int k = 0; k < j.n_views; ++k) {
+    const ZsAdamPackView& v = j.view[k];
+    const int inner = v.transpose ? j.Cout : j.Cin, rows = v.transpose ? j.Cin : j.Cout;
+    ZS_REQUIRE(v.dst && v.inner_pad >= inner && v.row_offset >= 0 && v.col_offset >= 0 &&
+                   v.ldw >= (int64_t)v.col_offset + (int64_t)j.taps * v.inner_pad &&
+                   (int64_t)(rows + v.row_offset) * v.ldw <= v.dst_elems,
+               "zs_adam_pack: weight job %d, view %d: %d rows x %d taps x inner %d do not fit (ldw %lld, %lld elements)", i, k,
+               rows + v.row_offset, j.taps, v.inner_pad, (long long)v.ldw, (long long)v.dst_elems);
+    ZS_REQUIRE(!v.row_inv || (!v.transpose && !j.co_split2), "zs_adam_pack: row_inv goes with a transpose-0 view without SPLIT2");
+  }
+  return ZS_OK;
+}
+
+extern "C" int zs_adam_pack_tiles(const ZsAdamPackJob* job) {
+  ZS_REQUIRE(job && job->len > 0 && (job->kind != ZS_APJ_WEIGHT || (job->Cout > 0 && job->Cin > 0 && job->taps >= 1)),
+             "zs_adam_pack_tiles: bad job");
+  const int64_t t = ap_tiles(*job);
+  ZS_REQUIRE(t < (1ll << 30), "zs_adam_pack_tiles: too many tiles");
+  return (int)t;
+}
+
+extern "C" int zs_adam_pack(const ZsAdam* a, const ZsAdamPackJob* jobs, const ZsAdamPackJob* jobs_dev, int32_t n, const double* sq_partial,
+                            int32_t n_partial, void* stream) {
+  ZS_REQUIRE(a && a->p && a->g && a->m && a->v && a->n > 0, "zs_adam_pack: bad args");
+  ZS_REQUIRE(a->step_ptr || (a->bc1 > 0.f && a->bc2 > 0.f), "zs_adam_pack: bias corrections");
+  ZS_REQUIRE(jobs && jobs_dev && n > 0 && n <= AP_MAX_JOBS, "zs_adam_pack: 1..%d jobs", AP_MAX_JOBS);
+  ZS_REQUIRE(!sq_partial || (n_partial > 0 && n_partial <= 1024 && a->sumsq), "zs_adam_pack: 1..1024 partials and sumsq");
+  int64_t total = 0, end = 0;
+  for (int i = 0; i < n; ++i) {
+    const ZsAdamPackJob& j = jobs[i];
+    ZS_REQUIRE(j.dtype == jobs[0].dtype && (j.dtype == ZS_F32 || j.dtype == ZS_BF16), "zs_adam_pack: dtype of job %d", i);
+    int rc = adam_pack_check(a, j, i);
+    if (rc) return rc;
+    ZS_REQUIRE(j.off >= end, "zs_adam_pack: job %d overlaps its predecessor", i);
+    end = j.off + j.len;
+    ZS_REQUIRE(j.tile_start == total, "zs_adam_pack: job %d: tile_start %d, expected %lld", i, j.tile_start, (long long)total);
+    total += ap_tiles(j);
+    ZS_REQUIRE(total < (1ll << 30), "zs_adam_pack: too many tiles");
+  }
+  const unsigned gx = (unsigned)((a->max_blocks > 0 && total > a->max_blocks) ? a->max_blocks : total);
+  if (jobs[0].dtype == ZS_F32)
+    hipLaunchKernelGGL(adam_pack_kernel<float>, dim3(gx), dim3(AP_THREADS), 0, (hipStream_t)stream, *a, jobs_dev, (int)n, (int)total, sq_partial, (int)n_partial);
+  else
+    hipLaunchKernelGGL(adam_pack_kernel<bf16_t>, dim3(gx), dim3(AP_THREADS), 0, (hipStream_t)stream, *a, jobs_dev, (int)n, (int)total, sq_partial, (int)n_partial);
+  return zs_check_launch("zs_adam_pack");
+}
+
 extern "C" int zs_host_fetch(const void* src, void* dst, size_t bytes, int32_t workgroups, void* stream) {
   ZS_REQUIRE(src && dst && bytes > 0 && bytes % 16 == 0 && (((uintptr_t)src) & 15) == 0 && (((uintptr_t)dst) & 15) == 0, "zs_host_fetch: bad args (16-byte granularity)");
   const int wg = workgroups > 0 ? workgroups : 32;
diff --git a/zerospeech-tts-without-t_amd/engine.py b/zerospeech-tts-without-t_amd/engine.py
--- a/zerospeech-tts-without-t_amd/engine.py
+++ b/zerospeech-tts-without-t_amd/engine.py
@@ -4,7 +4,7 @@
 
 from . import _lib as L
 from .layers import (Act, ConvLayer, GruLayer, cast_rows, colsum_ok, fork_side, grad_combine, instnorm_bwd, instnorm_fwd, join_side,
-                     next_uid, rup)
+                     next_uid, pack_operands, rup, weight_operand)
 
 LRELU = L.ZS_ACT_LRELU
 
@@ -33,6 +33,15 @@
 
 def linear_width(enc_mode, E):
     return {'multilabel_binary': 2 * E, 'binary': E * E}.get(enc_mode, E)
+
+
+def operands_of(layers):
+    w, v = [], []
+    for l in layers:
+        lw, lv = l.operands()
+        w += lw
+        v += lv
+    return w, v
 
 
 class EncoderEngine(object):
@@ -59,14 +68,17 @@
         self.tape = None
         self.tapes = {}
         self.bank_d = None
+        self.adam_plan = None
+
+    def operands(self):
+        w, v = operands_of(self.layers + [self.gru])
+        if self.bank_d is not None:
+            w += self._bank_d_operands()
+        return w, v
 
     def pack(self):
         with L.pack_batch(self.ctx.stream):
-            for l in self.layers:
-                l.pack()
-            self.gru.pack()
-            if self.bank_d is not None:
-                self._pack_bank_d()
+            pack_operands(self.ctx, *self.operands())
 
     def forward(self, x, training, noise=None, noise_kind=2, seed=0, drop_masks=None, seed_ptr=None, lengths=None, tape=None):
         c, ns = self.ctx, self.ns
@@ -245,16 +257,17 @@
 
     BANK_PAD = 3
 
-    def _pack_bank_d(self):
+    def _bank_d_operands(self):
         c, c1 = self.ctx, self.c1
         ld, cp = self.bank_d_ld, self.bank_d_cp
+        ops = []
         for i, l in enumerate(self.conv1s):
             k = l.k
-            for j in range(k):
-                s = j + self.BANK_PAD - k // 2
-                L.call('zs_pack_weight', 'ZsPackWeight', c.stream, dtype=c.dt, W=L.ptr(l.w, j), so=self.c_in * k, si=k, sj=1,
-                       Cout=c1, Cin=self.c_in, taps=1, transpose=1, co_split2=0, inner_pad=c1, dst=L.ptr(self.bank_d), ldw=ld,
-                       n_rows=self.bank_d_rows, n_cols=c1, row_offset=0, col_offset=s * cp + i * c1)
+            raw = [dict(dtype=c.dt, W=L.ptr(l.w, j), so=self.c_in * k, si=k, sj=1, Cout=c1, Cin=self.c_in, taps=1, transpose=1,
+                        co_split2=0, inner_pad=c1, dst=L.ptr(self.bank_d), ldw=ld, n_rows=self.bank_d_rows, n_cols=c1, row_offset=0,
+                        col_offset=(j + self.BANK_PAD - k // 2) * cp + i * c1) for j in range(k)]
+            ops.append(weight_operand(l.w, c1, self.c_in, k, (self.c_in * k, k, 1), [], raw=raw))
+        return ops
 
     def _bank_operand(self):
         if self.bank_d is None:
@@ -263,8 +276,9 @@
             self.bank_d_ld = 7 * self.bank_d_cp
             self.bank_d_rows = rup(self.c_in, 128)
             self.bank_d = torch.zeros(self.bank_d_rows * self.bank_d_ld + 512, dtype=c.tdt, device=c.device)
+            self.adam_plan = None
             with L.pack_batch(c.stream):
-                self._pack_bank_d()
+                pack_operands(c, self._bank_d_operands(), [])
         return self.bank_d
 
     def backward_input(self, dbits=None, dlogits=None, tape=None):
@@ -318,11 +332,12 @@
             [self.dense5, self.linear]
         self.tape = None
 
+    def operands(self):
+        return operands_of(self.layers + [self.gru])
+
     def pack(self):
         with L.pack_batch(self.ctx.stream):
-            for l in self.layers:
-                l.pack()
-            self.gru.pack()
+            pack_operands(self.ctx, *self.operands())
 
     def forward(self, bits, cidx, training, lengths=None):
         c, ns, ch = self.ctx, self.ns, self.ch
@@ -557,10 +572,12 @@
         self.layers = [l for b in self.blocks for l in b[:2]] + [self.conv9]
         self.tape = None
 
+    def operands(self):
+        return operands_of(self.layers)
+
     def pack(self):
         with L.pack_batch(self.ctx.stream):
-            for l in self.layers:
-                l.pack()
+            pack_operands(self.ctx, *self.operands())
 
     def forward(self, x, training, seed=0, drop_masks=None):
         c, ns = self.ctx, self.ns
diff --git a/zerospeech-tts-without-t_amd/layers.py b/zerospeech-tts-without-t_amd/layers.py
--- a/zerospeech-tts-without-t_amd/layers.py
+++ b/zerospeech-tts-without-t_amd/layers.py
@@ -182,6 +182,54 @@
 
     def check_status(self):
         check_status(self.device)
+
+
+def weight_view(dst, transpose, inner_pad, ldw, n_rows, n_cols, dst_off=0, row_offset=0, col_offset=0, parity=False, row_perm=None):
+    return dict(dst=dst, dst_off=dst_off, transpose=transpose, inner_pad=inner_pad, ldw=ldw, n_rows=n_rows, n_cols=n_cols,
+                row_offset=row_offset, col_offset=col_offset, parity=parity, row_perm=row_perm)
+
+
+def weight_operand(w, Cout, Cin, taps, strides, views, co_split2=0, raw=None):
+    return dict(w=w, Cout=Cout, Cin=Cin, taps=taps, strides=tuple(strides), views=views, co_split2=int(co_split2), raw=raw or [])
+
+
+def vector_operand(src, copies):
+    return dict(src=src, copies=copies)
+
+
+def pack_operands(ctx, weights, vectors):
+    st = ctx.stream
+    for op in weights:
+        so, si, sj = op['strides']
+        common = dict(dtype=ctx.dt, so=so, si=si, Cout=op['Cout'], Cin=op['Cin'], co_split2=op['co_split2'])
+        for v in op['views']:
+            kw = dict(common, transpose=v['transpose'], inner_pad=v['inner_pad'], dst=L.ptr(v['dst'], v['dst_off']), ldw=v['ldw'],
+                      n_rows=v['n_rows'], row_offset=v['row_offset'], row_perm=L.ptr(v['row_perm']))
+            if v['parity']:
+                ne, no = (op['taps'] + 1) // 2, op['taps'] // 2
+                L.call('zs_pack_weight', 'ZsPackWeight', st, W=L.ptr(op['w']), sj=2 * sj, taps=ne, n_cols=ne * v['inner_pad'],
+                       col_offset=v['col_offset'], **kw)
+                L.call('zs_pack_weight', 'ZsPackWeight', st, W=L.ptr(op['w'], sj), sj=2 * sj, taps=no, n_cols=no * v['inner_pad'],
+                       col_offset=v['col_offset'] + ne * v['inner_pad'], **kw)
+            else:
+                L.call('zs_pack_weight', 'ZsPackWeight', st, W=L.ptr(op['w']), sj=sj, taps=op['taps'], n_cols=v['n_cols'],
+                       col_offset=v['col_offset'], **kw)
+        for kw in op['raw']:
+            L.call('zs_pack_weight', 'ZsPackWeight', st, **kw)
+    for vc in vectors:
+        for cp in vc['copies']:
+            L.vec_copy(cp['dst'][cp['dst_off']:cp['dst_off'] + cp['n']], vc['src'][cp['src_offset']:], st, src_stride=cp['src_stride'],
+                       n=cp['n'])
+
+
+class PlanCtx(object):
+
+    def __init__(self, dtype='bf16'):
+        self.device = torch.device('meta')
+        self.dtype_name = dtype
+        self.dt, self.tdt = DTYPES[dtype]
+        self.es = 4 if dtype == 'fp32' else 2
+        self.kc = 128 // self.es
 
 
 class ConvLayer(object):
@@ -213,27 +261,19 @@
     def from_params(cls, ctx, P, G, name, pad_mode, **kw):
         return cls(ctx, P[name + '.weight'], P[name + '.bias'], G[name + '.weight'], G[name + '.bias'], pad_mode=pad_mode, name=name, **kw)
 
-    def pack(self):
-        c = self.ctx
-        common = dict(dtype=c.dt, W=L.ptr(self.w), so=self.so, si=self.si, sj=self.sj, Cout=self.Cout, Cin=self.Cin,
-                      taps=self.k, co_split2=int(self.split2))
-        L.call('zs_pack_weight', 'ZsPackWeight', c.stream, transpose=0, inner_pad=self.cin_pad, dst=L.ptr(self.wf),
-               ldw=self.ldw, n_rows=self.n_pad, n_cols=self.ldw, **common)
-        if self.parity:
-            ne, no = (self.k + 1) // 2, self.k // 2
-            ev = dict(common, taps=ne, sj=2 * self.sj)
-            od = dict(common, taps=no, sj=2 * self.sj, W=L.ptr(self.w, self.sj))
-            L.call('zs_pack_weight', 'ZsPackWeight', c.stream, transpose=1, inner_pad=self.cout_pad, dst=L.ptr(self.wd),
-                   ldw=self.ldw_d, n_rows=self.n_pad_d, n_cols=ne * self.cout_pad, **ev)
-            L.call('zs_pack_weight', 'ZsPackWeight', c.stream, transpose=1, inner_pad=self.cout_pad, dst=L.ptr(self.wd),
-                   ldw=self.ldw_d, n_rows=self.n_pad_d, n_cols=no * self.cout_pad, col_offset=ne * self.cout_pad, **od)
-        else:
-            L.call('zs_pack_weight', 'ZsPackWeight', c.stream, transpose=1, inner_pad=self.cout_pad, dst=L.ptr(self.wd),
-                   ldw=self.ldw_d, n_rows=self.n_pad_d, n_cols=self.ldw_d, **common)
+    def operands(self):
+        views = [weight_view(self.wf, 0, self.cin_pad, self.ldw, self.n_pad, self.ldw),
+                 weight_view(self.wd, 1, self.cout_pad, self.ldw_d, self.n_pad_d, self.ldw_d, parity=self.parity)]
+        w = [weight_operand(self.w, self.Cout, self.Cin, self.k, (self.so, self.si, self.sj), views, co_split2=self.split2)]
+        v = []
         if self.bias_p is not None:
             h = self.Cout // 2
-            L.vec_copy(self.bias_p[:h], self.b, c.stream, src_stride=2)
-            L.vec_copy(self.bias_p[h:], self.b[1:], c.stream, src_stride=2)
+            v = [vector_operand(self.b, [dict(dst=self.bias_p, dst_off=0, n=h, src_offset=0, src_stride=2),
+                                         dict(dst=self.bias_p, dst_off=h, n=h, src_offset=1, src_stride=2)])]
+        return w, v
+
+    def pack(self):
+        pack_operands(self.ctx, *self.operands())
 
     def bias_ptr(self):
         if self.b is None:
@@ -347,19 +387,24 @@
     def out_hw(self, H, W):
         return (H + 2 * self.pad - self.k) // self.stride + 1, (W + 2 * self.pad - self.k) // self.stride + 1
 
-    def pack(self):
+    def operands(self):
         c, k = self.ctx, self.k
         common = dict(dtype=c.dt, so=self.Cin * self.taps, si=self.taps, Cout=self.Cout, Cin=self.Cin, co_split2=0)
+        views = []
         if self.wf is not None:
-            L.call('zs_pack_weight', 'ZsPackWeight', c.stream, transpose=0, inner_pad=self.cin_pad, dst=L.ptr(self.wf), ldw=self.ldw,
-                   n_rows=self.n_pad, n_cols=self.ldw, W=L.ptr(self.w), sj=1, taps=self.taps, **common)
+            views.append(weight_view(self.wf, 0, self.cin_pad, self.ldw, self.n_pad, self.ldw))
+        raw = []
         step = self.stride
         for (ph, pw), (buf, ld) in self.wd.items():
             nh, nw = self.nt[ph], self.nt[pw]
             for kwp in range(nw):
-                L.call('zs_pack_weight', 'ZsPackWeight', c.stream, transpose=1, inner_pad=self.cout_pad, dst=L.ptr(buf), ldw=ld,
-                       n_rows=self.n_pad_d, n_cols=nh * self.cout_pad, col_offset=kwp * nh * self.cout_pad,
-                       W=L.ptr(self.w, (pw + step * kwp) * k + ph), sj=step, taps=nh, **common)
+                raw.append(dict(common, transpose=1, inner_pad=self.cout_pad, dst=L.ptr(buf), ldw=ld, n_rows=self.n_pad_d,
+                                n_cols=nh * self.cout_pad, col_offset=kwp * nh * self.cout_pad,
+                                W=L.ptr(self.w, (pw + step * kwp) * k + ph), sj=step, taps=nh))
+        return [weight_operand(self.w, self.Cout, self.Cin, self.taps, (self.Cin * self.taps, self.taps, 1), views, raw=raw)], []
+
+    def pack(self):
+        pack_operands(self.ctx, *self.operands())
 
     def fwd(self, X, H, W, out, act=L.ZS_ACT_NONE, slope=0.0, bias=True, out_f32=False):
         c = self.ctx
@@ -537,23 +582,24 @@
             hc, rem = n // 96, n % 96
             self.perm = ((rem // 32) * H + hc * 32 + (rem % 32)).to(torch.int32).to(dev)
 
+    def operands(self):
+        c, H, Cin = self.ctx, self.H, self.Cin
+        w, v = [], []
+        for d in range(2):
+            w.append(weight_operand(self.w_ih[d], 3 * H, Cin, 1, (Cin, 1, 0), [
+                weight_view(self.wih_f, 0, self.cin_pad, self.ih_ldw, 3 * H, self.ih_ldw, row_offset=3 * H * d),
+                weight_view(self.wih_d, 1, 3 * H, self.ih_ldw_d, self.ih_npad_d, 3 * H, col_offset=3 * H * d)]))
+            w.append(weight_operand(self.w_hh[d], 3 * H, H, 1, (H, 1, 0), [
+                weight_view(self.whh_f, 0, rup(H, c.kc), self.hh_ldw, (3 * H if self.fast else self.hh_npad), self.hh_ldw,
+                            dst_off=d * self.hh_npad * self.hh_ldw, row_perm=self.perm),
+                weight_view(self.whh_t, 1, rup(3 * H, c.kc), self.hh_ldw_t, self.hh_npad_t, self.hh_ldw_t,
+                            dst_off=d * self.hh_npad_t * self.hh_ldw_t)]))
+            v.append(vector_operand(self.b_ih[d], [dict(dst=self.bih, dst_off=3 * H * d, n=3 * H, src_offset=0, src_stride=1)]))
+            v.append(vector_operand(self.b_hh[d], [dict(dst=self.bhh, dst_off=3 * H * d, n=3 * H, src_offset=0, src_stride=1)]))
+        return w, v
+
     def pack(self):
-        c, H, Cin = self.ctx, self.H, self.Cin
-        for d in range(2):
-            com = dict(dtype=c.dt, so=Cin, si=1, sj=0, Cout=3 * H, Cin=Cin, taps=1, co_split2=0, W=L.ptr(self.w_ih[d]))
-            L.call('zs_pack_weight', 'ZsPackWeight', c.stream, transpose=0, inner_pad=self.cin_pad, dst=L.ptr(self.wih_f),
-                   ldw=self.ih_ldw, n_rows=3 * H, n_cols=self.ih_ldw, row_offset=3 * H * d, **com)
-            L.call('zs_pack_weight', 'ZsPackWeight', c.stream, transpose=1, inner_pad=3 * H, dst=L.ptr(self.wih_d),
-                   ldw=self.ih_ldw_d, n_rows=self.ih_npad_d, n_cols=3 * H, col_offset=3 * H * d, **com)
-            com = dict(dtype=c.dt, so=H, si=1, sj=0, Cout=3 * H, Cin=H, taps=1, co_split2=0, W=L.ptr(self.w_hh[d]))
-            L.call('zs_pack_weight', 'ZsPackWeight', c.stream, transpose=0, inner_pad=rup(H, c.kc),
-                   dst=L.ptr(self.whh_f, d * self.hh_npad * self.hh_ldw), ldw=self.hh_ldw,
-                   n_rows=(3 * H if self.fast else self.hh_npad), n_cols=self.hh_ldw, row_perm=L.ptr(self.perm), **com)
-            L.call('zs_pack_weight', 'ZsPackWeight', c.stream, transpose=1, inner_pad=rup(3 * H, c.kc),
-                   dst=L.ptr(self.whh_t, d * self.hh_npad_t * self.hh_ldw_t), ldw=self.hh_ldw_t, n_rows=self.hh_npad_t,
-                   n_cols=self.hh_ldw_t, **com)
-            L.vec_copy(self.bih[3 * H * d:3 * H * (d + 1)], self.b_ih[d], c.stream)
-            L.vec_copy(self.bhh[3 * H * d:3 * H * (d + 1)], self.b_hh[d], c.stream)
+        pack_operands(self.ctx, *self.operands())
 
     def _work(self, B):
         n = L.lib().zs_gru_work_bytes(B, self.H)
diff --git a/zerospeech-tts-without-t_amd/model.py b/zerospeech-tts-without-t_amd/model.py
--- a/zerospeech-tts-without-t_amd/model.py
+++ b/zerospeech-tts-without-t_amd/model.py
@@ -71,7 +71,28 @@
             self._engine()
         else:
             z['engine'].pack()
-            z['version'] = sum(p._version for p in self.parameters())
+            self.mark_packed()
+
+    def mark_packed(self):
+        self._zs['version'] = sum(p._version for p in self.parameters())
+
+    def adam_pack_plan(self):
+        eng = self._engine()
+        if not hasattr(eng, 'operands'):
+            return None
+        if getattr(eng, 'adam_plan', None) is None:
+            from .optim import AdamPackPlan
+            eng.adam_plan = AdamPackPlan(self._zs['flat'], eng.ctx, *eng.operands())
+        return eng.adam_plan
+
+    def adam_pack_jobs(self, dtype=None):
+        from .layers import PlanCtx
+        from .optim import plan_jobs
+        flat, gflat = self.flat_params()
+        P = {k: p.data for k, p in self.named_parameters()}
+        G = {k: self.grad_view(k) for k, _ in self.named_parameters()}
+        eng = self._make_engine(PlanCtx(dtype or self._zs_dtype), P, G)
+        return plan_jobs(flat, *eng.operands())
 
     def set_compute_dtype(self, dtype):
         if dtype != self._zs_dtype:
diff --git a/zerospeech-tts-without-t_amd/optim.py b/zerospeech-tts-without-t_amd/optim.py
--- a/zerospeech-tts-without-t_amd/optim.py
+++ b/zerospeech-tts-without-t_amd/optim.py
@@ -1,7 +1,110 @@
+import ctypes
+
 import torch
 
 from . import _lib as L
 from . import parallel
+from .layers import pack_operands
+
+MAX_TAPS = 7
+
+
+def _in_flat(flat, t):
+    return t.untyped_storage().data_ptr() == flat.untyped_storage().data_ptr() and t.device == flat.device
+
+
+def plan_jobs(flat, weights, vectors):
+    jobs, rest_w, rest_v, taken = [], [], [], set()
+
+    def dense(t, shape_strides):
+        return _in_flat(flat, t) and t.storage_offset() not in taken and shape_strides
+
+    for op in weights:
+        w, (so, si, sj), k = op['w'], op['strides'], op['taps']
+        ok = op['views'] and k <= MAX_TAPS and w.numel() == op['Cout'] * op['Cin'] * k and w.is_contiguous() and \
+            (so, si) == (op['Cin'] * k, k) and (sj == 1 or k == 1)
+        if dense(w, ok):
+            taken.add(w.storage_offset())
+            jobs.append(dict(kind='weight', off=w.storage_offset(), len=w.numel(), op=op))
+            if op['raw']:
+                rest_w.append(dict(op, views=[]))
+        else:
+            rest_w.append(op)
+    for vc in vectors:
+        b = vc['src']
+        if dense(b, b.is_contiguous() and len(vc['copies']) <= 2):
+            taken.add(b.storage_offset())
+            jobs.append(dict(kind='vector', off=b.storage_offset(), len=b.numel(), op=vc))
+        else:
+            rest_v.append(vc)
+    jobs.sort(key=lambda j: j['off'])
+    out, end = [], 0
+    for j in jobs:
+        if j['off'] > end:
+            out.append(dict(kind='range', off=end, len=j['off'] - end))
+        out.append(j)
+        end = j['off'] + j['len']
+    if end < flat.numel():
+        out.append(dict(kind='range', off=end, len=flat.numel() - end))
+    check_cover(out, flat.numel())
+    return out, rest_w, rest_v
+
+
+def check_cover(jobs, n):
+    end = 0
+    for i, j in enumerate(jobs):
+        if j['len'] <= 0 or j['off'] != end:
+            raise L.ZsError('adam_pack plan: job %d (%s) covers [%d, %d) but the jobs before it end at %d (%s)' %
+                            (i, j['kind'], j['off'], j['off'] + j['len'], end, 'overlap' if j['off'] < end else 'hole'))
+        end = j['off'] + j['len']
+    if end != n:
+        raise L.ZsError('adam_pack plan: the jobs cover [0, %d) of a buffer of %d elements' % (end, n))
+
+
+class AdamPackPlan(object):
+
+    def __init__(self, flat, ctx, weights, vectors):
+        self.ctx = ctx
+        jobs, self.rest_w, self.rest_v = plan_jobs(flat, weights, vectors)
+        J, V = L.STRUCTS['ZsAdamPackJob'], L.STRUCTS['ZsAdamPackView']
+        self._keep = []
+        arr = (J * len(jobs))()
+        tiles = L.lib().zs_adam_pack_tiles
+        total = 0
+        for a, j in zip(arr, jobs):
+            a.kind = {'weight': L.ZS_APJ_WEIGHT, 'vector': L.ZS_APJ_VECTOR, 'range': L.ZS_APJ_RANGE}[j['kind']]
+            a.dtype, a.off, a.len = ctx.dt, j['off'], j['len']
+            op = j.get('op')
+            if j['kind'] == 'weight':
+                a.Cout, a.Cin, a.taps, a.co_split2, a.n_views = op['Cout'], op['Cin'], op['taps'], op['co_split2'], len(op['views'])
+                for i, v in enumerate(op['views']):
+                    inv = None
+                    if v['row_perm'] is not None:
+                        inv = torch.empty_like(v['row_perm'])
+                        inv[v['row_perm'].long()] = torch.arange(inv.numel(), dtype=inv.dtype, device=inv.device)
+                        self._keep.append(inv)
+                    a.view[i] = V(dst=L.ptr(v['dst'], v['dst_off']), ldw=v['ldw'], dst_elems=v['dst'].numel() - v['dst_off'],
+                                  transpose=v['transpose'], inner_pad=v['inner_pad'], row_offset=v['row_offset'],
+                                  col_offset=v['col_offset'], parity=int(v['parity']), row_inv=L.ptr(inv))
+            elif j['kind'] == 'vector':
+                a.n_views = len(op['copies'])
+                for i, cp in enumerate(op['copies']):
+                    a.view[i] = V(dst=L.ptr(cp['dst'], cp['dst_off']), ldw=1, dst_elems=cp['dst'].numel() - cp['dst_off'],
+                                  vlen=cp['n'], src_offset=cp['src_offset'], src_stride=cp['src_stride'])
+            a.tile_start = total
+            n = tiles(ctypes.addressof(a))
+            if n <= 0:
+                L.check(n or -1, 'zs_adam_pack_tiles')
+            total += n
+        self.jobs, self.n, self.tiles = arr, len(jobs), total
+        self.jobs_dev = torch.frombuffer(bytearray(bytes(arr)), dtype=torch.uint8).to(flat.device)
+
+    def launch(self, adam, part, n_part, stream):
+        L.check(L.lib().zs_adam_pack(ctypes.addressof(adam), ctypes.addressof(self.jobs), L.ptr(self.jobs_dev), self.n, part, n_part,
+                                     stream), 'zs_adam_pack')
+        if self.rest_w or self.rest_v:
+            with L.pack_batch(stream):
+                pack_operands(self.ctx, self.rest_w, self.rest_v)
 
 
 class NetOpt(object):
@@ -32,13 +135,16 @@
         L.check(L.lib().zs_sqnorm(L.ptr(gflat), gflat.numel(), L.ptr(self.part), L.ptr(self.sq), st), 'zs_sqnorm')
         return self.sq
 
-    def _adam(self, bc1, bc2, max_norm, step_ptr=None):
+    def _adam_args(self, bc1, bc2, max_norm, step_ptr=None):
         flat, gflat = self.net.flat_params()
         b1, b2 = self.betas
-        L.call('zs_adam_clip', 'ZsAdam', torch.cuda.current_stream(flat.device).cuda_stream, p=L.ptr(flat), g=L.ptr(gflat),
-               m=L.ptr(self.m), v=L.ptr(self.v), n=flat.numel(), lr=self.lr, beta1=b1, beta2=b2, eps=1e-8, bc1=bc1, bc2=bc2,
-               sumsq=L.ptr(self.sq), max_norm=float(max_norm) if max_norm else 0.0, write_clipped_grad=0, step_ptr=step_ptr,
-               grad_scale=1.0 / parallel.world_size())
+        return dict(p=L.ptr(flat), g=L.ptr(gflat), m=L.ptr(self.m), v=L.ptr(self.v), n=flat.numel(), lr=self.lr, beta1=b1, beta2=b2,
+                    eps=1e-8, bc1=bc1, bc2=bc2, sumsq=L.ptr(self.sq), max_norm=float(max_norm) if max_norm else 0.0,
+                    write_clipped_grad=0, step_ptr=step_ptr, grad_scale=1.0 / parallel.world_size())
+
+    def _adam(self, bc1, bc2, max_norm, step_ptr=None):
+        L.call('zs_adam_clip', 'ZsAdam', torch.cuda.current_stream(self.m.device).cuda_stream,
+               **self._adam_args(bc1, bc2, max_norm, step_ptr))
 
     def adam(self, t, max_norm=None):
         b1, b2 = self.betas
@@ -54,9 +160,21 @@
         self.adam(self.t, max_norm)
 
     def device_step(self, step_ptr):
-        self.sqnorm()
-        self._adam(1.0, 1.0, self.max_norm, step_ptr=step_ptr)
-        self.net.repack()
+        plan = self.net.adam_pack_plan() if L.get_option('adam_pack') else None
+        if plan is None:
+            self.sqnorm()
+            self._adam(1.0, 1.0, self.max_norm, step_ptr=step_ptr)
+            self.net.repack()
+            return
+        _, gflat = self.net.flat_params()
+        st = torch.cuda.current_stream(gflat.device).cuda_stream
+        n_part = L.lib().zs_sqnorm_stage1(L.ptr(gflat), gflat.numel(), L.ptr(self.part), st)
+        if n_part <= 0:
+            L.check(n_part or -1, 'zs_sqnorm_stage1')
+        kw = self._adam_args(1.0, 1.0, self.max_norm, step_ptr=step_ptr)
+        adam = L.STRUCTS['ZsAdam'](**{k: v for k, v in kw.items() if v is not None})
+        plan.launch(adam, L.ptr(self.part), n_part, st)
+        self.net.mark_packed()
 
 
 def softmax_ce(ctx, logits, target, loss, correct, grad_scale=1.0):
```

New measurement: 3.153 million frames/s, median of 6. 1.3% higher.
